# lightalchemist/nonlocal-image-edit

Measured on AMD Instinct MI355X. Metric: megapixels/sec end-to-end enhance (4K img, m=200, K=50); device-resident input and output (host->host per SURVEY 8d: host_to_host.value), higher is better.
Workload: dtype f64; 1 GPU; cfg4: 4096x4096 synthetic luminance, 20x10 samples (p=200), K=50, T=10, L=4 layers; device-resident: the luminance plane is in HBM when the timed region starts and the 4 layer planes are left in HBM (no PCIe inside `value`); parallelism=single GPU, formulation=phi_free_tables, storage=fp64 tables, histograms, reductions and MFMA; fp32 output planes

## Files before the change

nonlocal-image-edit_amd/csrc/generic64.hip:

```cpp
#include "kernels.h"

#include <algorithm>

namespace nlek {

typedef double f64x4 __attribute__((ext_vector_type(4)));

namespace {
__device__ __forceinline__ double recip0_g(double s, double eps) {
    return (fabs(s) >= eps) ? 1.0 / s : 0.0;
}
}

constexpr int kAff64Pix = 64;

template <bool CHROMA>
__global__ __launch_bounds__(256) void k_affinity64(const float* __restrict__ lum, GridSpec gs,
                                                    const Sample4* __restrict__ samples, int p, int ld, double sw,
                                                    double pw, long long pix0, long long M, double* __restrict__ kab,
                                                    int skip_samples, const unsigned* __restrict__ smask,
                                                    const float* __restrict__ pa, const float* __restrict__ pb,
                                                    const float2* __restrict__ sab, double cw) {
    extern __shared__ __attribute__((aligned(16))) unsigned char smem_raw64[];
    int2* srow_col = reinterpret_cast<int2*>(smem_raw64);
// ... 275 lines not shown
        hipLaunchKernelGGL((k_rowpass64<NCLV>), dim3((unsigned)nb), dim3(256), shm, s, mode, d_X, M, ld, w, lw, d_t_in, \
                           d_lam, d_xvec, eps, d_partial);                                                              \
    }
    if (lw <= 64) NLE_RP64(1)
    else if (lw <= 128) NLE_RP64(2)
    else if (lw <= 256) NLE_RP64(4)
    else if (lw <= 512) NLE_RP64(8)
    else if (lw <= 1024) NLE_RP64(16)
    else NLE_RP64(32)
#undef NLE_RP64
    return hipGetLastError();
}

__global__ __launch_bounds__(256) void k_gram64d(const double* __restrict__ X, long long M, int ld, int r,
                                                 const double* __restrict__ cs, long long rows_per_chunk,
                                                 double* __restrict__ partial) {
    const int lane = threadIdx.x & 63, wave = threadIdx.x >> 6, l15 = lane & 15, kq = lane >> 4;
    const int nt = (r + 15) / 16;
    int t = blockIdx.x * 4 + wave;
    const int npairs = nt * (nt + 1) / 2;
    if (t >= npairs) return;
    int ti = 0;
    while (t >= nt - ti) {
        t -= nt - ti;
        ++ti;
    }
    const int tj = ti + t;
    const long long i0 = (long long)blockIdx.y * rows_per_chunk, i1 = min(M, i0 + rows_per_chunk);
    const int ca = ti * 16 + l15, cb = tj * 16 + l15;
    f64x4 acc = f64x4{0.0, 0.0, 0.0, 0.0};
    for (long long i = i0; i < i1; i += 4) {
        const long long row = i + kq;
        const bool ok = row < i1;
        const double c = ok ? (cs ? cs[row] : 1.0) : 0.0;
        const double a = (ok && ca < r) ? c * X[(size_t)row * ld + ca] : 0.0;
        const double b = (ok && cb < r) ? c * X[(size_t)row * ld + cb] : 0.0;
        acc = __builtin_amdgcn_mfma_f64_16x16x4f64(a, b, acc, 0, 0, 0);
    }
    double* out = partial + (size_t)blockIdx.y * r * r;
#pragma unroll
    for (int e = 0; e < 4; ++e) {
        const int ra = ti * 16 + kq + 4 * e;
        if (ra < r && cb < r) out[(size_t)cb * r + ra] = acc[e];
    }
}

__global__ void k_gram64d_reduce(const double* __restrict__ partial, int nchunks, int r, double* __restrict__ G) {
    const long long idx = (long long)blockIdx.x * blockDim.x + threadIdx.x;
    if (idx >= (long long)r * r) return;
    const int a = (int)(idx % r), b = (int)(idx / r);
    const int ta = a / 16, tb = b / 16;
    const size_t src = (ta <= tb) ? (size_t)b * r + a : (size_t)a * r + b;
    double s = 0.0;
    for (int c = 0; c < nchunks; ++c) s += partial[(size_t)c * r * r + src];
    G[idx] = s;
}

long long gram64d_chunk_rows(long long M) {
    long long rows = (M + 255) / 256;
    rows = std::max<long long>(((rows + 3) / 4) * 4, 256);
    return rows;
}
size_t gram64d_partial_elems(long long M, int r) {
    const long long rows = gram64d_chunk_rows(M);
    const long long nchunks = std::max<long long>(1, (M + rows - 1) / rows);
    return (size_t)nchunks * r * r;
}

hipError_t gram64d(hipStream_t s, const double* d_X, long long M, int ld, int r, const double* d_cs, double* d_partial,
                   double* d_G) {
    const long long rows = gram64d_chunk_rows(M);
    const int nchunks = (int)std::max<long long>(1, (M + rows - 1) / rows);
    const int nt = (r + 15) / 16, npairs = nt * (nt + 1) / 2;
    hipError_t e = hipMemsetAsync(d_partial, 0, (size_t)nchunks * r * r * sizeof(double), s);
    if (e != hipSuccess) return e;
    if (M > 0)
        hipLaunchKernelGGL(k_gram64d, dim3((unsigned)((npairs + 3) / 4), (unsigned)nchunks), dim3(256), 0, s, d_X, M, ld, r, d_cs,
                           rows, d_partial);
    hipLaunchKernelGGL(k_gram64d_reduce, dim3((unsigned)(((long long)r * r + 255) / 256)), dim3(256), 0, s, d_partial, nchunks, r,
                       d_G);
    return hipGetLastError();
}

__global__ __launch_bounds__(256) void k_apply_expand64(const double* __restrict__ V, long long M, int ld, int K,
                                                        const double* __restrict__ g, int L, float* __restrict__ Y,
                                                        long long ystride) {
    extern __shared__ __attribute__((aligned(16))) unsigned char smem_raw[];
    double* sg = reinterpret_cast<double*>(smem_raw);
    for (int j = threadIdx.x; j < L * K; j += 256) sg[j] = g[(size_t)(j / K) * ld + (j % K)];
    __syncthreads();
    for (long long i = (long long)blockIdx.x * 256 + threadIdx.x; i < M; i += (long long)gridDim.x * 256) {
        const double* v = V + (size_t)i * ld;
        for (int l = 0; l < L; ++l) {
            double s0 = 0.0, s1 = 0.0;
            int k = 0;
            for (; k + 1 < K; k += 2) {
                s0 += v[k] * sg[l * K + k];
                s1 += v[k + 1] * sg[l * K + k + 1];
            }
            if (k < K) s0 += v[k] * sg[l * K + k];
            Y[(size_t)l * ystride + i] = (float)(s0 + s1);
        }
    }
}

hipError_t apply_expand64(hipStream_t s, const double* d_V, long long M, int ld, int K, const double* d_g, int L, float* d_Y,
                          long long ystride) {
    if (M <= 0 || L <= 0) return hipSuccess;
    const size_t per_layer = (size_t)K * sizeof(double);
    if (per_layer > kApplyLdsBytes) return hipErrorInvalidValue;
    const int lmax = per_layer ? (int)std::min<size_t>(kApplyLdsBytes / per_layer, (size_t)L) : L;
    const int ngroups = (L + lmax - 1) / lmax, lg = (L + ngroups - 1) / ngroups;
    const long long nb = std::min<long long>((M + 255) / 256, 4096);
    for (int l0 = 0; l0 < L; l0 += lg) {
        const int ln = std::min(lg, L - l0);
        const size_t shm = (size_t)ln * per_layer;
        if (shm > 48 * 1024) {
            hipError_t ea = hipFuncSetAttribute(reinterpret_cast<const void*>(k_apply_expand64),
                                                hipFuncAttributeMaxDynamicSharedMemorySize, (int)shm);
            if (ea != hipSuccess) return ea;
        }
        hipLaunchKernelGGL(k_apply_expand64, dim3((unsigned)nb), dim3(256), shm, s, d_V, M, ld, K, d_g + (size_t)l0 * ld, ln,
                           d_Y + (size_t)l0 * ystride, ystride);
    }
    return hipGetLastError();
}

__global__ void k_scatter_rows64(const double* __restrict__ src, const long long* __restrict__ idx, int n, int ld,
                                 double* __restrict__ X, long long M) {
    const long long f = (long long)blockIdx.x * blockDim.x + threadIdx.x;
    if (f >= (long long)n * ld) return;
    const int k = (int)(f / ld), j = (int)(f % ld);
    const long long row = idx[k];
    if (row >= 0 && row < M) X[(size_t)row * ld + j] = src[f];
}

hipError_t scatter_rows64(hipStream_t s, const double* d_src, const long long* d_idx, int n, int ld, double* d_X, long long M) {
    if (n <= 0) return hipSuccess;
    hipLaunchKernelGGL(k_scatter_rows64, dim3((unsigned)(((long long)n * ld + 255) / 256)), dim3(256), 0, s, d_src, d_idx, n, ld,
                       d_X, M);
    return hipGetLastError();
}

__global__ void k_scale_rows64(double* __restrict__ X, int m, int n, const double* __restrict__ dl) {
    const long long f = (long long)blockIdx.x * blockDim.x + threadIdx.x;
    if (f < (long long)m * n) X[f] *= dl[f % m];
}
hipError_t scale_rows64(hipStream_t s, double* d_X, int m, int n, const double* d_dl) {
    if (m <= 0 || n <= 0) return hipSuccess;
    hipLaunchKernelGGL(k_scale_rows64, dim3((unsigned)(((long long)m * n + 255) / 256)), dim3(256), 0, s, d_X, m, n, d_dl);
    return hipGetLastError();
}

__global__ void k_to_f32(const double* __restrict__ X, long long n, float* __restrict__ out) {
    for (long long i = (long long)blockIdx.x * blockDim.x + threadIdx.x; i < n; i += (long long)gridDim.x * blockDim.x)
        out[i] = (float)X[i];
}
hipError_t to_f32(hipStream_t s, const double* d_X, long long n, float* d_out) {
    if (n <= 0) return hipSuccess;
    hipLaunchKernelGGL(k_to_f32, dim3((unsigned)std::min<long long>((n + 255) / 256, 8192)), dim3(256), 0, s, d_X, n, d_out);
    return hipGetLastError();
}

}
```

nonlocal-image-edit_amd/csrc/kernels.h:

```cpp
#pragma once
#include <hip/hip_runtime.h>

#include <vector>

namespace nlek {

struct GridSpec {
    int H, W;
    int rowStep, rowOff, nSelRows;
    int colStep, colOff, nSelCols;
    __host__ __device__ int p() const { return nSelRows * nSelCols; }
};

typedef float4 Sample4;

#if defined(__HIPCC__)
__device__ __forceinline__ float affinity_value(float pr, float pc, float px, Sample4 s, float nsw, float npw) {
    const float dr = pr - s.x, dc = pc - s.y, dv = px - s.z;
    return __builtin_amdgcn_exp2f(nsw * (dr * dr + dc * dc) + npw * (dv * dv));
}
__device__ __forceinline__ bool is_sample_pixel(const GridSpec& gs, int row, int col) {
    const int dr = row - gs.rowOff, dc = col - gs.colOff;
    if (dr < 0 || dc < 0) return false;
    const int qr = dr / gs.rowStep, qc = dc / gs.colStep;
    return (qr * gs.rowStep == dr) && (qc * gs.colStep == dc) && qr < gs.nSelRows && qc < gs.nSelCols;
}
__device__ __forceinline__ bool is_sample(const GridSpec& gs, const unsigned* smask, long long gi, int row, int col) {
    return smask ? ((smask[gi >> 5] >> (unsigned)(gi & 31)) & 1u) != 0 : is_sample_pixel(gs, row, col);
}
#endif

struct LaunchObserver {
    virtual void begin(int sub) = 0;
    virtual void end() = 0;
    virtual ~LaunchObserver() = default;
};
enum { SUB_HIST_G = 0, SUB_HIST_PIX = 1, SUB_HIST_HH = 2, SUB_HIST_Z = 3 };
enum { SUB_GHIST_ROWS = 0, SUB_GHIST_EE = 1, SUB_GHIST_GEMM = 2, SUB_GHIST_FINAL = 3 };

constexpr int kRowpassMaxBlocks = 1024;
constexpr size_t kApplyLdsBytes = 64 * 1024;
constexpr int kGramTilesPerWave = 7;
constexpr int kGramRowsPerStage = 32;

enum RowpassMode { ROWPASS_COLSUM = 0, ROWPASS_RECIP = 1, ROWPASS_XVEC = 2 };

hipError_t gather_samples(hipStream_t s, const float* d_lum, GridSpec gs, float* d_out);
hipError_t gather_samples_slab(hipStream_t s, const float* d_lum, GridSpec gs, int row0, int row1, double* d_out);

hipError_t affinity(hipStream_t s, const float* d_lum, GridSpec gs, const Sample4* d_samples,
                    int p, int ld, float nsw, float npw, long long pix0, long long M,
                    float* d_kab);

hipError_t ts_gemm(hipStream_t s, bool fused, const float* d_A, int lda, const float* d_lum,
                   GridSpec gs, const Sample4* d_samples, float nsw, float npw, long long pix0,
                   const float* d_B, int ldb, int kd, float* d_C, int ldc, long long M,
                   const double* d_u, double eps, const float* d_c = nullptr);

size_t ts_gemm_bf16x3_bsplit_elems(int kd, int ldb);
hipError_t ts_gemm_bf16x3_split(hipStream_t s, const float* d_B, int kd, int ldb, unsigned short* d_Bs);
hipError_t ts_gemm_bf16x3(hipStream_t s, const float* d_lum, GridSpec gs, const Sample4* d_samples, float nsw, float npw,
                          long long pix0, const unsigned short* d_Bs, int ldb, int kd, float* d_C, int ldc, long long M,
                          const float* d_c = nullptr);

hipError_t rowpass(hipStream_t s, int mode, const float* d_X, long long M, int ld,
                   const double* d_t_in, const double* d_lam, const float* d_xvec, double eps,
                   double* d_partial, int* nblocks);
hipError_t reduce_partials(hipStream_t s, const double* d_partial, int nblocks, int ld,
                           double* d_t_out, int nslices = 1);
hipError_t scale_vec(hipStream_t s, const double* d_lam, const double* d_t, int n, double* d_u);
hipError_t row_scalings(hipStream_t s, const float* d_X, long long M, int ld, const double* d_u,
                        double eps, double* d_out);

int gram_num_tiles(int ld);
int gram_chunk_rows(long long M);
size_t gram_partial_elems(long long M, int ld);
hipError_t gram(hipStream_t s, const float* d_X, long long M, int ld, const double* d_u,
                double eps, double* d_partial, double* d_tiles);
hipError_t gram_reduce(hipStream_t s, const double* d_partial, int nchunks, int ntiles, double* d_tiles);

int sink_pass_ld(int p);
int sink_pass_rows(long long M);
int sink_pass_max_p();
hipError_t sink_pass(hipStream_t s, int mode, const float* d_lum, GridSpec gs, const Sample4* d_samples,
                     int p, const double* d_w, float nsw, float npw, long long pix0, long long M, double eps,
                     double* d_ybuf, double* d_partial);
hipError_t sink_update(hipStream_t s, int mode, int p, int r, bool chol, const double* d_X1, const double* d_X2,
                       const double* d_lam, const double* d_z, int zrows, int zld, const double* d_sA_cur, double eps,
                       double* d_v, double* d_u, double* d_sA_next, double* d_w_next);
constexpr int kG64TilesPerWave = 23;
int gram64_ld(int p);
int gram64_num_tiles(int p);
size_t gram64_partial_elems(long long M, int p);
hipError_t gram64(hipStream_t s, const float* d_lum, GridSpec gs, const Sample4* d_samples, int p, float nsw,
                  float npw, long long pix0, long long M, const double* d_c, double* d_partial, double* d_tiles);
int project64_ld(int K);
hipError_t project64(hipStream_t s, const float* d_lum, GridSpec gs, const Sample4* d_samples, int p, float nsw,
                     float npw, long long pix0, long long M, const double* d_D, int K, const double* d_c, float* d_V,
                     int ldv);

hipError_t check_levels(hipStream_t s, const float* d_lum, long long n, int* d_flag);
hipError_t hist_tables(hipStream_t s, GridSpec gs, const Sample4* d_samples, int p, double hx, double hy, int row0,
                       int nrows_local, double* d_er, double* d_ecT, double* d_Ep);

hipError_t affinity64(hipStream_t s, const float* d_lum, GridSpec gs, const Sample4* d_samples, int p, int ld, double sw,
                      double pw, long long pix0, long long M, double* d_kab, bool skip_samples = false,
                      const unsigned* d_smask = nullptr);
constexpr size_t kDynLdsDefault = 64 * 1024;
size_t affinity64_chroma_lds_bytes(int ld);
hipError_t affinity64_chroma(hipStream_t s, const float* d_lum, const float* d_a, const float* d_b, GridSpec gs,
                             const Sample4* d_samples, const float2* d_sab, int p, int ld, double sw, double pw, double cw,
                             long long pix0, long long M, double* d_kab, bool skip_samples = false,
                             const unsigned* d_smask = nullptr);
int patch_kpad(int R);
size_t patch_spatch_bytes(int p, int R);
hipError_t patch_gather(hipStream_t s, const float* d_lum, int H, int W, int R, const long long* d_pix, int n, int* d_out);
hipError_t patch_affinity64(hipStream_t s, const float* d_lum, GridSpec gs, int R, const Sample4* d_samples,
                            const signed char* d_spatch, const int* d_snorm, int p, int ld, double sw, double pwd,
                            long long pix0, long long M, double* d_kab, bool skip_samples = false,
                            const unsigned* d_smask = nullptr);
int patch_ckpad(int R);
size_t patch_cpatch_bytes(int p, int R);
constexpr size_t kPatchChromaLdsMax = 128 * 1024;
size_t patch_affinity64_chroma_lds_bytes(int ld);
hipError_t patch_affinity64_chroma(hipStream_t s, const float* d_lum, const float* d_a, const float* d_b, GridSpec gs, int R,
                                   const Sample4* d_samples, const signed char* d_spatch, const int* d_snorm,
                                   const signed char* d_cpatch, const int* d_cnorm, int p, int ld, double sw, double pwd,
                                   double cwd, long long pix0, long long M, double* d_kab, bool skip_samples = false,
                                   const unsigned* d_smask = nullptr);
int farthest_max_blocks();
hipError_t farthest_samples(hipStream_t s, const float* d_lum, int H, int W, int p, double sw, double pw, double* d_m,
                            double* d_pv, int* d_pi, int* d_list);
hipError_t gather_pix(hipStream_t s, const float* d_lum, const long long* d_pix, int n, float* d_out);
hipError_t sample_mask(hipStream_t s, const long long* d_pix, int n, long long N, unsigned* d_mask);
hipError_t add64(hipStream_t s, double* d_y, const double* d_x, size_t n);
hipError_t row_scalings64(hipStream_t s, const double* d_X, long long M, int ld, int r, const double* d_u, double eps,
                          double* d_out);
hipError_t ts_gemm64(hipStream_t s, const double* d_A, long long M, int lda, int kd, const double* d_B, int nc,
                     const double* d_rs, double* d_C, int ldc);
hipError_t gemm64s(hipStream_t s, int m, int n, int kk, const double* A, long long rsA, long long csA, const double* B,
                   long long rsB, long long csB, double* C, long long rsC, long long csC, const double* dl = nullptr,
                   const double* dk = nullptr, const double* dr = nullptr, const double* add = nullptr, long long rsD = 0,
                   long long csD = 0);
hipError_t rowpass64(hipStream_t s, int mode, const double* d_X, long long M, int ld, int w, const double* d_t_in,
                     const double* d_lam, const float* d_xvec, double eps, double* d_partial, int* nblocks);
size_t gram64d_partial_elems(long long M, int r);
hipError_t gram64d(hipStream_t s, const double* d_X, long long M, int ld, int r, const double* d_cs, double* d_partial,
                   double* d_G);
hipError_t apply_expand64(hipStream_t s, const double* d_V, long long M, int ld, int K, const double* d_g, int L, float* d_Y,
                          long long ystride);
hipError_t scatter_rows64(hipStream_t s, const double* d_src, const long long* d_idx, int n, int ld, double* d_X, long long M);
hipError_t to_f32(hipStream_t s, const double* d_X, long long n, float* d_out);
hipError_t scale_rows64(hipStream_t s, double* d_X, int m, int n, const double* d_dl);

int tridiag_max_n();
hipError_t tridiag(hipStream_t s, int n, const double* d_Q, const double* d_diag_add, double* d_V, double* d_d, double* d_e,
                   double* d_hs);

int sytrd_max_n();
int sytrd_groups(int n);
size_t sytrd_pub_elems(int n);
hipError_t sytrd_dist(hipStream_t s, int n, int G, const double* d_A, const double* d_diag_add, double* d_pub, double* d_d,
                      double* d_e, int* d_status);
hipError_t tridiag_bisect(hipStream_t s, int n, const double* d_d, const double* d_e, double* d_D);
hipError_t sytrd_back(hipStream_t s, int n, const double* d_pub, int K, double* d_Z, int ldz);
size_t potrf_tmp_elems(int n);
hipError_t potrf_inverse(hipStream_t s, int n, const double* d_A, double* d_L, double* d_Linv, double* d_tmp, double* d_scal,
                         int* d_status);
hipError_t transpose64(hipStream_t s, int n, const double* d_src, double* d_dst, int lds = 0, int ldd = 0);
hipError_t symm_lower64(hipStream_t s, int n, const double* d_src, double* d_dst);
hipError_t fill64(hipStream_t s, double* d_p, size_t n, double v);
hipError_t scale_rc64(hipStream_t s, int n, const double* d_src, int lds, const double* d_dl, const double* d_dr, double* d_dst);

constexpr int kSortedThreads = 512;
struct SortedRows {
    const unsigned short* scol;
    const uint2* desc;
    const unsigned short* first;
    const double* E;
    bool rec;
    double kappa;
    const double* E2 = nullptr;
    double hx = 0.0;
    int lev_t0 = 0, lev_nt = 16;
    bool mom = false;
};
bool sorted_gsum_ok(GridSpec gs, double hx);
hipError_t sorted_gram_sums(hipStream_t s, GridSpec gs, int nrows_local, const unsigned short* d_scol, const uint2* d_desc,
                            const unsigned short* d_first, const double* d_E2, const double* d_cvec, double* d_Aout, double hx);
bool sorted_recurrence(GridSpec gs, double hx, double* kappa);
int sorted_max_width();
size_t sorted_scol_elems(int W, int nrows_local);
int sorted_gram_max_cols();
int sorted_expand_max_cols();
int sorted_expand_max_width();
int sorted_expand_layers(GridSpec gs);
hipError_t sorted_expand(hipStream_t s, GridSpec gs, int nrows_local, const unsigned short* d_scol, const uint2* d_desc,
                         const double* d_E, const double* d_g, size_t gstride, int nl, const double* d_cvec, float* d_out,
                         long long ostride, bool rec = false, double kappa = 0.0, bool round8 = false);
hipError_t dist_table(hipStream_t s, int W, double hx, double* d_E);
hipError_t sort_rows(hipStream_t s, const float* d_lum, GridSpec gs, int row0, int nrows_local, unsigned short* d_scol,
                     uint2* d_desc, unsigned short* d_first);
hipError_t sorted_pass(hipStream_t s, int mode, GridSpec gs, int row0, int nrows_local, const unsigned short* d_scol,
                       const uint2* d_desc, const unsigned short* d_first, const double* d_E, const double* d_g, double eps,
                       double* d_ybuf, double* d_h, const double* d_cvec, const float* d_xvec, bool rec, double kappa,
                       int lev_t0 = 0, int lev_nt = 16,
                       bool mom = false);
bool sorted_moments_ok(GridSpec gs, double hx);
hipError_t sorted_gram_rows(hipStream_t s, GridSpec gs, int nrows_local, const unsigned short* d_scol, const uint2* d_desc,
                            const unsigned short* d_first, const double* d_E, const double* d_cvec, double* d_Aout, bool rec,
                            double kappa);

size_t hist_tiled_workspace_elems(GridSpec gs, int nrows_local);
hipError_t sink_hist_tiled(hipStream_t s, int mode, const float* d_lum, GridSpec gs, int p, int ldp, int row0,
                           int nrows_local, const double* d_er, const double* d_ecT, const double* d_Ep,
                           const double* d_w, double eps, double* d_ybuf, double* d_ws, double* d_z,
                           LaunchObserver* obs = nullptr, const double* d_cvec = nullptr,
                           const float* d_xvec = nullptr,
                           const SortedRows* sorted = nullptr);
int apply_layers_per_launch(GridSpec gs);
bool use_sorted_expand(GridSpec gs, const SortedRows* sorted);
hipError_t apply_hist_layers(hipStream_t s, const float* d_lum, GridSpec gs, int p, int row0, int nrows_local,
                             const double* d_er, const double* d_ecT, const double* d_Ep, const double* d_wl, int ldw,
                             int nl, const double* d_c, double* d_ws, float* d_out, long long ostride,
                             LaunchObserver* obs, const SortedRows* sorted = nullptr, bool round8 = false);
hipError_t apply_small(hipStream_t s, int p, int K, int ldk, int L, int ldw, const double* d_m, const double* d_D,
                       const double* d_Vrows, const double* d_xA , const double* d_resp,
                       double* d_t, double* d_Wp, double* d_YA);
hipError_t scatter_samples(hipStream_t s, int p, int L, const long long* d_loc, const double* d_YA, float* d_Y,
                           long long ystride, bool round8 = false);

int ghist_max_cols();
size_t ghist_workspace_elems(GridSpec gs, int nrows_local);
hipError_t gram_hist(hipStream_t s, const float* d_lum, GridSpec gs, int p, int row0, int nrows_local,
                     const double* d_er, const double* d_ecT, const double* d_Ep, const double* d_c, double* d_ws,
                     double* d_Gk, LaunchObserver* obs = nullptr, const SortedRows* sorted = nullptr);

hipError_t bgr2lab8(hipStream_t s, const unsigned char* d_bgr, long long n, const double* d_lut, unsigned char* d_lab,
                    float* d_L);
hipError_t lab2bgr8(hipStream_t s, const unsigned char* d_lab, const float* d_L, const float* d_a, const float* d_b,
                    long long n, const double* d_lut, unsigned char* d_bgr);
hipError_t channel8(hipStream_t s, const unsigned char* d_img, long long n, int ch, float* d_out);
hipError_t plane_to_u8(hipStream_t s, const float* d_y, long long n, unsigned char* d_out);
hipError_t channel8_plane(hipStream_t s, const unsigned char* d_u8, long long n, float* d_out);
int bilateral8_max_radius();
hipError_t bilateral8(hipStream_t s, const float* d_src, int H, int W, int radius, const float* d_space_w,
                      const float* d_colour_w, float* d_dst);

hipError_t col_range(hipStream_t s, const float* d_X, long long M, int ld, int ncols, float* d_out, int nblocks);

hipError_t apply_expand(hipStream_t s, const float* d_V, long long M, int ld, const double* d_g,
                        int L, float* d_Y, long long ystride);

hipError_t scatter_rows(hipStream_t s, const float* d_src, const long long* d_idx, int n, int ld,
                        float* d_X, long long M);

struct ExactPlane {
    const float* lum;
    int H, W;
    const double* d_es;
    int es_len;
    const double* d_el;
    double* d_part;
};
void exact_tables(int H, int W, double hx, double hy, std::vector<double>* es, std::vector<double>* el);
size_t exact_part_elems(long long N);
hipError_t affinity_product64(hipStream_t s, const ExactPlane& pl, const double* d_X, int ldx, int ncols, double* d_Y, int ldy);
hipError_t exact_start(hipStream_t s, double* d_X, long long N, int ld, int col0, int ncols, unsigned seed);
hipError_t exact_scale2(hipStream_t s, const double* d_X, int ldx, long long N, int b, const double* d_c, const double* d_r,
                        double* d_Z);
hipError_t exact_combine(hipStream_t s, const double* d_Y, long long N, int b, const double* d_c, const double* d_r, double* d_A,
                         int lda);
hipError_t exact_recip(hipStream_t s, double* d_v, long long N, double eps);
hipError_t exact_axpby(hipStream_t s, const double* d_S, int lds, double alpha, const double* d_B, int ldb, double beta,
                       double* d_D, int ldd, long long N, int n, int pad);
int exact_col_blocks(long long N);
hipError_t exact_colnorm2(hipStream_t s, const double* d_A, int lda, const double* d_B, int ldb, const double* d_theta,
                          long long N, int n, double* d_part);
hipError_t exact_colmaxabs(hipStream_t s, const double* d_A, int lda, long long N, int n, double* d_pv);
hipError_t exact_scale_cols(hipStream_t s, double* d_A, int lda, long long N, int n, const double* d_s);

}
```

nonlocal-image-edit_amd/csrc/ortho.h:

```cpp
#pragma once
#include "devsolve.h"

namespace nlep {

constexpr double kCholMaxInvTrace = 1e9;

struct KaDevice {
    DevBuf<double> Ka;
    DevChol ch;
};

struct Nystrom {
    int r = 0, ldr = 0;
    bool chol = false;
    std::shared_ptr<KaDevice> dev;
    std::vector<double> VA;
    std::vector<double> lam;
    std::vector<double> B;
    std::vector<double> Ka;
};

struct Ortho {
    int q = 0, K = 0, r_wa = 0, r_q = 0;
    bool chol_wa = false;
    std::vector<double> Sq, Cproj, VArows, Wa;
};

struct OrthoSS {
    int q = 0, K = 0, r_wa = 0, r_q = 0;
    bool chol_wa = false;
    std::vector<double> Sq, D, Vrows;
    int p = 0, r = 0;
    std::vector<double> cA, rA, Kr, P, Wa, S, St, A2;
};

Ortho orthogonalize_host(const Nystrom& ny, int p, const std::vector<double>& u_c, const std::vector<double>& u_r,
                         std::vector<double> G, int n_eig, bool device_f32 = true, int topk_solver = 0);
void ortho_ss_prepare(OrthoSS& o, const Nystrom& ny, int p, const std::vector<double>& sA_c, const std::vector<double>& sA_r,
                      bool literal_q = false);
void ortho_ss_finish(OrthoSS& o, std::vector<double> Gk, int n_eig, int topk_solver = 0);
void ortho_ss_device(nle_ctx* c, OrthoSS& o, const Nystrom& ny, int p, const std::vector<double>& sA_c,
                     const std::vector<double>& sA_r, double* d_Gk, int n_eig, const std::function<void()>& enqueue_gram,
                     const std::function<void()>& reduce_gram, double* host_ms, double* host_overlapped_ms, Trace& tr);

}
```

nonlocal-image-edit_amd/csrc/ortho.hip:

```cpp
#include "ortho.h"

using namespace nlep;

namespace {

template <typename F>
void par_cols(int n, long long work_per_col, F&& body) {
    const long long work = work_per_col * n;
    const int nt = (int)std::min<long long>(std::min<long long>(16, work / 40000000 + 1), n);
    if (nt <= 1) {
        body(0, n);
        return;
    }
    nleh::run_parts(nt, nt, [&](int t) { body((int)((long long)n * t / nt), (int)((long long)n * (t + 1) / nt)); });
}
void mm(const double* A, const double* B, double* C, int m, int k, int n) {
    par_cols(n, (long long)m * k, [&](int j0, int j1) { nleh::gemm_nn_cols(A, B, C, m, k, n, j0, j1); });
}
void mm_nt(const double* A, const double* B, double* C, int m, int k, int n) {
    par_cols(n, (long long)m * k, [&](int j0, int j1) { nleh::gemm_nt_cols(A, B, C, m, k, n, j0, j1); });
}
void mm_tn(const double* A, const double* B, double* C, int m, int k, int n) {
    par_cols(n, (long long)m * k, [&](int j0, int j1) { nleh::gemm_tn_cols(A, B, C, m, k, n, j0, j1); });
}

void top_eigenpairs(const std::vector<double>& Qm, int q, int n_eig, int solver, std::vector<double>* Vq,
                    std::vector<double>* Sq, int* rq) {
    if (solver == 1 && q > 1) {
        const int nev = std::min(std::max(n_eig, 1), q - 1);
        Vq->assign((size_t)q * nev, 0.0);
        Sq->assign(nev, 0.0);
        int restarts = 0;
        const int nconv = nleh::lanczos_topk(Qm.data(), q, nev, NLE_EPS, 1000, Vq->data(), Sq->data(), &restarts);
        if (nconv < 0) throw Fail{NLE_ERR_NUMERIC, "Lanczos: the projected eigenproblem did not converge"};
        if (nconv < nev)
            std::fprintf(stderr, "# converged eigenvalues: %d\nEigen decomposition NOT successful. Results might be inaccurate.\n", nconv);
        int r = 0;
        while (r < nconv && (*Sq)[r] >= NLE_EPS) ++r;
        *rq = r;
        if (std::getenv("NLE_TRACE")) std::fprintf(stderr, "[nle trace] Lanczos top-%d of %d: %d restarts, %d converged\n", nev, q, restarts, nconv);
        return;
    }
    Vq->assign((size_t)q * std::min(q, std::max(n_eig, 1)), 0.0);
    Sq->assign(q, 0.0);
    if (!nleh::eigen_decomposition_topk(Qm.data(), q, NLE_EPS, n_eig, Vq->data(), Sq->data(), rq))
        throw Fail{NLE_ERR_NUMERIC, "eigensolver did not converge on Q"};
}

void trace_wa(int kept, int q, double largest, double smallest_kept, int nd = -1, const char* where = "") {
    if (!std::getenv("NLE_TRACE")) return;
    char defl[64] = "";
    if (nd >= 0) std::snprintf(defl, sizeof defl, ", %d deflated%s", nd, where);
    std::fprintf(stderr, "[nle trace] Wa: %d of %d eigenvalues >= 1e-10 (largest %.3e, smallest kept %.3e)%s\n", kept, q, largest,
                 smallest_kept, defl);
}

struct EigRoot {
    std::vector<double> U2, l2, Us;
    int r2 = 0;
};
EigRoot eigen_root(const std::vector<double>& Wa, int q) {
    EigRoot e;
    e.U2.resize((size_t)q * q);
    e.l2.resize(q);
    if (!nleh::eigen_decomposition(Wa.data(), q, NLE_EPS, e.U2.data(), e.l2.data(), &e.r2))
        throw Fail{NLE_ERR_NUMERIC, "eigensolver did not converge on Wa"};
    e.Us.resize((size_t)q * std::max(e.r2, 1));
    for (int k = 0; k < e.r2; ++k) {
        const double s = std::sqrt(recip0(e.l2[k]));
        for (int i = 0; i < q; ++i) e.Us[(size_t)k * q + i] = e.U2[(size_t)k * q + i] * s;
    }
    trace_wa(e.r2, q, e.l2[0], e.r2 > 0 ? e.l2[e.r2 - 1] : 0.0);
    return e;
}

bool certified_cholesky(const std::vector<double>& Wa, int q, std::vector<double>& L, std::vector<double>& Li) {
    double inv_diag = 0.0;
    for (int a = 0; a < q; ++a) inv_diag += Wa[(size_t)a * q + a] > 0.0 ? 1.0 / Wa[(size_t)a * q + a] : 1e300;
    if (!(inv_diag <= kCholMaxInvTrace)) return false;
    L.resize((size_t)q * q);
    Li.resize((size_t)q * q);
    double inv_trace = 0.0;
    return nleh::cholesky_with_inverse(Wa.data(), q, L.data(), Li.data(), &inv_trace, kCholMaxInvTrace) && inv_trace <= kCholMaxInvTrace;
}

void sample_scalings(OrthoSS& o, const Nystrom& ny, int p, const std::vector<double>& sA_c, const std::vector<double>& sA_r) {
    o.p = p;
    o.r = ny.r;
    o.q = ny.r;
    o.cA.resize(p);
    o.rA.resize(p);
    for (int a = 0; a < p; ++a) {
        o.cA[a] = recip0(sA_c[a]);
        o.rA[a] = recip0(sA_r[a]);
    }
}

void build_Wa(OrthoSS& o) {
    const int p = o.p, q = o.q;
    o.Wa.resize((size_t)q * q);
    for (int b = 0; b < q; ++b)
        for (int a = 0; a < q; ++a) o.Wa[(size_t)b * q + a] = o.rA[a] * o.Kr[(size_t)b * p + a] * o.cA[b];
}

}

namespace nlep {

Ortho orthogonalize_host(const Nystrom& ny, int p, const std::vector<double>& u_c,
                         const std::vector<double>& u_r, std::vector<double> G, int n_eig, bool device_f32,
                         int topk_solver) {
    const int r = ny.r, q = ny.r;
    std::vector<double> cA(q), rA(q), cA32(q);
    std::vector<double> left((size_t)q * r), right((size_t)q * r), phi32((size_t)q * r);
    for (int a = 0; a < q; ++a) {
        double sc = 0.0, sr = 0.0, sc32 = 0.0;
        for (int k = 0; k < r; ++k) {
            const double v = ny.VA[(size_t)k * p + a];
            const double v32 = device_f32 ? (double)(float)v : v;
            phi32[(size_t)k * q + a] = v32;
            sc += v * u_c[k];
            sr += v * u_r[k];
            sc32 += v32 * u_c[k];
        }
        cA[a] = recip0(sc);
        rA[a] = recip0(sr);
        cA32[a] = recip0(sc32);
    }
    for (int k = 0; k < r; ++k)
        for (int a = 0; a < q; ++a) {
            const double v = ny.VA[(size_t)k * p + a];
            left[(size_t)k * q + a] = rA[a] * v * ny.lam[k];
            right[(size_t)k * q + a] = cA[a] * v;
        }
    Ortho o;
    o.q = q;
    o.Wa.resize((size_t)q * q);
    mm_nt(left.data(), right.data(), o.Wa.data(), q, r, q);
    for (int a = 0; a < q; ++a) {
        const double c2 = cA32[a] * cA32[a];
        for (int j = 0; j < r; ++j) {
            const double vj = c2 * phi32[(size_t)j * q + a];
            for (int i = 0; i < r; ++i) G[(size_t)j * r + i] -= phi32[(size_t)i * q + a] * vj;
        }
    }
    std::vector<double> LG((size_t)q * r), WW((size_t)q * q);
    mm(left.data(), G.data(), LG.data(), q, r, r);
    mm_nt(LG.data(), left.data(), WW.data(), q, r, q);
    const auto [U2, l2, Us, r2] = eigen_root(o.Wa, q);
    std::vector<double> S((size_t)q * q);
    o.r_wa = r2;
    if (r2 <= 0) throw Fail{NLE_ERR_NUMERIC, "Wa has no eigenvalue >= 1e-10"};
    std::vector<double> Vq, Sq, T2;
    int rq = 0, K = 0;
    if (topk_solver == 0) {
        std::vector<double> WF((size_t)q * r2), Qt((size_t)r2 * r2);
        mm(WW.data(), Us.data(), WF.data(), q, q, r2);
        mm_tn(Us.data(), WF.data(), Qt.data(), q, r2, r2);
        for (int k = 0; k < r2; ++k) Qt[(size_t)k * r2 + k] += l2[k];
        std::vector<double> Vt;
        top_eigenpairs(Qt, r2, n_eig, topk_solver, &Vt, &Sq, &rq);
        K = std::min(n_eig, rq);
        if (K <= 0) throw Fail{NLE_ERR_NUMERIC, "Q has no eigenvalue >= 1e-10"};
        T2.resize((size_t)q * K);
        mm(Us.data(), Vt.data(), T2.data(), q, r2, K);
    } else {
        mm_nt(Us.data(), U2.data(), S.data(), q, r2, q);
        std::vector<double> T1((size_t)q * q), Qm((size_t)q * q);
        mm(S.data(), WW.data(), T1.data(), q, q, q);
        mm(T1.data(), S.data(), Qm.data(), q, q, q);
        for (size_t i = 0; i < Qm.size(); ++i) Qm[i] += o.Wa[i];
        top_eigenpairs(Qm, q, n_eig, topk_solver, &Vq, &Sq, &rq);
        K = std::min(n_eig, rq);
        if (K <= 0) throw Fail{NLE_ERR_NUMERIC, "Q has no eigenvalue >= 1e-10"};
        T2.resize((size_t)q * K);
        mm(S.data(), Vq.data(), T2.data(), q, q, K);
    }
    o.K = K;
    o.r_q = rq;
    o.Sq.assign(Sq.begin(), Sq.begin() + K);
    for (int k = 0; k < K; ++k) {
        const double s = std::sqrt(recip0(Sq[k]));
        for (int i = 0; i < q; ++i) T2[(size_t)k * q + i] *= s;
    }
    o.Cproj.resize((size_t)r * K);
    mm_tn(left.data(), T2.data(), o.Cproj.data(), q, r, K);
    o.VArows.resize((size_t)q * K);
    mm(o.Wa.data(), T2.data(), o.VArows.data(), q, q, K);
    return o;
}

void ortho_ss_prepare(OrthoSS& o, const Nystrom& ny, int p, const std::vector<double>& sA_c,
                      const std::vector<double>& sA_r, bool literal_q) {
    const int r = ny.r, q = ny.r;
    sample_scalings(o, ny, p, sA_c, sA_r);
    if (ny.chol) {
        o.Kr = ny.Ka;
    } else {
        std::vector<double> VL((size_t)p * r);
        o.Kr.resize((size_t)p * p);
        for (int k = 0; k < r; ++k)
            for (int a = 0; a < p; ++a) VL[(size_t)k * p + a] = ny.VA[(size_t)k * p + a] * ny.lam[k];
        mm_nt(VL.data(), ny.VA.data(), o.Kr.data(), p, r, p);
        if (r < p) {
            o.P.resize((size_t)p * p);
            mm_nt(ny.VA.data(), ny.VA.data(), o.P.data(), p, r, p);
        }
    }
    build_Wa(o);
    o.S.resize((size_t)q * q);
    if (!literal_q && std::getenv("NLE_FORCE_EIG") == nullptr) {
        std::vector<double> L, Li;
        if (certified_cholesky(o.Wa, q, L, Li)) {
            std::vector<double> Lt((size_t)q * q);
            for (int k = 0; k < q; ++k)
                for (int a = 0; a < q; ++a) {
                    o.S[(size_t)k * q + a] = Li[(size_t)a * q + k];
                    Lt[(size_t)k * q + a] = L[(size_t)a * q + k];
                }
            o.St = std::move(Li);
            o.A2.resize((size_t)q * q);
            mm(Lt.data(), L.data(), o.A2.data(), q, q, q);
            o.r_wa = q;
            o.chol_wa = true;
            return;
        }
    }
    const auto [U2, l2, Us, r2] = eigen_root(o.Wa, q);
    mm_nt(Us.data(), U2.data(), o.S.data(), q, r2, q);
    o.r_wa = r2;
    o.St = o.S;
    o.A2 = o.Wa;
}

void ortho_ss_finish(OrthoSS& o, std::vector<double> Gk, int n_eig, int topk_solver) {
    const int p = o.p, r = o.r, q = o.q;
    const std::vector<double>&cA = o.cA, &rA = o.rA, &Kr = o.Kr, &Wa = o.Wa, &S = o.S;
    for (int a = q; a < p; ++a) {
        const double c2 = cA[a] * cA[a];
        const double* ka = Kr.data() + (size_t)a * p;
        for (int j = 0; j < p; ++j) {
            const double vj = c2 * ka[j];
            for (int i = 0; i < p; ++i) Gk[(size_t)j * p + i] += ka[i] * vj;
        }
    }
    if (r < p) {
        std::vector<double> T((size_t)p * p);
        mm(o.P.data(), Gk.data(), T.data(), p, p, p);
        mm(T.data(), o.P.data(), Gk.data(), p, p, p);
    }
    std::vector<double> WW((size_t)q * q);
    for (int b = 0; b < q; ++b)
        for (int a = 0; a < q; ++a) WW[(size_t)b * q + a] = rA[a] * Gk[(size_t)b * p + a] * rA[b];
    std::vector<double> T1((size_t)q * q), Qm((size_t)q * q);
    mm(o.St.data(), WW.data(), T1.data(), q, q, q);
    mm(T1.data(), S.data(), Qm.data(), q, q, q);
    for (size_t i = 0; i < Qm.size(); ++i) Qm[i] += o.A2[i];
    std::vector<double> Vq, Sq;
    int rq = 0;
    top_eigenpairs(Qm, q, n_eig, topk_solver, &Vq, &Sq, &rq);
    const int K = std::min(n_eig, rq);
    if (K <= 0) throw Fail{NLE_ERR_NUMERIC, "Q has no eigenvalue >= 1e-10"};
    o.K = K;
    o.r_q = rq;
    o.Sq.assign(Sq.begin(), Sq.begin() + K);
    std::vector<double> T2((size_t)q * K), RT2((size_t)q * K);
    mm(S.data(), Vq.data(), T2.data(), q, q, K);
    for (int k = 0; k < K; ++k) {
        const double sv = std::sqrt(recip0(Sq[k]));
        for (int i = 0; i < q; ++i) {
            T2[(size_t)k * q + i] *= sv;
            RT2[(size_t)k * q + i] = rA[i] * T2[(size_t)k * q + i];
        }
    }
    o.D.resize((size_t)p * K);
    if (r < p) {
        mm(o.P.data(), RT2.data(), o.D.data(), p, q, K);
    } else {
        o.D = RT2;
    }
    o.Vrows.assign((size_t)p * K, 0.0);
    std::vector<double> WT((size_t)q * K);
    mm(Wa.data(), T2.data(), WT.data(), q, q, K);
    for (int k = 0; k < K; ++k) {
        for (int a = 0; a < q; ++a) o.Vrows[(size_t)k * p + a] = WT[(size_t)k * q + a];
        for (int a = q; a < p; ++a) {
            double sv = 0.0;
            for (int j = 0; j < p; ++j) sv += Kr[(size_t)a * p + j] * o.D[(size_t)k * p + j];
            o.Vrows[(size_t)k * p + a] = cA[a] * sv;
        }
    }
}

namespace {


struct SsDevice {
    DevBuf<double> rA, cA, Kr, P, VA, lam;
};

void scalings_Kr_P(hipStream_t st, OrthoSS& o, const Nystrom& ny, int p, const std::vector<double>& sA_c,
                   const std::vector<double>& sA_r, SsDevice& dv) {
    const int r = ny.r;
    const size_t pp = (size_t)p * p;
    sample_scalings(o, ny, p, sA_c, sA_r);
    dv.rA.alloc(p);
    dv.cA.alloc(p);
    HIP_OK(hipMemcpyAsync(dv.rA.p, o.rA.data(), p * sizeof(double), hipMemcpyHostToDevice, st));
    HIP_OK(hipMemcpyAsync(dv.cA.p, o.cA.data(), p * sizeof(double), hipMemcpyHostToDevice, st));
    if (ny.chol) {
        o.Kr = ny.Ka;
        return;
    }
    dv.VA.alloc((size_t)p * r);
    dv.lam.alloc(r);
    dv.Kr.alloc(pp);
    HIP_OK(hipMemcpyAsync(dv.VA.p, ny.VA.data(), (size_t)p * r * sizeof(double), hipMemcpyHostToDevice, st));
    HIP_OK(hipMemcpyAsync(dv.lam.p, ny.lam.data(), r * sizeof(double), hipMemcpyHostToDevice, st));
    HIP_OK(nlek::gemm64s(st, p, p, r, dv.VA.p, 1, p, dv.VA.p, p, 1, dv.Kr.p, 1, p, nullptr, dv.lam.p));
    if (r < p) {
        dv.P.alloc(pp);
        HIP_OK(nlek::gemm64s(st, p, p, r, dv.VA.p, 1, p, dv.VA.p, p, 1, dv.P.p, 1, p));
    }
    o.Kr.resize(pp);
    HIP_OK(hipMemcpyAsync(o.Kr.data(), dv.Kr.p, pp * sizeof(double), hipMemcpyDeviceToHost, st));
    HIP_OK(hipStreamSynchronize(st));
}

struct WaRoot {
    enum Form { kEigen, kCholesky, kDeflated } form = kEigen;
    bool on_device = false;
    int m = 0;
    int r_wa = 0, nd = 0;
    std::vector<double> F, L, G, l2_kept;
    DevBuf<double> d_F, d_L, d_G;
    bool chol_form() const { return form != kEigen; }
};

struct WaDeviceWork {
    DevSymEig es;
    DevChol ch;
    DevBuf<double> Ah, Vd, wgt, W, neg1;
};

void wa_root_device(nle_ctx* c, const OrthoSS& o, const Nystrom& ny, const SsDevice& dv, double* d_Wa, bool force_eig,
                    const std::function<void()>& enqueue_gram, WaDeviceWork& ws, WaRoot& w, Trace& tr) {
    const int p = o.p, q = o.q, max_defl = q / 8;
    const size_t qq = (size_t)q * q;
    hipStream_t st = c->stream, sa = aux_stream(c);
    ws.es.prepare(c, q, sa);
    ws.ch.prepare(c, q, sa);
    ws.Ah.alloc(qq);
    w.d_F.alloc(qq);
    ws.Vd.alloc((size_t)q * (max_defl + 1));
    ws.wgt.alloc(max_defl + 1);
    ws.W.alloc((size_t)(max_defl + 1) * q);
    w.d_G.alloc((size_t)q * (max_defl + 1));
    ws.neg1.alloc(max_defl + 1);
    HIP_OK(hipStreamSynchronize(st));
    enqueue_gram();
    if (ny.dev)
        HIP_OK(nlek::scale_rc64(sa, q, ny.dev->Ka.p, p, dv.rA.p, dv.cA.p, d_Wa));
    else
        upload_staged(c, d_Wa, o.Wa.data(), qq, sa);
    HIP_OK(nlek::symm_lower64(sa, q, d_Wa, ws.Ah.p));
    bool reduced = false;
    if (!force_eig) {
        reduced = ws.es.reduce(c, q, ws.Ah.p, nullptr);
        if (c->world > 1) reduced = ranks_where(c, !reduced) == 0;
        tr.mark("ss:   Wa: tridiagonal form + eigenvalues (device)");
    }
    if (reduced) {
        const std::vector<double>& D = ws.es.D;
        int kept = 0;
        while (kept < q && D[kept] >= NLE_EPS) ++kept;
        const int nd = q - kept;
        if (kept > 0 && nd <= max_defl && D[0] > 0.0) {
            const double sig = D[0];
            if (nd > 0) {
                ws.es.vectors(c, kept, nd, ws.Vd.p);
                tr.mark("ss:   Wa: dropped eigenvectors (host inverse iteration)");
                std::vector<double> wgt(nd);
                for (int t = 0; t < nd; ++t) wgt[t] = sig - D[kept + t];
                HIP_OK(hipMemcpyAsync(ws.wgt.p, wgt.data(), nd * sizeof(double), hipMemcpyHostToDevice, sa));
                HIP_OK(nlek::gemm64s(sa, q, q, nd, ws.Vd.p, 1, q, ws.Vd.p, q, 1, ws.Ah.p, 1, q, nullptr, ws.wgt.p, nullptr, ws.Ah.p, 1, q));
                HIP_OK(hipStreamSynchronize(sa));
            }
            ws.ch.factor(c, q, ws.Ah.p);
            const bool fact_ok = ws.ch.finish(c);
            if (!fact_ok && std::getenv("NLE_TRACE"))
                fprintf(stderr, "[nle trace] Wa: the deflated matrix did not factor (trace of the inverse %.3e, %d dropped, sigma %.3e)\n",
                        ws.ch.inv_trace, nd, sig);
            if (fact_ok) {
                HIP_OK(nlek::transpose64(sa, q, ws.ch.Linv.p, w.d_F.p));
                if (nd > 0) {
                    HIP_OK(nlek::fill64(sa, ws.neg1.p, nd, -1.0));
                    HIP_OK(nlek::gemm64s(sa, nd, q, q, ws.Vd.p, q, 1, ws.ch.Linv.p, q, 1, ws.W.p, 1, nd));
                    HIP_OK(nlek::gemm64s(sa, q, q, nd, ws.Vd.p, 1, q, ws.W.p, 1, nd, w.d_F.p, 1, q, nullptr, ws.neg1.p, nullptr, w.d_F.p, 1, q));
                    HIP_OK(nlek::gemm64s(sa, q, nd, q, ws.ch.L.p, q, 1, ws.Vd.p, 1, q, w.d_G.p, 1, q));
                }
                w.form = nd > 0 ? WaRoot::kDeflated : WaRoot::kCholesky;
                w.on_device = true;
                w.r_wa = kept;
                w.nd = nd;
                trace_wa(kept, q, D[0], D[kept - 1], nd, " (device)");
            }
        }
    }
    if (w.on_device) {
        w.d_L.alloc(qq);
        HIP_OK(hipMemcpyAsync(w.d_L.p, ws.ch.L.p, qq * sizeof(double), hipMemcpyDeviceToDevice, sa));
    }
    HIP_OK(hipEventRecord(c->aux_ev, sa));
    HIP_OK(hipStreamWaitEvent(st, c->aux_ev, 0));
}

void wa_root_host(OrthoSS& o, bool cholesky_forms, bool force_eig, WaRoot& w, Trace& tr) {
    const int q = o.q, max_defl = q / 8;
    const size_t qq = (size_t)q * q;
    if (o.Wa.empty()) build_Wa(o);
    std::vector<double>& L = w.L;
    std::vector<double> Li, Vd;
    const bool attempt_chol = q < 64 || q >= 512;
    bool factored = cholesky_forms && !force_eig && attempt_chol && certified_cholesky(o.Wa, q, L, Li);
    int kept = q, nd = 0;
    if (!factored && cholesky_forms && !force_eig && q >= 16 && q < 512) {
        std::vector<double> Dbelow(max_defl + 1);
        Vd.resize((size_t)q * (max_defl + 1));
        double lam_max = 0.0, lam_min_kept = 0.0;
        tr.mark(attempt_chol ? "ss:   Wa built, Cholesky attempt" : "ss:   Wa built");
        if (nleh::sym_eigen_below(o.Wa.data(), q, NLE_EPS, max_defl, &kept, &lam_max, &lam_min_kept, Dbelow.data(), Vd.data())) {
            tr.mark("ss:   Wa eigenvalues + dropped eigenvectors");
            nd = q - kept;
            if (kept > 0 && nd <= max_defl && lam_max > 0.0) {
                const double sig = lam_max;
                std::vector<double> Ah(qq);
                for (int cidx = 0; cidx < q; ++cidx)
                    for (int ridx = 0; ridx < q; ++ridx)
                        Ah[(size_t)cidx * q + ridx] = ridx >= cidx ? o.Wa[(size_t)cidx * q + ridx] : o.Wa[(size_t)ridx * q + cidx];
                for (int t = 0; t < nd; ++t) {
                    const double wgt = sig - Dbelow[t];
                    const double* v = Vd.data() + (size_t)t * q;
                    for (int cidx = 0; cidx < q; ++cidx) {
                        const double vc = wgt * v[cidx];
                        for (int ridx = 0; ridx < q; ++ridx) Ah[(size_t)cidx * q + ridx] += v[ridx] * vc;
                    }
                }
                L.resize(qq);
                Li.resize(qq);
                double inv_trace = 0.0;
                factored = nleh::cholesky_with_inverse(Ah.data(), q, L.data(), Li.data(), &inv_trace);
                if (factored) {
                    tr.mark("ss:   deflated matrix + its Cholesky factor and inverse");
                    trace_wa(kept, q, lam_max, lam_min_kept, nd);
                }
            }
        }
    }
    if (factored) {
        std::vector<double>& F = w.F;
        F.resize(qq);
        for (int k = 0; k < q; ++k)
            for (int a = 0; a < q; ++a) F[(size_t)k * q + a] = Li[(size_t)a * q + k];
        w.G.assign((size_t)q * std::max(nd, 1), 0.0);
        std::vector<double> wv(q);
        for (int t = 0; t < nd; ++t) {
            const double* v = Vd.data() + (size_t)t * q;
            for (int k = 0; k < q; ++k) {
                double acc = 0.0, g = 0.0;
                for (int a = 0; a < q; ++a) {
                    acc += v[a] * Li[(size_t)a * q + k];
                    g += L[(size_t)k * q + a] * v[a];
                }
                wv[k] = acc;
                w.G[(size_t)t * q + k] = g;
            }
            for (int k = 0; k < q; ++k)
                for (int a = 0; a < q; ++a) F[(size_t)k * q + a] -= v[a] * wv[k];
        }
        w.form = nd > 0 ? WaRoot::kDeflated : WaRoot::kCholesky;
        w.r_wa = nd > 0 ? kept : q;
        w.nd = nd;
        return;
    }
    EigRoot e = eigen_root(o.Wa, q);
    w.form = WaRoot::kEigen;
    w.r_wa = e.r2;
    w.l2_kept.assign(e.l2.begin(), e.l2.begin() + e.r2);
    w.F = std::move(e.Us);
}

void upload_host_root(hipStream_t st, int q, WaRoot& w) {
    const size_t qq = (size_t)q * q;
    if (w.chol_form()) {
        w.d_L.alloc(qq);
        HIP_OK(hipMemcpyAsync(w.d_L.p, w.L.data(), qq * sizeof(double), hipMemcpyHostToDevice, st));
    }
    w.d_F.alloc((size_t)q * w.m);
    HIP_OK(hipMemcpyAsync(w.d_F.p, w.F.data(), (size_t)q * w.m * sizeof(double), hipMemcpyHostToDevice, st));
    if (w.form == WaRoot::kDeflated) {
        w.d_G.alloc((size_t)q * w.nd);
        HIP_OK(hipMemcpyAsync(w.d_G.p, w.G.data(), (size_t)q * w.nd * sizeof(double), hipMemcpyHostToDevice, st));
    }
    HIP_OK(hipStreamSynchronize(st));
}

void form_Qt(hipStream_t st, const OrthoSS& o, const SsDevice& dv, const WaRoot& w, double* d_Gk,
             const std::function<void()>& reduce_gram, double* d_Qm) {
    const int p = o.p, r = o.r, q = o.q, m = w.m;
    const size_t qq = (size_t)q * q;
    DevBuf<double> d_T((size_t)p * p), d_T1((size_t)m * q);
    reduce_gram();
    if (q < p) {
        std::vector<double> c2(p - q);
        for (int a = q; a < p; ++a) c2[a - q] = o.cA[a] * o.cA[a];
        DevBuf<double> d_c2(p - q);
        HIP_OK(hipMemcpyAsync(d_c2.p, c2.data(), (p - q) * sizeof(double), hipMemcpyHostToDevice, st));
        HIP_OK(nlek::gemm64s(st, p, p, p - q, dv.Kr.p + (size_t)q * p, 1, p, dv.Kr.p + (size_t)q * p, p, 1, d_Gk, 1, p, nullptr,
                             d_c2.p, nullptr, d_Gk, 1, p));
        HIP_OK(hipStreamSynchronize(st));
    }
    if (r < p) {
        HIP_OK(nlek::gemm64s(st, p, p, p, dv.P.p, 1, p, d_Gk, 1, p, d_T.p, 1, p));
        HIP_OK(nlek::gemm64s(st, p, p, p, d_T.p, 1, p, dv.P.p, 1, p, d_Gk, 1, p));
    }
    HIP_OK(nlek::gemm64s(st, m, q, q, w.d_F.p, q, 1, d_Gk, 1, p, d_T1.p, 1, m, nullptr, dv.rA.p));
    if (!w.chol_form()) {
        HIP_OK(nlek::gemm64s(st, m, m, q, d_T1.p, 1, m, w.d_F.p, 1, q, d_Qm, 1, m, nullptr, dv.rA.p));
        return;
    }
    DevBuf<double> d_A2(qq);
    HIP_OK(nlek::gemm64s(st, q, q, q, w.d_L.p, q, 1, w.d_L.p, 1, q, d_A2.p, 1, q));
    if (w.form == WaRoot::kDeflated) {
        DevBuf<double> d_neg(w.nd);
        HIP_OK(nlek::fill64(st, d_neg.p, w.nd, -1.0));
        HIP_OK(nlek::gemm64s(st, q, q, w.nd, w.d_G.p, 1, q, w.d_G.p, q, 1, d_A2.p, 1, q, nullptr, d_neg.p, nullptr, d_A2.p, 1, q));
    }
    HIP_OK(nlek::gemm64s(st, m, m, q, d_T1.p, 1, m, w.d_F.p, 1, q, d_Qm, 1, m, nullptr, dv.rA.p, nullptr, d_A2.p, 1, q));
}

struct QtEig {
    bool on_device = false;
    std::vector<double> Vq, Sq, sv;
    DevSymEig es;
    DevBuf<double> d_Vq, d_l2q;
};

void top_eigenpairs_Qt(nle_ctx* c, OrthoSS& o, const WaRoot& w, const double* d_Qm, int n_eig, QtEig& t, double* host_ms,
                       Trace& tr) {
    hipStream_t st = c->stream;
    const int m = w.m;
    const size_t mm_ = (size_t)m * m;
    int rq = 0;
    double h0 = 0.0;
    t.on_device = c->topk_solver == 0 && use_dev_solver(m) && !std::getenv("NLE_HOST_Q");
    if (t.on_device) {
        const double* d_add = nullptr;
        if (!w.chol_form()) {
            t.d_l2q.alloc(m);
            HIP_OK(hipMemcpyAsync(t.d_l2q.p, w.l2_kept.data(), m * sizeof(double), hipMemcpyHostToDevice, st));
            d_add = t.d_l2q.p;
        }
        t.on_device = t.es.reduce(c, m, d_Qm, d_add);
        if (c->world > 1) t.on_device = ranks_where(c, !t.on_device) == 0;
    }
    if (t.on_device) {
        tr.mark("ss: Q, its tridiagonal form and eigenvalues (device)");
        h0 = now_ms();
        t.Sq = t.es.D;
        while (rq < m && t.Sq[rq] >= NLE_EPS) ++rq;
        const int Kd = std::min(n_eig, rq);
        if (Kd > 0) {
            t.d_Vq.alloc((size_t)m * Kd);
            t.es.vectors(c, 0, Kd, t.d_Vq.p);
        }
    } else {
        std::vector<double> Qm(mm_);
        HIP_OK(hipMemcpyAsync(Qm.data(), d_Qm, mm_ * sizeof(double), hipMemcpyDeviceToHost, st));
        HIP_OK(hipStreamSynchronize(st));
        tr.mark("ss: Q on the device + download");
        h0 = now_ms();
        if (!w.chol_form())
            for (int k = 0; k < m; ++k) Qm[(size_t)k * m + k] += w.l2_kept[k];
        top_eigenpairs(Qm, m, n_eig, c->topk_solver, &t.Vq, &t.Sq, &rq);
    }
    const int K = std::min(n_eig, rq);
    if (K <= 0) throw Fail{NLE_ERR_NUMERIC, "Q has no eigenvalue >= 1e-10"};
    o.K = K;
    o.r_q = rq;
    o.Sq.assign(t.Sq.begin(), t.Sq.begin() + K);
    t.sv.resize(K);
    for (int k = 0; k < K; ++k) t.sv[k] = std::sqrt(recip0(t.Sq[k]));
    *host_ms += now_ms() - h0;
    tr.mark(t.on_device ? "ss: eigenvectors of Q (inverse iteration on the host, back-transformation enqueued)" : "ss: eig(Q) (host)");
}

void D_and_Vrows(hipStream_t st, OrthoSS& o, const SsDevice& dv, const WaRoot& w, QtEig& t, const double* d_Wa, Trace& tr) {
    const int p = o.p, r = o.r, q = o.q, m = w.m, K = o.K;
    DevBuf<double> d_sv(K), d_T2((size_t)q * K), d_D((size_t)p * K), d_Vr((size_t)p * K);
    if (!t.on_device) {
        t.d_Vq.alloc((size_t)m * K);
        HIP_OK(hipMemcpyAsync(t.d_Vq.p, t.Vq.data(), (size_t)m * K * sizeof(double), hipMemcpyHostToDevice, st));
    }
    HIP_OK(hipMemcpyAsync(d_sv.p, t.sv.data(), K * sizeof(double), hipMemcpyHostToDevice, st));
    HIP_OK(nlek::gemm64s(st, q, K, m, w.d_F.p, 1, q, t.d_Vq.p, 1, m, d_T2.p, 1, q, nullptr, nullptr, d_sv.p));
    if (r < p) {
        HIP_OK(nlek::gemm64s(st, p, K, q, dv.P.p, 1, p, d_T2.p, 1, q, d_D.p, 1, p, nullptr, dv.rA.p));
    } else {
        HIP_OK(hipMemcpyAsync(d_D.p, d_T2.p, (size_t)q * K * sizeof(double), hipMemcpyDeviceToDevice, st));
        HIP_OK(nlek::scale_rows64(st, d_D.p, p, K, dv.rA.p));
    }
    HIP_OK(nlek::gemm64s(st, q, K, q, d_Wa, 1, q, d_T2.p, 1, q, d_Vr.p, 1, p));
    if (q < p)
        HIP_OK(nlek::gemm64s(st, p - q, K, p, dv.Kr.p + q, 1, p, d_D.p, 1, p, d_Vr.p + q, 1, p, dv.cA.p + q));
    o.D.resize((size_t)p * K);
    o.Vrows.resize((size_t)p * K);
    HIP_OK(hipMemcpyAsync(o.D.data(), d_D.p, o.D.size() * sizeof(double), hipMemcpyDeviceToHost, st));
    HIP_OK(hipMemcpyAsync(o.Vrows.data(), d_Vr.p, o.Vrows.size() * sizeof(double), hipMemcpyDeviceToHost, st));
    HIP_OK(hipStreamSynchronize(st));
    tr.mark("ss: D, Vrows on the device");
}

}

void ortho_ss_device(nle_ctx* c, OrthoSS& o, const Nystrom& ny, int p, const std::vector<double>& sA_c,
                     const std::vector<double>& sA_r, double* d_Gk, int n_eig, const std::function<void()>& enqueue_gram,
                     const std::function<void()>& reduce_gram, double* host_ms, double* host_overlapped_ms, Trace& tr) {
    const int q = ny.r;
    hipStream_t st = c->stream;
    SsDevice dv;
    scalings_Kr_P(st, o, ny, p, sA_c, sA_r, dv);
    const double h0 = now_ms();
    const bool dev_wa = use_dev_solver(q) && !std::getenv("NLE_HOST_WA");
    const bool force_eig = std::getenv("NLE_FORCE_EIG") != nullptr;
    if (!(dev_wa && ny.dev)) build_Wa(o);
    DevBuf<double> d_Wa((size_t)q * q);
    WaRoot w;
    WaDeviceWork ws;
    if (dev_wa)
        wa_root_device(c, o, ny, dv, d_Wa.p, force_eig, enqueue_gram, ws, w, tr);
    else
        enqueue_gram();
    if (!w.on_device) wa_root_host(o, !dev_wa, force_eig, w, tr);
    o.r_wa = w.r_wa;
    o.chol_wa = w.form == WaRoot::kCholesky;
    *host_overlapped_ms += now_ms() - h0;
    tr.mark(w.on_device ? "ss: Wa root (device, second stream, beside the Gram kernels)" : "ss: Wa root (host, under the Gram kernels)");
    w.m = w.chol_form() ? q : std::max(w.r_wa, 0);
    if (w.m <= 0) throw Fail{NLE_ERR_NUMERIC, "Wa has no eigenvalue >= 1e-10"};
    DevBuf<double> d_Qm((size_t)w.m * w.m);
    if (!dev_wa) HIP_OK(hipMemcpyAsync(d_Wa.p, o.Wa.data(), (size_t)q * q * sizeof(double), hipMemcpyHostToDevice, st));
    if (!w.on_device) upload_host_root(st, q, w);
    form_Qt(st, o, dv, w, d_Gk, reduce_gram, d_Qm.p);
    QtEig t;
    top_eigenpairs_Qt(c, o, w, d_Qm.p, n_eig, t, host_ms, tr);
    D_and_Vrows(st, o, dv, w, t, d_Wa.p, tr);
}

}
```

nonlocal-image-edit_amd/csrc/pipeline.hip:

```cpp
#include "ortho.h"

using nlek::GridSpec;
using namespace nlep;

namespace {
struct SampleSet {
    GridSpec gs;
    int p = 0;
    std::vector<long long> pix;
    std::vector<float> val;
    std::vector<float4> packed;
    bool quantised = false;
    unsigned level_tiles = 0xffffu;
    int R = 0;
    bool listed = false;
    std::vector<int> patch;
    const float* d_a = nullptr;
    const float* d_b = nullptr;
    double hc = 0.0;
    bool chroma_quantised = false;
    std::vector<int> aval, bval;
    bool chroma() const { return d_a != nullptr; }
};

// ... 189 lines not shown
    const double sw = 1.0 / (hx * hx), pwd = (1.0 / (hy * hy)) / d;
    const bool chroma = s.chroma();
    const double cwd = chroma ? chroma_cwd(s) : 0.0;
    std::vector<double> Ka((size_t)p * p);
    for (int j = 0; j < p; ++j) {
        const int rj = (int)(s.pix[j] / s.gs.W), cj = (int)(s.pix[j] % s.gs.W);
        const int* yj = s.patch.data() + (size_t)j * d;
        for (int i = j; i < p; ++i) {
            const int ri = (int)(s.pix[i] / s.gs.W), ci = (int)(s.pix[i] % s.gs.W);
            const int* yi = s.patch.data() + (size_t)i * d;
            long long S = 0;
            for (int k = 0; k < d; ++k) S += (long long)(yi[k] - yj[k]) * (yi[k] - yj[k]);
            const long long dr = ri - rj, dc = ci - cj;
            double e = -sw * (double)(dr * dr + dc * dc) - pwd * (double)S;
            if (chroma) e = e - cwd * (double)chroma_ssd(s, i, j);
            const double v = std::exp(e);
            Ka[(size_t)j * p + i] = v;
            Ka[(size_t)i * p + j] = v;
        }
    }
    return Ka;
}

struct PatchOperands {
    DevBuf<signed char> spatch;
    DevBuf<int> snorm;
    DevBuf<float2> sab;
    DevBuf<signed char> cpatch;
    DevBuf<int> cnorm;
};
void upload_chroma_operands(nle_ctx* c, const SampleSet& s, PatchOperands* po) {
    if (s.R <= 0) {
        std::vector<float2> ab(s.p);
        for (int j = 0; j < s.p; ++j) ab[j] = make_float2((float)s.aval[j], (float)s.bval[j]);
        po->sab.alloc(s.p);
        HIP_OK(hipMemcpyAsync(po->sab.p, ab.data(), ab.size() * sizeof(float2), hipMemcpyHostToDevice, c->stream));
        HIP_OK(hipStreamSynchronize(c->stream));
        return;
    }
    const int d = (2 * s.R + 1) * (2 * s.R + 1), kp = nlek::patch_ckpad(s.R);
    std::vector<signed char> bytes(nlek::patch_cpatch_bytes(s.p, s.R), 0);
    std::vector<int> norm(s.p, 0);
    for (int j = 0; j < s.p; ++j)
        for (int k = 0; k < 2 * d; ++k) {
            const int v = (k < d ? s.aval[(size_t)j * d + k] : s.bval[(size_t)j * d + k - d]) - 128;
            bytes[(size_t)j * kp + k] = (signed char)v;
            norm[j] += v * v;
        }
    po->cpatch.alloc(bytes.size());
    po->cnorm.alloc(s.p);
    HIP_OK(hipMemcpyAsync(po->cpatch.p, bytes.data(), bytes.size(), hipMemcpyHostToDevice, c->stream));
    HIP_OK(hipMemcpyAsync(po->cnorm.p, norm.data(), norm.size() * sizeof(int), hipMemcpyHostToDevice, c->stream));
    HIP_OK(hipStreamSynchronize(c->stream));
}
void upload_patch_operands(nle_ctx* c, const SampleSet& s, PatchOperands* po) {
    if (s.chroma()) upload_chroma_operands(c, s, po);
    if (s.R <= 0) return;
    const int d = (2 * s.R + 1) * (2 * s.R + 1), kp = nlek::patch_kpad(s.R);
    std::vector<signed char> bytes(nlek::patch_spatch_bytes(s.p, s.R), 0);
    std::vector<int> norm(s.p, 0);
    for (int j = 0; j < s.p; ++j)
        for (int k = 0; k < d; ++k) {
            const int v = s.patch[(size_t)j * d + k] - 128;
            bytes[(size_t)j * kp + k] = (signed char)v;
            norm[j] += v * v;
        }
    po->spatch.alloc(bytes.size());
    po->snorm.alloc(s.p);
    HIP_OK(hipMemcpyAsync(po->spatch.p, bytes.data(), bytes.size(), hipMemcpyHostToDevice, c->stream));
    HIP_OK(hipMemcpyAsync(po->snorm.p, norm.data(), norm.size() * sizeof(int), hipMemcpyHostToDevice, c->stream));
    HIP_OK(hipStreamSynchronize(c->stream));
}

hipError_t affinity_rows64(hipStream_t st, const float* d_lum, const SampleSet& ss, const float4* d_samples,
                           const PatchOperands& po, int ld, double hx, double hy, long long pix0, long long M, double* d_kab,
                           bool skip_samples = false, const unsigned* d_smask = nullptr) {
    const double sw = 1.0 / (hx * hx), pw = 1.0 / (hy * hy);
    if (ss.chroma()) {
        const double cwd = chroma_cwd(ss);
        if (ss.R <= 0)
            return nlek::affinity64_chroma(st, d_lum, ss.d_a, ss.d_b, ss.gs, d_samples, po.sab.p, ss.p, ld, sw, pw, cwd, pix0, M,
                                           d_kab, skip_samples, d_smask);
        return nlek::patch_affinity64_chroma(st, d_lum, ss.d_a, ss.d_b, ss.gs, ss.R, d_samples, po.spatch.p, po.snorm.p,
                                             po.cpatch.p, po.cnorm.p, ss.p, ld, sw, pw / ((2 * ss.R + 1) * (2 * ss.R + 1)), cwd,
                                             pix0, M, d_kab, skip_samples, d_smask);
    }
    if (ss.R <= 0)
        return nlek::affinity64(st, d_lum, ss.gs, d_samples, ss.p, ld, sw, pw, pix0, M, d_kab, skip_samples, d_smask);
    const double pwd = pw / ((2 * ss.R + 1) * (2 * ss.R + 1));
    return nlek::patch_affinity64(st, d_lum, ss.gs, ss.R, d_samples, po.spatch.p, po.snorm.p, ss.p, ld, sw, pwd, pix0, M, d_kab,
                                  skip_samples, d_smask);
}

std::vector<double> build_Ka(const SampleSet& s, double hx, double hy) {
    if (s.R > 0) return build_Ka_patch(s, hx, hy);
    const int p = s.p;
    const double sw = 1.0 / (hx * hx), pw = 1.0 / (hy * hy);
    const bool chroma = s.chroma();
    const double cw = chroma ? chroma_cwd(s) : 0.0;
    std::vector<double> Ka((size_t)p * p);
    auto column = [&](int j) {
        const int rj = (int)(s.pix[j] / s.gs.W), cj = (int)(s.pix[j] % s.gs.W);
        for (int i = j; i < p; ++i) {
            const int ri = (int)(s.pix[i] / s.gs.W), ci = (int)(s.pix[i] % s.gs.W);
            const long long dr = ri - rj, dc = ci - cj;
            const double sq = (double)(dr * dr + dc * dc);
            const double dv = (double)s.val[i] - (double)s.val[j];
            double e = -sw * sq - pw * (dv * dv);
            if (chroma) e = e - cw * (double)chroma_ssd(s, i, j);
            const double v = std::exp(e);
            Ka[(size_t)j * p + i] = v;
            Ka[(size_t)i * p + j] = v;
        }
    };
    const int nt = p >= 384 ? 8 : 1;
    std::vector<int> cut(nt + 1, p);
    for (int t = 0; t < nt; ++t) cut[t] = (int)(p * (1.0 - std::sqrt(1.0 - (double)t / nt)));
    nleh::run_parts(nt, nt, [&](int t) {
        for (int j = cut[t]; j < cut[t + 1]; ++j) column(j);
    });
    return Ka;
}



Nystrom solve_Ka(nle_ctx* c, const std::vector<double>& Ka, int p, bool allow_chol) {
    Nystrom n;
    if (allow_chol && std::getenv("NLE_FORCE_EIG") == nullptr) {
        if (c && use_dev_solver(p) && !std::getenv("NLE_HOST_KA")) {
            const size_t pp = (size_t)p * p;
            auto kd = std::make_shared<KaDevice>();
            kd->Ka.alloc(pp);
            upload_staged(c, kd->Ka.p, Ka.data(), pp, c->stream);
            kd->ch.factor(c, p, kd->Ka.p);
            if (kd->ch.finish(c) && kd->ch.inv_trace <= kCholMaxInvTrace) {
                n.chol = true;
                n.r = p;
                n.ldr = ld4(p);
                n.lam.assign(p, 1.0);
                n.Ka = Ka;
                n.dev = std::move(kd);
                return n;
            }
        } else {
            std::vector<double> L((size_t)p * p), Li((size_t)p * p);
            double inv_trace = 0.0;
            if (nleh::cholesky_with_inverse(Ka.data(), p, L.data(), Li.data(), &inv_trace, kCholMaxInvTrace) &&
                inv_trace <= kCholMaxInvTrace) {
                n.chol = true;
                n.r = p;
                n.ldr = ld4(p);
                n.VA = std::move(L);
                n.lam.assign(p, 1.0);
                n.B.resize((size_t)p * p);
                for (int k = 0; k < p; ++k)
                    for (int a = 0; a < p; ++a) n.B[(size_t)k * p + a] = Li[(size_t)a * p + k];
                n.Ka = Ka;
                return n;
            }
        }
    }
    std::vector<double> U((size_t)p * p), D(p);
    int r = 0;
    if (!nleh::eigen_decomposition(Ka.data(), p, NLE_EPS, U.data(), D.data(), &r))
        throw Fail{NLE_ERR_NUMERIC, "eigensolver did not converge on Ka"};
    int nnz = 0;
    for (int k = 0; k < r; ++k)
        if (std::fabs(D[k]) >= NLE_EPS) ++nnz;
    r = std::min(r, nnz);
    if (r <= 0) throw Fail{NLE_ERR_NUMERIC, "Ka has no eigenvalue >= 1e-10"};
    n.r = r;
    n.ldr = ld4(r);
    n.VA.assign(U.begin(), U.begin() + (size_t)p * r);
    n.lam.assign(D.begin(), D.begin() + r);
    n.B.resize((size_t)p * r);
    for (int k = 0; k < r; ++k) {
        const double inv = recip0(n.lam[k]);
        for (int a = 0; a < p; ++a) n.B[(size_t)k * p + a] = n.VA[(size_t)k * p + a] * inv;
    }
    return n;
}

std::vector<float> build_B(const Nystrom& n, int p) {
    std::vector<float> B((size_t)p * n.ldr, 0.f);
    for (int k = 0; k < n.r; ++k) {
        const double inv = recip0(n.lam[k]);
        for (int s = 0; s < p; ++s) B[(size_t)s * n.ldr + k] = (float)(n.VA[(size_t)k * p + s] * inv);
    }
    return B;
}

inline hipError_t scatter_rows_any(hipStream_t s, const float* rows, const long long* idx, int n, int ld, float* d_X,
                                   long long M) {
    return nlek::scatter_rows(s, rows, idx, n, ld, d_X, M);
}
inline hipError_t scatter_rows_any(hipStream_t s, const double* rows, const long long* idx, int n, int ld, double* d_X,
                                   long long M) {
    return nlek::scatter_rows64(s, rows, idx, n, ld, d_X, M);
}

template <typename T>
void scatter_sample_rows(nle_ctx* c, const std::vector<long long>& pix, int nrows, const std::vector<double>& src, int K,
                         int ld, long long pix0, long long M, T* d_X) {
    std::vector<T> rows;
    std::vector<long long> idx;
    for (int a = 0; a < nrows; ++a) {
        const long long loc = pix[a] - pix0;
        if (loc < 0 || loc >= M) continue;
        idx.push_back(loc);
        const size_t off = rows.size();
        rows.resize(off + ld, T(0));
        for (int k = 0; k < K; ++k) rows[off + k] = (T)src[(size_t)k * nrows + a];
    }
    DevBuf<T> d_rows(rows.size());
    DevBuf<long long> d_idx(idx.size());
    if (!idx.empty()) {
        HIP_OK(hipMemcpyAsync(d_rows.p, rows.data(), rows.size() * sizeof(T), hipMemcpyHostToDevice, c->stream));
        HIP_OK(hipMemcpyAsync(d_idx.p, idx.data(), idx.size() * sizeof(long long), hipMemcpyHostToDevice, c->stream));
        PROFILED(c, NLE_K_SMALL, scatter_rows_any(c->stream, d_rows.p, d_idx.p, (int)idx.size(), ld, d_X, M));
    }
    HIP_OK(hipStreamSynchronize(c->stream));
}

void build_phi(nle_ctx* c, const float* d_lum, const SampleSet& ss, const Nystrom& ny, double hx,
               double hy, long long pix0, long long M, float* d_phi) {
    const int p = ss.p;
    DevBuf<float4> d_samples(p);
    HIP_OK(hipMemcpyAsync(d_samples.p, ss.packed.data(), p * sizeof(float4), hipMemcpyHostToDevice, c->stream));
    std::vector<float> B = build_B(ny, p);
    DevBuf<float> d_B(B.size());
    HIP_OK(hipMemcpyAsync(d_B.p, B.data(), B.size() * sizeof(float), hipMemcpyHostToDevice, c->stream));
    const float sw = nsw_of(hx), pw = nsw_of(hy);
    static const bool env3 = std::getenv("NLE_NYSTROM_BF16X3") != nullptr;
    if (c->nystrom_bf16x3 || env3) {
        DevBuf<unsigned short> d_Bs(nlek::ts_gemm_bf16x3_bsplit_elems(p, ny.ldr));
        HIP_OK(nlek::ts_gemm_bf16x3_split(c->stream, d_B.p, p, ny.ldr, d_Bs.p));
        PROFILED(c, NLE_K_NYSTROM, nlek::ts_gemm_bf16x3(c->stream, d_lum, ss.gs, d_samples.p, sw, pw, pix0, d_Bs.p, ny.ldr, p,
                                                        d_phi, ny.ldr, M));
    } else {
        PROFILED(c, NLE_K_NYSTROM, nlek::ts_gemm(c->stream, true, nullptr, 0, d_lum, ss.gs, d_samples.p, sw, pw, pix0,
                                                 d_B.p, ny.ldr, p, d_phi, ny.ldr, M, nullptr, NLE_EPS));
    }
    scatter_sample_rows(c, ss.pix, p, ny.VA, ny.r, ny.ldr, pix0, M, d_phi);
}

inline hipError_t rowpass_any(hipStream_t s, int mode, const float* X, long long M, int ld, int , const double* t,
                              const double* lam, const float* xv, double eps, double* partial, int* nb) {
    return nlek::rowpass(s, mode, X, M, ld, t, lam, xv, eps, partial, nb);
}
inline hipError_t rowpass_any(hipStream_t s, int mode, const double* X, long long M, int ld, int r, const double* t,
                              const double* lam, const float* xv, double eps, double* partial, int* nb) {
    return nlek::rowpass64(s, mode, X, M, ld, r, t, lam, xv, eps, partial, nb);
}
inline int pass_width(const float*, int ld, int ) { return ld; }
inline int pass_width(const double*, int , int r) { return ld4(r); }

template <typename T_>
void sinkhorn_passes(nle_ctx* c, const T_* d_phi, long long M, int ld_phi, int r,
                     const std::vector<double>& lam, int T, std::vector<double>* u_c,
                     std::vector<double>* u_r, double* d_u_c_out ) {
    if (T < 1) throw Fail{NLE_ERR_INVALID, "nSinkhornIter must be >= 1"};
    if (std::is_same<T_, double>::value && r > 2048)
        throw Fail{NLE_ERR_INVALID, "the fp64 Sinkhorn pass takes a logical width of at most 2048"};
    const int ld = pass_width(d_phi, ld_phi, r);
    std::vector<double> lam_pad(ld, 0.0);
    std::copy(lam.begin(), lam.begin() + r, lam_pad.begin());
    DevBuf<double> d_lam(ld), d_t[3], d_partial((size_t)nlek::kRowpassMaxBlocks * ld);
    for (auto& b : d_t) b.alloc(ld);
    HIP_OK(hipMemcpyAsync(d_lam.p, lam_pad.data(), ld * sizeof(double), hipMemcpyHostToDevice, c->stream));
    int nb = 0;
    PROFILED(c, NLE_K_SINKHORN_PASS, rowpass_any(c->stream, nlek::ROWPASS_COLSUM, d_phi, M, ld_phi, r, nullptr, nullptr,
                                                   nullptr, NLE_EPS, d_partial.p, &nb));
    PROFILED(c, NLE_K_REDUCE, nlek::reduce_partials(c->stream, d_partial.p, nb, ld, d_t[0].p));
    all_reduce(c, d_t[0].p, ld);
    int cur = 0;
    int idx_c_in = 0, idx_r_in = 0;
    for (int it = 0; it < T; ++it) {
        idx_c_in = cur;
        int nxt = (cur + 1) % 3;
        PROFILED(c, NLE_K_SINKHORN_PASS, rowpass_any(c->stream, nlek::ROWPASS_RECIP, d_phi, M, ld_phi, r, d_t[cur].p,
                                                       d_lam.p, nullptr, NLE_EPS, d_partial.p, &nb));
        PROFILED(c, NLE_K_REDUCE, nlek::reduce_partials(c->stream, d_partial.p, nb, ld, d_t[nxt].p));
        all_reduce(c, d_t[nxt].p, ld);
        cur = nxt;
        idx_r_in = cur;
        if (it + 1 < T) {
            nxt = (cur + 1) % 3;
            if (nxt == idx_c_in) nxt = (nxt + 1) % 3;
            PROFILED(c, NLE_K_SINKHORN_PASS, rowpass_any(c->stream, nlek::ROWPASS_RECIP, d_phi, M, ld_phi, r, d_t[cur].p,
                                                           d_lam.p, nullptr, NLE_EPS, d_partial.p, &nb));
            PROFILED(c, NLE_K_REDUCE, nlek::reduce_partials(c->stream, d_partial.p, nb, ld, d_t[nxt].p));
            all_reduce(c, d_t[nxt].p, ld);
            cur = nxt;
        }
    }
    std::vector<double> tc(ld), tr(ld);
    HIP_OK(hipMemcpyAsync(tc.data(), d_t[idx_c_in].p, ld * sizeof(double), hipMemcpyDeviceToHost, c->stream));
    HIP_OK(hipMemcpyAsync(tr.data(), d_t[idx_r_in].p, ld * sizeof(double), hipMemcpyDeviceToHost, c->stream));
    if (d_u_c_out) PROFILED(c, NLE_K_SMALL, nlek::scale_vec(c->stream, d_lam.p, d_t[idx_c_in].p, ld, d_u_c_out));
    HIP_OK(hipStreamSynchronize(c->stream));
    u_c->assign(r, 0.0);
    u_r->assign(r, 0.0);
    for (int k = 0; k < r; ++k) {
        (*u_c)[k] = lam[k] * tc[k];
        (*u_r)[k] = lam[k] * tr[k];
    }
}

std::vector<double> unpack_tiles(const std::vector<double>& tiles, int ld, int n, int ts) {
// ... 10 lines not shown
                    if (ti == tj && j < i) continue;
                    const double v = tl[a * ts + b];
                    G[(size_t)j * n + i] = v;
                    G[(size_t)i * n + j] = v;
                }
        }
    return G;
}

std::vector<double> gram_all(nle_ctx* c, const float* d_phi, long long M, int ld, int r, const double* d_u) {
    const int ntiles = nlek::gram_num_tiles(ld);
    DevBuf<double> d_partial(std::max<size_t>(nlek::gram_partial_elems(std::max<long long>(M, 1), ld), 1));
    DevBuf<double> d_tiles((size_t)ntiles * 1024);
    if (M > 0) {
        PROFILED(c, NLE_K_GRAM, nlek::gram(c->stream, d_phi, M, ld, d_u, NLE_EPS, d_partial.p, d_tiles.p));
    } else {
        HIP_OK(hipMemsetAsync(d_tiles.p, 0, (size_t)ntiles * 1024 * sizeof(double), c->stream));
    }
    all_reduce(c, d_tiles.p, (size_t)ntiles * 1024);
    std::vector<double> tiles((size_t)ntiles * 1024);
    HIP_OK(hipMemcpyAsync(tiles.data(), d_tiles.p, tiles.size() * sizeof(double), hipMemcpyDeviceToHost, c->stream));
    HIP_OK(hipStreamSynchronize(c->stream));
    return unpack_tiles(tiles, ld, r, 32);
}

struct StageMs {
    double sinkhorn = 0, gram = 0, project = 0, host = 0, host_overlapped = 0;
    void take(Timer& s, Timer& g, Timer& p) {
        sinkhorn = s.ms();
        gram = g.ms();
        project = p.ms();
    }
};

template <typename O>
void adopt_ortho(nle_filter* f, const O& o) {
    f->K = o.K;
    f->ldv = ld4(o.K);
    f->eigvals = o.Sq;
    f->r_wa = o.r_wa;
    f->r_q = o.r_q;
    f->chol_wa = o.chol_wa ? 1 : 0;
}

void train_materialised(nle_ctx* c, nle_filter* f, const float* d_lum, const SampleSet& ss, const Nystrom& ny,
                        double hx, double hy, int T, int n_eig, long long pix0, long long M, StageMs* ms) {
    Timer tm_s(c->stream), tm_g(c->stream), tm_p(c->stream);
    tm_s.start();
    DevBuf<float> d_phi((size_t)std::max<long long>(M, 1) * ny.ldr);
    build_phi(c, d_lum, ss, ny, hx, hy, pix0, M, d_phi.p);
    std::vector<double> u_c, u_r;
    DevBuf<double> d_u_c(ny.ldr);
    sinkhorn_passes(c, d_phi.p, M, ny.ldr, ny.r, ny.lam, T, &u_c, &u_r, d_u_c.p);
    tm_s.stop();
    tm_g.start();
    std::vector<double> G = gram_all(c, d_phi.p, M, ny.ldr, ny.r, d_u_c.p);
    tm_g.stop();
    double h0 = now_ms();
    Ortho o = orthogonalize_host(ny, ss.p, u_c, u_r, std::move(G), n_eig, true, c->topk_solver);
    ms->host += now_ms() - h0;
    adopt_ortho(f, o);
    f->formulation = NLE_MODE_MATERIALISED;
    tm_p.start();
    std::vector<float> Cp((size_t)ny.r * f->ldv, 0.f);
    for (int k = 0; k < o.K; ++k)
        for (int j = 0; j < ny.r; ++j) Cp[(size_t)j * f->ldv + k] = (float)o.Cproj[(size_t)k * ny.r + j];
    DevBuf<float> d_Cp(Cp.size());
    HIP_OK(hipMemcpyAsync(d_Cp.p, Cp.data(), Cp.size() * sizeof(float), hipMemcpyHostToDevice, c->stream));
    DevBuf<float> d_V((size_t)std::max<long long>(M, 1) * f->ldv);
    PROFILED(c, NLE_K_PROJECT, nlek::ts_gemm(c->stream, false, d_phi.p, ny.ldr, nullptr, ss.gs, nullptr, 0.f, 0.f, 0,
                                             d_Cp.p, f->ldv, ny.r, d_V.p, f->ldv, M, d_u_c.p, NLE_EPS));
    scatter_sample_rows(c, ss.pix, o.q, o.VArows, o.K, f->ldv, pix0, M, d_V.p);
    tm_p.stop();
    HIP_OK(hipStreamSynchronize(c->stream));
    f->v_bytes = d_V.n * sizeof(float);
    f->d_V = d_V.take();
    ms->take(tm_s, tm_g, tm_p);
}

void build_phi64(nle_ctx* c, const float* d_lum, const SampleSet& ss, const Nystrom& ny, double hx, double hy, long long pix0,
                 long long M, double* d_phi) {
    const int p = ss.p, ldp = ld4(p), r = ny.r, ldr = ny.ldr;
    DevBuf<float4> d_samples(p);
    HIP_OK(hipMemcpyAsync(d_samples.p, ss.packed.data(), p * sizeof(float4), hipMemcpyHostToDevice, c->stream));
    DevBuf<double> d_B(ny.B.size());
    HIP_OK(hipMemcpyAsync(d_B.p, ny.B.data(), ny.B.size() * sizeof(double), hipMemcpyHostToDevice, c->stream));
    PatchOperands po;
    upload_patch_operands(c, ss, &po);
    HIP_OK(hipMemsetAsync(d_phi, 0, (size_t)std::max<long long>(M, 1) * ldr * sizeof(double), c->stream));
    const long long chunk = 1ll << 20;
    DevBuf<double> d_kab((size_t)std::min<long long>(std::max<long long>(M, 1), chunk) * ldp);
    for (long long i0 = 0; i0 < M; i0 += chunk) {
        const long long m = std::min(chunk, M - i0);
        PROFILED(c, NLE_K_AFFINITY, affinity_rows64(c->stream, d_lum, ss, d_samples.p, po, ldp, hx, hy, pix0 + i0, m, d_kab.p));
        PROFILED(c, NLE_K_NYSTROM, nlek::ts_gemm64(c->stream, d_kab.p, m, ldp, p, d_B.p, r, nullptr, d_phi + (size_t)i0 * ldr, ldr));
    }
    scatter_sample_rows(c, ss.pix, p, ny.VA, r, ldr, pix0, M, d_phi);
}

std::vector<double> gram_all64(nle_ctx* c, const double* d_phi, long long M, int ld, int r, const double* d_u) {
    DevBuf<double> d_cs, d_part(std::max<size_t>(nlek::gram64d_partial_elems(std::max<long long>(M, 1), r), 1)), d_G((size_t)r * r);
    if (d_u && M > 0) {
        d_cs.alloc((size_t)M);
        PROFILED(c, NLE_K_SMALL, nlek::row_scalings64(c->stream, d_phi, M, ld, r, d_u, NLE_EPS, d_cs.p));
    }
    PROFILED(c, NLE_K_GRAM, nlek::gram64d(c->stream, d_phi, M, ld, r, d_cs.p, d_part.p, d_G.p));
    all_reduce(c, d_G.p, (size_t)r * r);
    std::vector<double> G((size_t)r * r);
    HIP_OK(hipMemcpyAsync(G.data(), d_G.p, G.size() * sizeof(double), hipMemcpyDeviceToHost, c->stream));
    HIP_OK(hipStreamSynchronize(c->stream));
    return G;
}

void train_generic64(nle_ctx* c, nle_filter* f, const float* d_lum, const SampleSet& ss, const Nystrom& ny, double hx,
                     double hy, int T, int n_eig, long long pix0, long long M, StageMs* ms) {
    Timer tm_s(c->stream), tm_g(c->stream), tm_p(c->stream);
    tm_s.start();
    const size_t phi_elems = (size_t)std::max<long long>(M, 1) * ny.ldr;
    size_t free_b = 0, total_b = 0;
    const bool no_fit = hipMemGetInfo(&free_b, &total_b) == hipSuccess && phi_elems * sizeof(double) > free_b + c->arena_bytes;
    if (ranks_where(c, no_fit) > 0)
        throw Fail{NLE_ERR_INVALID, "fp64 formulation: Phi (N x r doubles) does not fit in device memory; use an integer-valued "
                                    "luminance plane with a sample grid of at most 32 x 36 (table formulation) or NLE_MODE_MATERIALISED"};
    DevBuf<double> d_phi(phi_elems);
    build_phi64(c, d_lum, ss, ny, hx, hy, pix0, M, d_phi.p);
    std::vector<double> u_c, u_r;
    DevBuf<double> d_u_c(ny.ldr);
    sinkhorn_passes(c, d_phi.p, M, ny.ldr, ny.r, ny.lam, T, &u_c, &u_r, d_u_c.p);
    tm_s.stop();
    tm_g.start();
    std::vector<double> G = gram_all64(c, d_phi.p, M, ny.ldr, ny.r, d_u_c.p);
    tm_g.stop();
    double h0 = now_ms();
    Ortho o = orthogonalize_host(ny, ss.p, u_c, u_r, std::move(G), n_eig, false, c->topk_solver);
    ms->host += now_ms() - h0;
    adopt_ortho(f, o);
    f->formulation = NLE_MODE_MATERIALISED_F64;
    tm_p.start();
    DevBuf<double> d_Cp(o.Cproj.size()), d_cs((size_t)std::max<long long>(M, 1));
    HIP_OK(hipMemcpyAsync(d_Cp.p, o.Cproj.data(), o.Cproj.size() * sizeof(double), hipMemcpyHostToDevice, c->stream));
    PROFILED(c, NLE_K_SMALL, nlek::row_scalings64(c->stream, d_phi.p, M, ny.ldr, ny.r, d_u_c.p, NLE_EPS, d_cs.p));
    DevBuf<double> d_V((size_t)std::max<long long>(M, 1) * f->ldv);
    HIP_OK(hipMemsetAsync(d_V.p, 0, d_V.n * sizeof(double), c->stream));
    PROFILED(c, NLE_K_PROJECT, nlek::ts_gemm64(c->stream, d_phi.p, M, ny.ldr, ny.r, d_Cp.p, o.K, d_cs.p, d_V.p, f->ldv));
    scatter_sample_rows(c, ss.pix, o.q, o.VArows, o.K, f->ldv, pix0, M, d_V.p);
    tm_p.stop();
    HIP_OK(hipStreamSynchronize(c->stream));
    f->v64_bytes = d_V.n * sizeof(double);
    f->d_V64 = d_V.take();
    ms->take(tm_s, tm_g, tm_p);
}

void build_update_operands(nle_ctx* c, const Nystrom& ny, int p, DevBuf<double>& d_X1, DevBuf<double>& d_X2,
                           DevBuf<double>& d_lam) {
    const int r = ny.r;
    if (ny.dev) {
        const size_t n2 = (size_t)2 * p, pp = (size_t)p * p;
        d_X1.alloc(n2 * p);
        d_X2.alloc(n2 * p);
        d_lam.alloc(p);
        HIP_OK(hipMemsetAsync(d_X1.p, 0, n2 * p * sizeof(double), c->stream));
        HIP_OK(nlek::transpose64(c->stream, p, ny.dev->ch.Linv.p, d_X1.p, p, 2 * p));
        HIP_OK(hipMemcpyAsync(d_X2.p, ny.dev->ch.Linv.p, pp * sizeof(double), hipMemcpyDeviceToDevice, c->stream));
        HIP_OK(hipMemcpyAsync(d_X2.p + pp, ny.dev->Ka.p, pp * sizeof(double), hipMemcpyDeviceToDevice, c->stream));
        HIP_OK(nlek::fill64(c->stream, d_lam.p, p, 1.0));
    } else {
        const size_t n2 = (size_t)2 * p;
        std::vector<double> X1(n2 * r, 0.0), X2(n2 * r);
        for (int k = 0; k < r; ++k)
            for (int a = 0; a < p; ++a) {
                const double b = ny.B[(size_t)k * p + a];
                const double va = ny.chol ? ny.Ka[(size_t)k * p + a] : ny.VA[(size_t)k * p + a];
                X1[(size_t)k * n2 + a] = b;
                if (!ny.chol) X1[(size_t)k * n2 + p + a] = va;
                X2[(size_t)a * r + k] = b;
                X2[(size_t)(p + a) * r + k] = va;
            }
        d_X1.alloc(X1.size());
        d_X2.alloc(X2.size());
        d_lam.alloc(r);
        HIP_OK(hipMemcpyAsync(d_X1.p, X1.data(), X1.size() * sizeof(double), hipMemcpyHostToDevice, c->stream));
        HIP_OK(hipMemcpyAsync(d_X2.p, X2.data(), X2.size() * sizeof(double), hipMemcpyHostToDevice, c->stream));
        HIP_OK(hipMemcpyAsync(d_lam.p, ny.lam.data(), r * sizeof(double), hipMemcpyHostToDevice, c->stream));
        HIP_OK(hipStreamSynchronize(c->stream));
    }
}

struct SampleSinkhorn {
    nle_ctx* c;
    int p, T, zld;
    DevBuf<double> d_w, d_sAh, d_X1, d_X2, d_lam, d_uv;
    std::vector<double> sA_c, sA_r;

    SampleSinkhorn(nle_ctx* c_, int p_, int zld_, int T_)
        : c(c_), p(p_), T(T_), zld(zld_), d_w(zld_), d_sAh((size_t)2 * T_ * p_), d_uv((size_t)3 * p_) {
        HIP_OK(hipMemsetAsync(d_w.p, 0, zld * sizeof(double), c->stream));
    }

    Nystrom run(const std::function<Nystrom()>& solve, const std::function<void(int, bool)>& pass_pixels, double* d_z,
                int zrows) {
        pass_pixels(nlek::ROWPASS_COLSUM, false);
        Nystrom ny = solve();
        build_update_operands(c, ny, p, d_X1, d_X2, d_lam);
        auto update = [&](int n, int mode) {
            all_reduce(c, d_z, (size_t)zrows * zld);
            PROFILED(c, NLE_K_SMALL,
                     nlek::sink_update(c->stream, mode, p, ny.r, ny.chol, d_X1.p, d_X2.p, d_lam.p, d_z, zrows, zld,
                                       n > 0 ? d_sAh.p + (size_t)(n - 1) * p : nullptr, NLE_EPS, d_uv.p, d_uv.p + 2 * p,
                                       d_sAh.p + (size_t)n * p, d_w.p));
        };
        update(0, nlek::ROWPASS_COLSUM);
        for (int n = 1; n < 2 * T; ++n) {
            pass_pixels(nlek::ROWPASS_RECIP, n == 2 * T - 1);
            update(n, nlek::ROWPASS_RECIP);
        }
        sA_c.resize(p);
        sA_r.resize(p);
        HIP_OK(hipMemcpyAsync(sA_c.data(), d_sAh.p + (size_t)(2 * T - 2) * p, p * sizeof(double), hipMemcpyDeviceToHost,
                              c->stream));
        HIP_OK(hipMemcpyAsync(sA_r.data(), d_sAh.p + (size_t)(2 * T - 1) * p, p * sizeof(double), hipMemcpyDeviceToHost,
                              c->stream));
        return ny;
    }
};

void train_sample_space(nle_ctx* c, nle_filter* f, const float* d_lum, const SampleSet& ss,
                        const std::function<Nystrom()>& solve, double hx, double hy, int T, int n_eig, long long pix0,
                        long long M, StageMs* ms) {
    const int p = ss.p;
    const int P64 = nlek::sink_pass_ld(p);
    const float nsw = nsw_of(hx), npw = nsw_of(hy);
    Trace tr;
    Timer tm_s(c->stream), tm_g(c->stream), tm_p(c->stream);
    tm_s.start();
    DevBuf<float4> d_samples(P64);
    HIP_OK(hipMemsetAsync(d_samples.p, 0, P64 * sizeof(float4), c->stream));
    HIP_OK(hipMemcpyAsync(d_samples.p, ss.packed.data(), p * sizeof(float4), hipMemcpyHostToDevice, c->stream));
    constexpr int kZS = 8;
    const int npart = nlek::sink_pass_rows(std::max<long long>(M, 1));
    DevBuf<double> d_z((size_t)kZS * P64), d_partial, d_cbuf((size_t)std::max<long long>(M, 1));
    const bool hist = ss.quantised && c->mode != NLE_MODE_PHI_FREE_EXP && ss.gs.nSelCols <= nlek::ghist_max_cols() &&
                      ss.gs.nSelRows <= 32 && M > 0;
    if (!hist && p > nlek::sink_pass_max_p()) throw Fail{NLE_ERR_INVALID, "Phi-free path: too many samples for the generic kernels"};
    const int nrows_local = (int)(M / ss.gs.W), row0 = (int)(pix0 / ss.gs.W);
    DevBuf<double> d_er, d_ecT, d_Ep, d_hws;
    if (hist) {
        d_er.alloc((size_t)nrows_local * ss.gs.nSelRows);
        d_ecT.alloc((size_t)ss.gs.nSelCols * ss.gs.W);
        d_Ep.alloc((size_t)256 * p);
        d_hws.alloc(nlek::hist_tiled_workspace_elems(ss.gs, nrows_local));
        PROFILED(c, NLE_K_SMALL, nlek::hist_tables(c->stream, ss.gs, d_samples.p, p, hx, hy, row0, nrows_local, d_er.p,
                                                   d_ecT.p, d_Ep.p));
    } else {
        d_partial.alloc((size_t)npart * P64);
    }
    SampleSinkhorn sk(c, p, P64, T);
    const bool sorted = hist && ss.gs.W <= nlek::sorted_max_width() && std::getenv("NLE_NO_SORTED_ROWS") == nullptr;
    DevBuf<unsigned short> d_scol, d_first;
    DevBuf<uint2> d_desc;
    DevBuf<double> d_E, d_E2;
    nlek::SortedRows sr{};
    if (sorted) {
        d_scol.alloc(nlek::sorted_scol_elems(ss.gs.W, nrows_local));
        d_first.alloc((size_t)nrows_local * 258);
        d_desc.alloc((size_t)nrows_local * nlek::kSortedThreads);
        d_E.alloc((size_t)ss.gs.W + 1);
        PROFILED(c, NLE_K_SMALL, nlek::dist_table(c->stream, ss.gs.W, hx, d_E.p));
        PROFILED(c, NLE_K_SMALL, nlek::sort_rows(c->stream, d_lum, ss.gs, row0, nrows_local, d_scol.p, d_desc.p, d_first.p));
        HIP_OK(hipMemsetAsync(d_cbuf.p, 0, d_cbuf.n * sizeof(double), c->stream));
        sr = nlek::SortedRows{d_scol.p, d_desc.p, d_first.p, d_E.p, false, 0.0};
        sr.rec = nlek::sorted_recurrence(ss.gs, hx, &sr.kappa);
        sr.mom = nlek::sorted_moments_ok(ss.gs, hx);
        if (std::getenv("NLE_ALL_LEVEL_TILES") == nullptr) {
            int t0 = 0, t1 = 16;
            while (t0 < 15 && !((ss.level_tiles >> t0) & 1u)) ++t0;
            while (t1 > t0 + 1 && !((ss.level_tiles >> (t1 - 1)) & 1u)) --t1;
            sr.lev_t0 = t0;
            sr.lev_nt = t1 - t0;
        }
        if (nlek::sorted_gsum_ok(ss.gs, hx)) {
            d_E2.alloc((size_t)ss.gs.W + 1);
            PROFILED(c, NLE_K_SMALL, nlek::dist_table(c->stream, ss.gs.W, hx / std::sqrt(2.0), d_E2.p));
            sr.E2 = d_E2.p;
            sr.hx = hx;
        }
    }
    const nlek::SortedRows* srp = sorted ? &sr : nullptr;
    tr.mark("ss: alloc+upload");
    auto pass_pixels = [&](int mode, bool last) {
        double* ybuf = last ? d_cbuf.p : nullptr;
        if (hist) {
            static const int kmap[4] = {NLE_K_SINK_TABLES, NLE_K_SINKHORN_PASS, NLE_K_REDUCE, NLE_K_REDUCE};
            ProfObserver obs(c, kmap);
            HIP_OK(nlek::sink_hist_tiled(c->stream, mode, d_lum, ss.gs, p, P64, row0, nrows_local, d_er.p, d_ecT.p,
                                         d_Ep.p, sk.d_w.p, NLE_EPS, ybuf, d_hws.p, d_z.p, &obs, nullptr, nullptr, srp));
        } else if (M > 0) {
            PROFILED(c, NLE_K_SINKHORN_PASS, nlek::sink_pass(c->stream, mode, d_lum, ss.gs, d_samples.p, p, sk.d_w.p, nsw,
                                                             npw, pix0, M, NLE_EPS, ybuf, d_partial.p));
            PROFILED(c, NLE_K_REDUCE, nlek::reduce_partials(c->stream, d_partial.p, npart, P64, d_z.p, kZS));
        } else {
            HIP_OK(hipMemsetAsync(d_z.p, 0, (size_t)kZS * P64 * sizeof(double), c->stream));
        }
    };
    const Nystrom ny = sk.run(solve, pass_pixels, d_z.p, hist ? 1 : kZS);
    f->r = ny.r;
    f->chol_ka = ny.chol ? 1 : 0;
    f->formulation = hist ? NLE_MODE_PHI_FREE : NLE_MODE_PHI_FREE_EXP;
    tm_s.stop();
    tr.mark("ss: passes enqueued");
    HIP_OK(hipStreamSynchronize(c->stream));
    tr.mark("ss: sinkhorn sync");

    tm_g.start();
    const int ntiles = nlek::gram64_num_tiles(p);
    const size_t g_elems = hist ? (size_t)p * p : (size_t)ntiles * 256;
    DevBuf<double> d_gpart, d_tiles(g_elems);
    auto enqueue_gram = [&] {
        if (M <= 0) {
            HIP_OK(hipMemsetAsync(d_tiles.p, 0, g_elems * sizeof(double), c->stream));
        } else if (hist) {
            d_gpart.alloc(nlek::ghist_workspace_elems(ss.gs, nrows_local));
            static const int gmap[4] = {NLE_K_GRAM_ROWS, NLE_K_SMALL, NLE_K_GRAM_GEMM, NLE_K_SMALL};
            ProfObserver obs(c, gmap);
            HIP_OK(nlek::gram_hist(c->stream, d_lum, ss.gs, p, row0, nrows_local, d_er.p, d_ecT.p, d_Ep.p, d_cbuf.p,
                                   d_gpart.p, d_tiles.p, &obs, srp));
        } else {
            d_gpart.alloc(std::max<size_t>(nlek::gram64_partial_elems(M, p), 1));
            PROFILED(c, NLE_K_GRAM, nlek::gram64(c->stream, d_lum, ss.gs, d_samples.p, p, nsw, npw, pix0, M, d_cbuf.p,
                                                 d_gpart.p, d_tiles.p));
        }
    };
    OrthoSS o;
    if (hist && c->topk_solver == 0) {
        ortho_ss_device(c, o, ny, p, sk.sA_c, sk.sA_r, d_tiles.p, n_eig, enqueue_gram,
                        [&] { all_reduce(c, d_tiles.p, g_elems); }, &ms->host, &ms->host_overlapped, tr);
        tm_g.stop();
    } else {
        enqueue_gram();
        double h0 = now_ms();
        ortho_ss_prepare(o, ny, p, sk.sA_c, sk.sA_r, c->topk_solver != 0);
        const double h_overlapped = now_ms() - h0;
        tr.mark("ss: ortho prepare (host)");
        all_reduce(c, d_tiles.p, g_elems);
        std::vector<double> tiles(g_elems);
        HIP_OK(hipMemcpyAsync(tiles.data(), d_tiles.p, tiles.size() * sizeof(double), hipMemcpyDeviceToHost, c->stream));
        tm_g.stop();
        HIP_OK(hipStreamSynchronize(c->stream));
        tr.mark("ss: gram sync");
        h0 = now_ms();
        ortho_ss_finish(o, hist ? std::move(tiles) : unpack_tiles(tiles, nlek::gram64_ld(p), p, 16), n_eig, c->topk_solver);
        ms->host += now_ms() - h0;
        tr.mark("ss: ortho finish (host)");
        ms->host_overlapped += h_overlapped;
    }
    adopt_ortho(f, o);

    tm_p.start();
    if (o.K > 128) throw Fail{NLE_ERR_INVALID, "Phi-free path supports at most 128 eigenvectors"};
    const int ldd = nlek::project64_ld(o.K);
    std::vector<double> Dp((size_t)p * ldd, 0.0);
    for (int k = 0; k < o.K; ++k)
        for (int a = 0; a < p; ++a) Dp[(size_t)a * ldd + k] = o.D[(size_t)k * p + a];
    DevBuf<double> d_D(Dp.size());
    HIP_OK(hipMemcpyAsync(d_D.p, Dp.data(), Dp.size() * sizeof(double), hipMemcpyHostToDevice, c->stream));
    if (hist) {
        auto own = [&](auto& buf) {
            using T = std::remove_pointer_t<decltype(buf.p)>;
            const size_t bytes = buf.n * sizeof(T);
            T* ptr = buf.take();
            f->owned.emplace_back(ptr, bytes);
            return ptr;
        };
        std::vector<double> Vr((size_t)p * ldd, 0.0);
        for (int k = 0; k < o.K; ++k)
            for (int a = 0; a < p; ++a) Vr[(size_t)a * ldd + k] = o.Vrows[(size_t)k * p + a];
        DevBuf<double> d_Vr(Vr.size());
        DevBuf<long long> d_spix(p), d_sloc(p);
        DevBuf<float> d_slab((size_t)M);
        std::vector<long long> sloc(p);
        for (int a = 0; a < p; ++a) {
            const long long loc = ss.pix[a] - pix0;
            sloc[a] = (loc >= 0 && loc < M) ? loc : -1;
        }
        HIP_OK(hipMemcpyAsync(d_Vr.p, Vr.data(), Vr.size() * sizeof(double), hipMemcpyHostToDevice, c->stream));
        HIP_OK(hipMemcpyAsync(d_spix.p, ss.pix.data(), p * sizeof(long long), hipMemcpyHostToDevice, c->stream));
        HIP_OK(hipMemcpyAsync(d_sloc.p, sloc.data(), p * sizeof(long long), hipMemcpyHostToDevice, c->stream));
        HIP_OK(hipMemcpyAsync(d_slab.p, d_lum + pix0, (size_t)M * sizeof(float), hipMemcpyDeviceToDevice, c->stream));
        HIP_OK(hipStreamSynchronize(c->stream));
        f->lazy = true;
        f->gs = ss.gs;
        f->nsw = nsw;
        f->npw = npw;
        f->ldd = ldd;
        f->P64 = P64;
        f->d_lum = own(d_slab);
        f->d_c = own(d_cbuf);
        f->d_er = own(d_er);
        f->d_ecT = own(d_ecT);
        f->d_Ep = own(d_Ep);
        f->d_D = own(d_D);
        f->d_Vrows = own(d_Vr);
        f->d_samples = own(d_samples);
        f->d_sample_pix = own(d_spix);
        f->d_sample_loc = own(d_sloc);
        if (sorted) {
            f->has_sorted = true;
            f->sorted = nlek::SortedRows{own(d_scol), own(d_desc), own(d_first), own(d_E), sr.rec, sr.kappa};
            f->sorted.lev_t0 = sr.lev_t0;
            f->sorted.lev_nt = sr.lev_nt;
            f->sorted.mom = sr.mom;
        }
        f->h_Vrows = o.Vrows;
        f->h_sample_pix = ss.pix;
        tm_p.stop();
        ms->take(tm_s, tm_g, tm_p);
        return;
    }
    DevBuf<float> d_V((size_t)std::max<long long>(M, 1) * f->ldv);
    PROFILED(c, NLE_K_PROJECT, nlek::project64(c->stream, d_lum, ss.gs, d_samples.p, p, nsw, npw, pix0, M, d_D.p, o.K,
                                               d_cbuf.p, d_V.p, f->ldv));
    tr.mark("ss: project enqueued");
    scatter_sample_rows(c, ss.pix, p, o.Vrows, o.K, f->ldv, pix0, M, d_V.p);
    tm_p.stop();
    HIP_OK(hipStreamSynchronize(c->stream));
    tr.mark("ss: project sync");
    f->v_bytes = d_V.n * sizeof(float);
    f->d_V = d_V.take();
    ms->take(tm_s, tm_g, tm_p);
}

void train_stream64(nle_ctx* c, nle_filter* f, const float* d_lum, const SampleSet& ss, const std::function<Nystrom()>& solve,
                    double hx, double hy, int T, int n_eig, long long pix0, long long M, StageMs* ms) {
    const int p = ss.p, ld = ld4(p);
    hipStream_t st = c->stream;
    Trace tr;
    Timer tm_s(st), tm_g(st), tm_p(st);
    tm_s.start();
    size_t budget_mb = 2048;
    if (const char* e = std::getenv("NLE_STREAM64_CHUNK_MB")) budget_mb = (size_t)std::max(1, std::atoi(e));
    const long long rows_fit = (long long)((budget_mb << 20) / ((size_t)ld * sizeof(double)));
    const long long CH = std::max<long long>(256, std::min<long long>(std::max<long long>(M, 1), rows_fit));
    DevBuf<float4> d_samples(p);
    HIP_OK(hipMemcpyAsync(d_samples.p, ss.packed.data(), p * sizeof(float4), hipMemcpyHostToDevice, st));
    PatchOperands po;
    upload_patch_operands(c, ss, &po);
    DevBuf<unsigned> d_smask;
    if (ss.listed) {
        const long long N = (long long)ss.gs.H * ss.gs.W;
        DevBuf<long long> d_spix(p);
        d_smask.alloc((size_t)((N + 31) / 32));
        HIP_OK(hipMemcpyAsync(d_spix.p, ss.pix.data(), p * sizeof(long long), hipMemcpyHostToDevice, st));
        PROFILED(c, NLE_K_SMALL, nlek::sample_mask(st, d_spix.p, p, N, d_smask.p));
        HIP_OK(hipStreamSynchronize(st));
    }
    DevBuf<double> d_K((size_t)CH * ld), d_partial((size_t)nlek::kRowpassMaxBlocks * ld), d_zc(ld), d_z(ld), d_ones(ld),
        d_cbuf((size_t)std::max<long long>(M, 1));
    SampleSinkhorn sk(c, p, ld, T);
    HIP_OK(nlek::fill64(st, d_ones.p, ld, 1.0));
    tr.mark("s64: alloc+upload");
    auto chunk_rows = [&](long long i0) { return std::min<long long>(CH, M - i0); };
    auto gen = [&](long long i0, long long mc) {
        PROFILED(c, NLE_K_AFFINITY, affinity_rows64(st, d_lum, ss, d_samples.p, po, ld, hx, hy, pix0 + i0, mc, d_K.p, true,
                                                    d_smask.p));
    };
    auto pass_pixels = [&](int mode, bool last) {
        HIP_OK(hipMemsetAsync(d_z.p, 0, ld * sizeof(double), st));
        for (long long i0 = 0; i0 < M; i0 += CH) {
            const long long mc = chunk_rows(i0);
            gen(i0, mc);
            int nb = 0;
            PROFILED(c, NLE_K_SINKHORN_PASS, nlek::rowpass64(st, mode, d_K.p, mc, ld, ld, sk.d_w.p, d_ones.p, nullptr, NLE_EPS, d_partial.p, &nb));
            PROFILED(c, NLE_K_REDUCE, nlek::reduce_partials(st, d_partial.p, nb, ld, d_zc.p));
            HIP_OK(nlek::add64(st, d_z.p, d_zc.p, ld));
            if (last) PROFILED(c, NLE_K_SMALL, nlek::row_scalings64(st, d_K.p, mc, ld, p, sk.d_w.p, NLE_EPS, d_cbuf.p + i0));
        }
    };
    const Nystrom ny = sk.run(solve, pass_pixels, d_z.p, 1);
    f->r = ny.r;
    f->chol_ka = ny.chol ? 1 : 0;
    f->formulation = NLE_MODE_STREAMED_F64;
    tm_s.stop();
    HIP_OK(hipStreamSynchronize(st));
    tr.mark("s64: sinkhorn");
    tm_g.start();
    const size_t pp = (size_t)p * p;
    DevBuf<double> d_G(pp), d_Gc(pp), d_gpart(std::max<size_t>(nlek::gram64d_partial_elems(CH, p), 1));
    auto enqueue_gram = [&] {
        HIP_OK(hipMemsetAsync(d_G.p, 0, pp * sizeof(double), st));
        for (long long i0 = 0; i0 < M; i0 += CH) {
            const long long mc = chunk_rows(i0);
            gen(i0, mc);
            PROFILED(c, NLE_K_GRAM, nlek::gram64d(st, d_K.p, mc, ld, p, d_cbuf.p + i0, d_gpart.p, d_Gc.p));
            HIP_OK(nlek::add64(st, d_G.p, d_Gc.p, pp));
        }
    };
    OrthoSS o;
    ortho_ss_device(c, o, ny, p, sk.sA_c, sk.sA_r, d_G.p, n_eig, enqueue_gram, [&] { all_reduce(c, d_G.p, pp); }, &ms->host,
                    &ms->host_overlapped, tr);
    tm_g.stop();
    adopt_ortho(f, o);
    tm_p.start();
    DevBuf<double> d_D((size_t)p * o.K), d_V((size_t)std::max<long long>(M, 1) * f->ldv);
    HIP_OK(hipMemcpyAsync(d_D.p, o.D.data(), o.D.size() * sizeof(double), hipMemcpyHostToDevice, st));
    HIP_OK(hipMemsetAsync(d_V.p, 0, d_V.n * sizeof(double), st));
    for (long long i0 = 0; i0 < M; i0 += CH) {
        const long long mc = chunk_rows(i0);
        gen(i0, mc);
        PROFILED(c, NLE_K_PROJECT, nlek::ts_gemm64(st, d_K.p, mc, ld, p, d_D.p, o.K, d_cbuf.p + i0, d_V.p + (size_t)i0 * f->ldv, f->ldv));
    }
    scatter_sample_rows(c, ss.pix, p, o.Vrows, o.K, f->ldv, pix0, M, d_V.p);
    tm_p.stop();
    HIP_OK(hipStreamSynchronize(st));
    tr.mark("s64: project");
    f->v64_bytes = d_V.n * sizeof(double);
    f->d_V64 = d_V.take();
    ms->take(tm_s, tm_g, tm_p);
}

void ensure_V(nle_filter* f) {
    if (f->d_V) return;
    nle_ctx* c = f->ctx;
    if (f->d_V64) {
        DevBuf<float> d_V((size_t)std::max<long long>(f->n_local, 1) * f->ldv);
        HIP_OK(nlek::to_f32(c->stream, f->d_V64, f->n_local * f->ldv, d_V.p));
        HIP_OK(hipStreamSynchronize(c->stream));
        f->v_bytes = d_V.n * sizeof(float);
        f->d_V = d_V.take();
        return;
    }
    if (!f->lazy) return;
    const long long M = f->n_local, pix0 = (long long)f->row0 * f->W;
    DevBuf<float> d_V((size_t)std::max<long long>(M, 1) * f->ldv);
    PROFILED(c, NLE_K_PROJECT, nlek::project64(c->stream, f->d_lum - pix0, f->gs, f->d_samples, f->p, f->nsw, f->npw, pix0,
                                               M, f->d_D, f->K, f->d_c, d_V.p, f->ldv));
    scatter_sample_rows(c, f->h_sample_pix, f->p, f->h_Vrows, f->K, f->ldv, pix0, M, d_V.p);
    HIP_OK(hipStreamSynchronize(c->stream));
    f->v_bytes = d_V.n * sizeof(float);
    f->d_V = d_V.take();
}

using LayersDone = std::function<void(int, int)>;
void apply_sample_space(nle_filter* f, const float* d_x, const double* h_g , int L, float* d_y,
                        const LayersDone& done = nullptr, int group = 0, bool round8 = false) {
    nle_ctx* c = f->ctx;
    const long long M = f->n_local, pix0 = (long long)f->row0 * f->W;
    const int p = f->p, K = f->K, P64 = f->P64, nrows_local = (int)(M / f->W);
    const float* lum = f->d_lum - pix0;
    DevBuf<double> d_ws(std::max<size_t>(nlek::hist_tiled_workspace_elems(f->gs, std::max(nrows_local, 1)), 1)), d_m(P64),
        d_resp((size_t)L * K), d_t(K), d_Wp((size_t)L * P64), d_YA((size_t)L * p);
    HIP_OK(hipMemcpyAsync(d_resp.p, h_g, (size_t)L * K * sizeof(double), hipMemcpyHostToDevice, c->stream));
    if (M > 0) {
        static const int rmap[4] = {NLE_K_SINK_TABLES, NLE_K_APPLY_REDUCE, NLE_K_REDUCE, NLE_K_REDUCE};
        ProfObserver obs(c, rmap);
        HIP_OK(nlek::sink_hist_tiled(c->stream, nlek::ROWPASS_XVEC, lum, f->gs, p, P64, f->row0, nrows_local, f->d_er,
                                     f->d_ecT, f->d_Ep, nullptr, NLE_EPS, nullptr, d_ws.p, d_m.p, &obs, f->d_c, d_x,
                                     f->has_sorted ? &f->sorted : nullptr));
    } else {
        HIP_OK(hipMemsetAsync(d_m.p, 0, P64 * sizeof(double), c->stream));
    }
    all_reduce(c, d_m.p, P64);
    DevBuf<double> d_xA(p);
    {
        const bool slabs = c->slab_input && c->world > 1;
        PROFILED(c, NLE_K_SMALL, nlek::gather_samples_slab(c->stream, d_x, f->gs, slabs ? f->row0 : 0, slabs ? f->row1 : f->H, d_xA.p));
        if (slabs) all_reduce(c, d_xA.p, p);
    }
    PROFILED(c, NLE_K_SMALL, nlek::apply_small(c->stream, p, K, f->ldd, L, P64, d_m.p, f->d_D, f->d_Vrows, d_xA.p,
// ... 289 lines not shown
            std::vector<double> TS((size_t)m * nk, 0.0);
            nleh::gemm_nn_cols(Tmm.data(), S.data(), TS.data(), m, m, nk, 0, nk);
            std::vector<double> Tk((size_t)nk * nk, 0.0);
            nleh::gemm_tn_cols(S.data(), TS.data(), Tk.data(), m, nk, nk, 0, nk);
            std::fill(Tm.begin(), Tm.end(), 0.0);
            for (int j = 0; j < nk; ++j)
                for (int i = 0; i < nk; ++i) Tm[(size_t)j * ldq + i] = Tk[(size_t)j * nk + i];
            sv.ms_host += now_ms() - h0;
            m = nk;
            qn = nk + b;
            HIP_OK(hipStreamSynchronize(st));
        }
    }
    tr.mark("exact eigensolver");
    if (tr.on)
        std::fprintf(stderr, "[nle trace] exact: N %lld, %lld block products of up to %d columns (x2), %d restarts\n", N,
                     sv.products, b, restarts);
    int Kp = 0;
    while (Kp < std::min(nev, nk) && theta[Kp] >= NLE_EPS) ++Kp;
    if (Kp == 0) throw Fail{NLE_ERR_NUMERIC, "exact filter: no eigenvalue >= 1e-10"};
    const int ldv = ld4(Kp);
    DevBuf<double> d_V((size_t)N * ldv);
    HIP_OK(nlek::exact_axpby(st, V.p, ldt, 1.0, nullptr, 0, 0.0, d_V.p, ldv, N, Kp, ldv));
    const int nb = nlek::exact_col_blocks(N);
    DevBuf<double> d_pv((size_t)nb * Kp), d_s(Kp);
    HIP_OK(nlek::exact_colmaxabs(st, d_V.p, ldv, N, Kp, d_pv.p));
    std::vector<double> pv((size_t)nb * Kp), sgn(Kp, 1.0);
    HIP_OK(hipMemcpyAsync(pv.data(), d_pv.p, pv.size() * sizeof(double), hipMemcpyDeviceToHost, st));
    HIP_OK(hipStreamSynchronize(st));
    for (int k = 0; k < Kp; ++k) {
        double best = 0.0;
        for (int blk = 0; blk < nb; ++blk)
            if (std::fabs(pv[(size_t)blk * Kp + k]) > std::fabs(best)) best = pv[(size_t)blk * Kp + k];
        sgn[k] = best < 0.0 ? -1.0 : 1.0;
    }
    HIP_OK(hipMemcpyAsync(d_s.p, sgn.data(), Kp * sizeof(double), hipMemcpyHostToDevice, st));
    HIP_OK(nlek::exact_scale_cols(st, d_V.p, ldv, N, Kp, d_s.p));
    HIP_OK(hipStreamSynchronize(st));
    f->K = Kp;
    f->ldv = ldv;
    f->eigvals.assign(theta.begin(), theta.begin() + Kp);
    f->formulation = NLE_MODE_EXACT_F64;
    f->p = f->r = 0;
    f->r_wa = 0;
    f->r_q = Kp;
    f->v64_bytes = d_V.n * sizeof(double);
    f->d_V64 = d_V.take();
    f->ms[0] = 0.0;
    f->ms[2] = sv.ms_prod;
    f->ms[4] = sv.ms_host;
    f->ms[3] = std::max(0.0, now_ms() - t_solve - sv.ms_prod - sv.ms_host);
}

nle_filter* train_exact_impl(nle_ctx* c, const float* d_lum, int H, int W, double hx, double hy, int T, int n_eig) {
    check_exact(c, H, W, n_eig);
    HIP_OK(hipSetDevice(c->device));
    auto f = new nle_filter();
    try {
        f->ctx = c;
        f->H = H;
        f->W = W;
        f->row0 = 0;
        f->row1 = H;
        f->n_local = (long long)H * W;
        const double t_begin = now_ms();
        pinned_reset(c);
        Trace tr;
        train_exact64(c, f, d_lum, H, W, hx, hy, T, n_eig, tr);
        prof_flush(c);
        f->ms[5] = now_ms() - t_begin;
        c->filters.insert(f);
    } catch (...) {
        if (f->d_V64) arena_release(c, f->d_V64, f->v64_bytes);
        delete f;
        throw;
    }
    return f;
}

nle_filter* train_impl(nle_ctx* c, const float* d_lum_in, int H, int W, int nRow, int nCol, double hx,
                       double hy, int T, int n_eig) {
    const GridSpec gs = checked_grid(H, W, nRow, nCol);
    const float* d_lum = d_lum_in;
    if (c->slab_input && c->world > 1) {
        int r0, r1;
        slab(H, c->rank, c->world, &r0, &r1);
        d_lum = d_lum_in - (size_t)r0 * W;
    }
    if (T < 1) throw Fail{NLE_ERR_INVALID, "nSinkhornIter must be >= 1"};
    if (n_eig < 1) throw Fail{NLE_ERR_INVALID, "nEigenVectors must be >= 1"};
    if (!(hx > 0) || !(hy > 0)) throw Fail{NLE_ERR_INVALID, "hx and hy must be > 0"};
    if (c->mode == NLE_MODE_EXACT_F64) return train_exact_impl(c, d_lum_in, H, W, hx, hy, T, n_eig);
    if (gs.p() > 2048) throw Fail{NLE_ERR_INVALID, "more than 2048 samples is not supported"};
    if (c->world > H) throw Fail{NLE_ERR_INVALID, "more ranks than image rows"};
    const bool generic_ok = gs.p() <= nlek::sink_pass_max_p() && n_eig <= 128;
    const bool tables_ok =
        n_eig <= 128 && gs.nSelCols <= nlek::ghist_max_cols() && gs.nSelRows <= 32 && c->mode != NLE_MODE_PHI_FREE_EXP;
    if (c->mode == NLE_MODE_PHI_FREE_EXP && !generic_ok)
        throw Fail{NLE_ERR_INVALID, "Phi-free path without tables supports at most 256 samples and 128 eigenvectors"};
    if (c->mode == NLE_MODE_PHI_FREE && !generic_ok && !tables_ok)
        throw Fail{NLE_ERR_INVALID, "Phi-free path supports at most 128 eigenvectors and a 32 x 36 sample grid"};
    const int R = c->patch_radius;
    if (R > 0 && c->mode != NLE_MODE_AUTO && c->mode != NLE_MODE_MATERIALISED_F64 && c->mode != NLE_MODE_STREAMED_F64)
        throw Fail{NLE_ERR_INVALID, "patch affinities (patch radius > 0) run in NLE_MODE_AUTO, NLE_MODE_MATERIALISED_F64 or "
                                    "NLE_MODE_STREAMED_F64 only"};
    check_patch_radius(c, R, H, W);
    const bool chroma = c->chroma_a != nullptr;
    if (chroma && c->mode != NLE_MODE_AUTO && c->mode != NLE_MODE_MATERIALISED_F64 && c->mode != NLE_MODE_STREAMED_F64)
        throw Fail{NLE_ERR_INVALID, "chroma affinities (nle_ctx_set_chroma) run in NLE_MODE_AUTO, NLE_MODE_MATERIALISED_F64 or "
                                    "NLE_MODE_STREAMED_F64 only"};
    check_chroma(c, R, gs.p());
    const bool farthest = c->sampler == NLE_SAMPLER_FARTHEST;
    if (farthest && c->mode != NLE_MODE_AUTO && c->mode != NLE_MODE_MATERIALISED_F64 && c->mode != NLE_MODE_STREAMED_F64)
        throw Fail{NLE_ERR_INVALID, "the farthest sampler runs in NLE_MODE_AUTO, NLE_MODE_MATERIALISED_F64 or "
                                    "NLE_MODE_STREAMED_F64 only"};
    check_sampler(c, hx, hy);
    const bool want_fuse = R == 0 && !farthest && !chroma && (c->mode == NLE_MODE_PHI_FREE || c->mode == NLE_MODE_PHI_FREE_EXP ||
                                      (c->mode == NLE_MODE_AUTO && tables_ok));
    HIP_OK(hipSetDevice(c->device));

    auto f = new nle_filter();
    try {
        f->ctx = c;
        f->H = H;
        f->W = W;
        slab(H, c->rank, c->world, &f->row0, &f->row1);
        const long long pix0 = (long long)f->row0 * W;
        const long long M = (long long)(f->row1 - f->row0) * W;
        f->n_local = M;
        const double t_begin = now_ms();
        pinned_reset(c);
        Trace tr;
        StageMs sm;
        Timer tm_a(c->stream);
        tm_a.start();
        std::vector<long long> list;
        if (farthest) list = farthest_list(c, d_lum, gs, hx, hy);
        SampleSet ss = fetch_samples(c, d_lum, gs, (want_fuse && tables_ok) || R > 0 || chroma, c->slab_input && c->world > 1,
                                     R, farthest ? &list : nullptr, chroma);
        if (R > 0 && ranks_where(c, !ss.quantised) > 0)
            throw Fail{NLE_ERR_INVALID, "patch affinities (patch radius > 0) need an integer-valued luminance plane in [0, 255] "
                                        "(the L channel of 8-bit Lab)"};
        if (chroma && ranks_where(c, !ss.quantised || !ss.chroma_quantised) > 0)
            throw Fail{NLE_ERR_INVALID, "chroma affinities need integer-valued L, a and b planes in [0, 255] (the channels of "
                                        "8-bit Lab)"};
        f->chroma_hc = chroma ? ss.hc : 0.0;
        const bool fuse = c->mode == NLE_MODE_AUTO ? (want_fuse && tables_ok && ss.quantised)
                                                   : (want_fuse && (generic_ok || (tables_ok && ss.quantised)));
        if (c->mode == NLE_MODE_PHI_FREE && !fuse)
            throw Fail{NLE_ERR_INVALID, "Phi-free path: more than 256 samples needs an integer-valued luminance plane"};
        tr.mark("fetch_samples");
        f->p = ss.p;
        f->h_sample_pix = ss.pix;
        double h0 = now_ms();
        std::vector<double> Ka = build_Ka(ss, hx, hy);
        tr.mark("build_Ka");
        sm.host += now_ms() - h0;
        auto solve = [&](bool allow_chol) {
            const double t0 = now_ms();
            Nystrom ny = solve_Ka(c, Ka, ss.p, allow_chol);
            tr.mark(ny.chol ? "chol(Ka)" : "eig(Ka)");
            sm.host += now_ms() - t0;
            return ny;
        };
        tm_a.stop();
        bool stream64 = c->mode == NLE_MODE_STREAMED_F64;
        if (!fuse && c->mode == NLE_MODE_AUTO) {
            size_t free_b = 0, total_b = 0;
            const size_t need = (size_t)std::max<long long>(M, 1) * ld4(ss.p) * sizeof(double);
            if (hipMemGetInfo(&free_b, &total_b) == hipSuccess && need > (free_b + c->arena_bytes) / 2) stream64 = true;
            if (std::getenv("NLE_AUTO_STREAM64")) stream64 = true;
            if (c->world > 1) stream64 = ranks_where(c, stream64) > 0;
        }
        if (fuse) {
            train_sample_space(c, f, d_lum, ss, [&] { return solve(true); }, hx, hy, T, n_eig, pix0, M, &sm);
        } else if (stream64) {
            train_stream64(c, f, d_lum, ss, [&] { return solve(true); }, hx, hy, T, n_eig, pix0, M, &sm);
        } else {
            const Nystrom ny = solve(false);
            f->r = ny.r;
            if (c->mode == NLE_MODE_MATERIALISED)
                train_materialised(c, f, d_lum, ss, ny, hx, hy, T, n_eig, pix0, M, &sm);
            else
                train_generic64(c, f, d_lum, ss, ny, hx, hy, T, n_eig, pix0, M, &sm);
        }
        tr.mark("train path");
        prof_flush(c);
        f->ms[0] = tm_a.ms();
        f->ms[1] = sm.sinkhorn;
        f->ms[2] = sm.gram;
        f->ms[3] = sm.project;
        f->ms[4] = sm.host;
        f->ms[5] = now_ms() - t_begin;
        c->filters.insert(f);
    } catch (...) {
        delete f;
        throw;
    }
    return f;
}

void apply_impl(nle_filter* f, const float* d_x_in, int H, int W, const double* h_g , int L,
                float* d_y, const LayersDone& done = nullptr, int group = 0, bool round8 = false) {
    nle_ctx* c = f->ctx;
    const float* d_x = (c->slab_input && c->world > 1) ? d_x_in - (size_t)f->row0 * f->W : d_x_in;
    if ((long long)H * W != (long long)f->H * f->W)
        throw Fail{NLE_ERR_INVALID, "Number of values in channel must match that of training image."};
    if (L < 1 || L > 64) throw Fail{NLE_ERR_INVALID, "number of layers must be in [1, 64]"};
    HIP_OK(hipSetDevice(c->device));
    if (f->lazy) {
        apply_sample_space(f, d_x, h_g, L, d_y, done, group, round8);
        return;
    }
    if (!f->d_V64) ensure_V(f);
    const int ld = f->ldv;
    const long long M = f->n_local;
    const long long pix0 = (long long)f->row0 * f->W;
    DevBuf<double> d_partial((size_t)nlek::kRowpassMaxBlocks * ld), d_t(ld), d_resp((size_t)L * ld),
        d_g((size_t)L * ld);
    std::vector<double> resp((size_t)L * ld, 0.0);
    for (int l = 0; l < L; ++l)
        for (int k = 0; k < f->K; ++k) resp[(size_t)l * ld + k] = h_g[(size_t)l * f->K + k];
    HIP_OK(hipMemcpyAsync(d_resp.p, resp.data(), resp.size() * sizeof(double), hipMemcpyHostToDevice, c->stream));
    int nb = 0;
    if (f->d_V64)
        PROFILED(c, NLE_K_APPLY_REDUCE, nlek::rowpass64(c->stream, nlek::ROWPASS_XVEC, f->d_V64, M, ld, ld, nullptr, nullptr,
                                                        d_x + pix0, NLE_EPS, d_partial.p, &nb));
    else
    PROFILED(c, NLE_K_APPLY_REDUCE, nlek::rowpass(c->stream, nlek::ROWPASS_XVEC, f->d_V, M, ld, nullptr, nullptr,
                                                  d_x + pix0, NLE_EPS, d_partial.p, &nb));
    PROFILED(c, NLE_K_REDUCE, nlek::reduce_partials(c->stream, d_partial.p, nb, ld, d_t.p));
    all_reduce(c, d_t.p, ld);
    for (int l = 0; l < L; ++l)
        PROFILED(c, NLE_K_SMALL, nlek::scale_vec(c->stream, d_resp.p + (size_t)l * ld, d_t.p, ld, d_g.p + (size_t)l * ld));
    if (f->d_V64)
        PROFILED(c, NLE_K_APPLY_EXPAND, nlek::apply_expand64(c->stream, f->d_V64, M, ld, f->K, d_g.p, L, d_y, M));
    else
    PROFILED(c, NLE_K_APPLY_EXPAND, nlek::apply_expand(c->stream, f->d_V, M, ld, d_g.p, L, d_y, M));
    if (done) done(0, L);
    HIP_OK(hipStreamSynchronize(c->stream));
    prof_flush(c);
}

void layer_resp(const double* ev, int K, int L, double* out) {
    for (int j = 0; j < L; ++j)
        for (int k = 0; k < K; ++k) {
            const double a = std::pow(ev[k], (double)j);
            out[(size_t)j * K + k] = (j < L - 1) ? a - std::pow(ev[k], (double)(j + 1)) : a;
        }
}

}

extern "C" {

int nle_layer_responses(const double* h_eigvals, int K, int L, double* h_resp) {
    if (!h_eigvals || !h_resp || K < 0 || L < 1) return NLE_ERR_INVALID;
    layer_resp(h_eigvals, K, L, h_resp);
    return NLE_OK;
}

int nle_compute_kernel(nle_ctx* ctx, const float* d_lum, int H, int W, int n_row_samples, int n_col_samples,
                       double hx, double hy, double* h_Ka, float* d_kab) {
    if (!ctx || !d_lum) return NLE_ERR_INVALID;
    return guard(ctx, [&] {
        const GridSpec gs = checked_grid(H, W, n_row_samples, n_col_samples);
        if (ctx->patch_radius > 0)
            throw Fail{NLE_ERR_INVALID, "nle_compute_kernel (fp32) does not take patch affinities: use nle_compute_kernel64"};
        if (ctx->chroma_a)
            throw Fail{NLE_ERR_INVALID, "nle_compute_kernel (fp32) does not take chroma affinities: use nle_compute_kernel64"};
        if (ctx->sampler != NLE_SAMPLER_GRID)
            throw Fail{NLE_ERR_INVALID, "nle_compute_kernel (fp32) takes the grid sampler only: use nle_compute_kernel64"};
        HIP_OK(hipSetDevice(ctx->device));
        SampleSet ss = fetch_samples(ctx, d_lum, gs);
        if (h_Ka) {
            std::vector<double> Ka = build_Ka(ss, hx, hy);
            std::copy(Ka.begin(), Ka.end(), h_Ka);
        }
        if (d_kab) {
            int row0, row1;
            slab(H, ctx->rank, ctx->world, &row0, &row1);
            DevBuf<float4> d_samples(ss.p);
            HIP_OK(hipMemcpyAsync(d_samples.p, ss.packed.data(), ss.p * sizeof(float4), hipMemcpyHostToDevice, ctx->stream));
            PROFILED(ctx, NLE_K_AFFINITY,
                     nlek::affinity(ctx->stream, d_lum, gs, d_samples.p, ss.p, ld4(ss.p), nsw_of(hx), nsw_of(hy),
                                    (long long)row0 * W, (long long)(row1 - row0) * W, d_kab));
            HIP_OK(hipStreamSynchronize(ctx->stream));
            prof_flush(ctx);
        }
    });
}

int nle_nystrom(nle_ctx* ctx, const float* d_lum, int H, int W, int n_row_samples, int n_col_samples, double hx,
                double hy, double* h_eigvals, int* r, float* d_phi) {
    if (!ctx || !d_lum || !d_phi || !r) return NLE_ERR_INVALID;
    return guard(ctx, [&] {
        const GridSpec gs = checked_grid(H, W, n_row_samples, n_col_samples);
        if (ctx->patch_radius > 0)
            throw Fail{NLE_ERR_INVALID, "nle_nystrom (fp32) does not take patch affinities: use the fp64 formulations"};
        if (ctx->chroma_a)
            throw Fail{NLE_ERR_INVALID, "nle_nystrom (fp32) does not take chroma affinities: use the fp64 formulations"};
        if (ctx->sampler != NLE_SAMPLER_GRID)
            throw Fail{NLE_ERR_INVALID, "nle_nystrom (fp32) takes the grid sampler only: use the fp64 formulations"};
        HIP_OK(hipSetDevice(ctx->device));
        SampleSet ss = fetch_samples(ctx, d_lum, gs);
        std::vector<double> Ka = build_Ka(ss, hx, hy);
        Nystrom ny = solve_Ka(nullptr, Ka, ss.p, false);
        int row0, row1;
        slab(H, ctx->rank, ctx->world, &row0, &row1);
        build_phi(ctx, d_lum, ss, ny, hx, hy, (long long)row0 * W, (long long)(row1 - row0) * W, d_phi);
        *r = ny.r;
        if (h_eigvals) std::copy(ny.lam.begin(), ny.lam.end(), h_eigvals);
// ... 564 lines not shown
```

nonlocal-image-edit_amd/csrc/pipeline_internal.h:

```cpp
#pragma once
#include <hip/hip_runtime.h>
#include <dlfcn.h>
#include <rccl/rccl.h>

#include <algorithm>
#include <atomic>
#include <mutex>
#include <functional>
#include <chrono>
#include <cmath>
#include <cstdio>
#include <cstdlib>
#include <cstring>
#include <map>
#include <memory>
#include <set>
#include <string>
#include <thread>
#include <type_traits>
#include <vector>

#include "../../include/nle.h"
#include "eigen_sym.h"
#include "kernels.h"

using nlek::GridSpec;

struct nle_ctx {
    int device = 0;
    hipStream_t stream = nullptr;
    bool own_stream = false;
    int rank = 0, world = 1;
    nle_allreduce_fn allreduce = nullptr;
    void* ar_user = nullptr;
    ncclComm_t comm = nullptr;
    bool own_comm = false;
    std::atomic<int> comm_aborted{0};
    std::mutex comm_mu;
    double* d_comm = nullptr;
    size_t comm_len = 0;
    std::string err;
    std::multimap<size_t, void*> arena_free;
    size_t arena_bytes = 0;
    double* d_lut = nullptr;
    std::set<nle_filter*> filters;
    hipEvent_t aux_ev = nullptr;
    void* h_stage = nullptr;
    size_t h_stage_bytes = 0, h_stage_used = 0, h_stage_want = 0;
    hipStream_t aux_stream = nullptr;
    hipStream_t copy_stream = nullptr;
    hipEvent_t copy_ev[2] = {nullptr, nullptr};
    int mode = 0;
    bool slab_input = false;
    bool nystrom_bf16x3 = false;
    int patch_radius = 0;
    const float* chroma_a = nullptr;
    const float* chroma_b = nullptr;
    double chroma_hc = 0.0;
    int sampler = 0;
    int topk_solver = 0;
    bool profiling = false;
    bool profile_all = false;
    struct ProfRec {
        int kid;
        hipEvent_t a, b;
    };
    std::vector<ProfRec> prof_pending;
    std::vector<hipEvent_t> prof_pool;
    long long prof_launches[NLE_KERNEL_COUNT] = {0};
    double prof_ms[NLE_KERNEL_COUNT] = {0};
};

struct nle_filter {
    nle_ctx* ctx = nullptr;
    int H = 0, W = 0, row0 = 0, row1 = 0;
    long long n_local = 0;
    int K = 0, ldv = 0, r = 0, p = 0;
    float* d_V = nullptr;
    size_t v_bytes = 0;
    double* d_V64 = nullptr;
    size_t v64_bytes = 0;
    std::vector<double> eigvals;
    double chroma_hc = 0.0;
    double ms[6] = {0, 0, 0, 0, 0, 0};
    int formulation = 0, r_wa = 0, r_q = 0, chol_ka = 0, chol_wa = 0;
    bool lazy = false;
    nlek::GridSpec gs{};
    float nsw = 0.f, npw = 0.f;
    int ldd = 0, P64 = 0;
    float* d_plane = nullptr;
    size_t plane_bytes = 0;
    float* d_lum = nullptr;
    double *d_c = nullptr, *d_er = nullptr, *d_ecT = nullptr, *d_Ep = nullptr, *d_D = nullptr, *d_Vrows = nullptr;
    float4* d_samples = nullptr;
    long long *d_sample_pix = nullptr, *d_sample_loc = nullptr;
    bool has_sorted = false;
    nlek::SortedRows sorted{};
    std::vector<std::pair<void*, size_t>> owned;
    std::vector<double> h_Vrows;
    std::vector<long long> h_sample_pix;
};


namespace nlep {

struct Fail {
    int code;
    std::string msg;
};

#define HIP_OK(expr)                                                                              \
    do {                                                                                          \
        hipError_t e_ = (expr);                                                                   \
        if (e_ != hipSuccess)                                                                     \
            throw Fail{NLE_ERR_HIP, std::string(#expr) + ": " + hipGetErrorString(e_)};           \
    } while (0)

inline thread_local nle_ctx* g_cur = nullptr;
struct CurCtx {
    nle_ctx* prev;
    explicit CurCtx(nle_ctx* c) : prev(g_cur) { g_cur = c; }
    ~CurCtx() { g_cur = prev; }
};

inline void* arena_alloc(nle_ctx* c, size_t bytes) {
    if (c) {
        auto it = c->arena_free.lower_bound(bytes);
        if (it != c->arena_free.end() && it->first <= bytes + bytes / 4 + 4096) {
            void* p = it->second;
            c->arena_free.erase(it);
            return p;
        }
    }
    void* p = nullptr;
    hipError_t e = hipMalloc(&p, bytes);
    if (e != hipSuccess && c && !c->arena_free.empty()) {
        (void)hipStreamSynchronize(c->stream);
        for (auto& kv : c->arena_free) (void)hipFree(kv.second);
        c->arena_free.clear();
        c->arena_bytes = 0;
        e = hipMalloc(&p, bytes);
    }
    if (e != hipSuccess) throw Fail{NLE_ERR_HIP, std::string("hipMalloc: ") + hipGetErrorString(e)};
    if (c) c->arena_bytes += bytes;
    return p;
}

inline void arena_release(nle_ctx* c, void* p, size_t bytes) {
    if (!p) return;
    if (c) {
        c->arena_free.emplace(bytes, p);
    } else {
        (void)hipFree(p);
    }
}

template <typename T>
struct DevBuf {
    T* p = nullptr;
    size_t n = 0;
    nle_ctx* owner = nullptr;
    DevBuf() = default;
    explicit DevBuf(size_t count) { alloc(count); }
    DevBuf(const DevBuf&) = delete;
    DevBuf& operator=(const DevBuf&) = delete;
    void alloc(size_t count) {
        release();
        if (count) {
            owner = g_cur;
            p = static_cast<T*>(arena_alloc(owner, count * sizeof(T)));
        }
        n = count;
    }
    void release() {
        if (p) arena_release(owner, p, n * sizeof(T));
        p = nullptr;
        n = 0;
    }
    T* take() {
        T* q = p;
        p = nullptr;
        n = 0;
        return q;
    }
    ~DevBuf() { release(); }
};

struct Timer {
    hipEvent_t a = nullptr, b = nullptr;
    hipStream_t s;
    explicit Timer(hipStream_t st) : s(st) {
        HIP_OK(hipEventCreate(&a));
        HIP_OK(hipEventCreate(&b));
    }
    ~Timer() {
        if (a) (void)hipEventDestroy(a);
        if (b) (void)hipEventDestroy(b);
    }
    void start() { HIP_OK(hipEventRecord(a, s)); }
    void stop() { HIP_OK(hipEventRecord(b, s)); }
    double ms() {
        HIP_OK(hipEventSynchronize(b));
        float t = 0.f;
        HIP_OK(hipEventElapsedTime(&t, a, b));
        return t;
    }
};

inline int ld4(int n) { return (n + 3) & ~3; }

constexpr double kLog2e = 1.4426950408889634074;
inline float nsw_of(double h) { return (float)(-kLog2e / (h * h)); }

inline hipEvent_t prof_event(nle_ctx* c) {
    if (!c->prof_pool.empty()) {
        hipEvent_t e = c->prof_pool.back();
        c->prof_pool.pop_back();
        return e;
    }
    hipEvent_t e = nullptr;
    HIP_OK(hipEventCreate(&e));
    return e;
}

struct Prof {
    nle_ctx* c;
    int kid;
    hipEvent_t a = nullptr, b = nullptr;
    Prof(nle_ctx* c_, int kid_) : c(c_), kid(kid_) {
        if (!c->profiling) return;
        if (!c->profile_all && (kid == NLE_K_SMALL || kid == NLE_K_REDUCE || kid == NLE_K_SINK_TABLES)) return;
        a = prof_event(c);
        b = prof_event(c);
        HIP_OK(hipEventRecord(a, c->stream));
    }
    void end() {
        if (!a) return;
        HIP_OK(hipEventRecord(b, c->stream));
        c->prof_pending.push_back({kid, a, b});
        a = nullptr;
    }
};

#define PROFILED(ctx_, kid_, expr)  \
    do {                            \
        Prof pf_((ctx_), (kid_));   \
        HIP_OK(expr);               \
        pf_.end();                  \
    } while (0)

struct ProfObserver : nlek::LaunchObserver {
    nle_ctx* c;
    const int* map;
    Prof* cur = nullptr;
    ProfObserver(nle_ctx* c_, const int* map_) : c(c_), map(map_) {}
    void begin(int sub) override { cur = new Prof(c, map[sub]); }
    void end() override {
        if (cur) {
            cur->end();
            delete cur;
            cur = nullptr;
        }
    }
    ~ProfObserver() override { end(); }
};

inline void prof_flush(nle_ctx* c) {
    for (auto& r : c->prof_pending) {
        float t = 0.f;
        if (hipEventElapsedTime(&t, r.a, r.b) == hipSuccess) {
            c->prof_ms[r.kid] += t;
            c->prof_launches[r.kid] += 1;
        }
        c->prof_pool.push_back(r.a);
        c->prof_pool.push_back(r.b);
    }
    c->prof_pending.clear();
}

inline bool make_grid(int H, int W, int nRow, int nCol, GridSpec* gs) {
    if (H <= 0 || W <= 0 || nRow <= 0 || nCol <= 0 || nRow > H || nCol > W) return false;
    gs->H = H;
    gs->W = W;
    gs->rowStep = H / nRow;
    gs->colStep = W / nCol;
    gs->rowOff = (gs->rowStep - 1 + (H - gs->rowStep * nRow)) / 2;
    gs->colOff = (gs->colStep - 1 + (W - gs->colStep * nCol)) / 2;
    auto count = [](int n, int off, int step) {
        const int hi = std::min(n - 1, n - off);
        if (hi < off) return 0;
        return (hi - off) / step + 1;
    };
    gs->nSelRows = count(H, gs->rowOff, gs->rowStep);
    gs->nSelCols = count(W, gs->colOff, gs->colStep);
    return gs->nSelRows > 0 && gs->nSelCols > 0;
}

inline void slab(int H, int rank, int world, int* row0, int* row1) {
    *row0 = (int)(((long long)rank * H) / world);
    *row1 = (int)(((long long)(rank + 1) * H) / world);
}

inline double recip0(double v, double eps = NLE_EPS) { return std::fabs(v) >= eps ? 1.0 / v : 0.0; }

inline void check_image_size(int H, int W) {
    if (H <= 0 || W <= 0) throw Fail{NLE_ERR_INVALID, "image must be non-empty"};
    if ((long long)H * W >= (1ll << 31)) throw Fail{NLE_ERR_INVALID, "image too large (H*W must be < 2^31)"};
}

struct RcclApi {
    void* lib = nullptr;
    ncclResult_t (*GetUniqueId)(ncclUniqueId*) = nullptr;
    ncclResult_t (*CommInitRank)(ncclComm_t*, int, ncclUniqueId, int) = nullptr;
    ncclResult_t (*CommDestroy)(ncclComm_t) = nullptr;
    ncclResult_t (*CommAbort)(ncclComm_t) = nullptr;
    ncclResult_t (*AllReduce)(const void*, void*, size_t, ncclDataType_t, ncclRedOp_t, ncclComm_t, hipStream_t) = nullptr;
    const char* (*GetErrorString)(ncclResult_t) = nullptr;
};
inline RcclApi& rccl() {
    static RcclApi api = [] {
        RcclApi a;
        for (const char* name : {"librccl.so.1", "librccl.so", "/opt/rocm/lib/librccl.so.1"}) {
            a.lib = dlopen(name, RTLD_NOW | RTLD_GLOBAL);
            if (a.lib) break;
        }
        if (!a.lib) throw Fail{NLE_ERR_COMM, std::string("cannot load librccl.so: ") + dlerror()};
        auto sym = [&](const char* n) {
            void* p = dlsym(a.lib, n);
            if (!p) throw Fail{NLE_ERR_COMM, std::string("librccl.so lacks ") + n};
            return p;
        };
        a.GetUniqueId = reinterpret_cast<decltype(a.GetUniqueId)>(sym("ncclGetUniqueId"));
        a.CommInitRank = reinterpret_cast<decltype(a.CommInitRank)>(sym("ncclCommInitRank"));
        a.CommDestroy = reinterpret_cast<decltype(a.CommDestroy)>(sym("ncclCommDestroy"));
        a.CommAbort = reinterpret_cast<decltype(a.CommAbort)>(sym("ncclCommAbort"));
        a.AllReduce = reinterpret_cast<decltype(a.AllReduce)>(sym("ncclAllReduce"));
        a.GetErrorString = reinterpret_cast<decltype(a.GetErrorString)>(sym("ncclGetErrorString"));
        return a;
    }();
    return api;
}
#define RCCL_OK(expr)                                                                                           \
    do {                                                                                                        \
        ncclResult_t r_ = (expr);                                                                               \
        if (r_ != ncclSuccess) throw Fail{NLE_ERR_COMM, std::string(#expr) + ": " + rccl().GetErrorString(r_)}; \
    } while (0)

inline void all_reduce(nle_ctx* c, double* d, size_t n) {
    if (c->comm_aborted.load(std::memory_order_acquire))
        throw Fail{NLE_ERR_COMM, "the communicator of this ctx was aborted (another rank failed)"};
    if (c->comm) {
        std::lock_guard<std::mutex> lk(c->comm_mu);
        if (c->comm_aborted.load(std::memory_order_acquire))
            throw Fail{NLE_ERR_COMM, "the communicator of this ctx was aborted (another rank failed)"};
        RCCL_OK(rccl().AllReduce(d, d, n, ncclDouble, ncclSum, c->comm, c->stream));
        return;
    }
    if (c->world <= 1) return;
    if (!c->allreduce || !c->d_comm || c->comm_len < n)
        throw Fail{NLE_ERR_COMM, "world > 1 but no all-reduce callback / comm buffer too small"};
    HIP_OK(hipMemcpyAsync(c->d_comm, d, n * sizeof(double), hipMemcpyDeviceToDevice, c->stream));
    if (c->allreduce(c->ar_user, c->d_comm, n) != 0) throw Fail{NLE_ERR_COMM, "all-reduce callback failed"};
    HIP_OK(hipMemcpyAsync(d, c->d_comm, n * sizeof(double), hipMemcpyDeviceToDevice, c->stream));
}

inline int ranks_where(nle_ctx* c, bool flag) {
    if (c->world <= 1 && !c->comm) return flag ? 1 : 0;
    DevBuf<double> d(1);
    double v = flag ? 1.0 : 0.0;
    HIP_OK(hipMemcpyAsync(d.p, &v, sizeof v, hipMemcpyHostToDevice, c->stream));
    all_reduce(c, d.p, 1);
    HIP_OK(hipMemcpyAsync(&v, d.p, sizeof v, hipMemcpyDeviceToHost, c->stream));
    HIP_OK(hipStreamSynchronize(c->stream));
    return (int)(v + 0.5);
}

inline void pinned_reset(nle_ctx* c) {
    if (c->h_stage_want > c->h_stage_bytes) {
        if (c->h_stage) (void)hipHostFree(c->h_stage);
        c->h_stage = nullptr;
        c->h_stage_bytes = 0;
        const size_t want = c->h_stage_want + c->h_stage_want / 4;
        if (hipHostMalloc(&c->h_stage, want, hipHostMallocDefault) == hipSuccess) c->h_stage_bytes = want;
        else c->h_stage = nullptr;
    }
    c->h_stage_used = 0;
    c->h_stage_want = 0;
}
inline void* pinned_take(nle_ctx* c, size_t bytes) {
    bytes = (bytes + 255) & ~(size_t)255;
    c->h_stage_want += bytes;
    if (!c->h_stage || c->h_stage_used + bytes > c->h_stage_bytes) return nullptr;
    void* p = static_cast<char*>(c->h_stage) + c->h_stage_used;
    c->h_stage_used += bytes;
    return p;
}
inline void upload_staged(nle_ctx* c, double* d_dst, const double* h_src, size_t n, hipStream_t st) {
    if (void* hp = pinned_take(c, n * sizeof(double))) {
        std::memcpy(hp, h_src, n * sizeof(double));
        h_src = static_cast<const double*>(hp);
    }
    HIP_OK(hipMemcpyAsync(d_dst, h_src, n * sizeof(double), hipMemcpyHostToDevice, st));
}

inline double now_ms() {
    using namespace std::chrono;
    return duration<double, std::milli>(steady_clock::now().time_since_epoch()).count();
}
struct Trace {
    bool on;
    double t0, last;
    Trace() : on(std::getenv("NLE_TRACE") != nullptr) { t0 = last = now_ms(); }
    void mark(const char* what) {
        if (!on) return;
        const double t = now_ms();
        std::fprintf(stderr, "[nle trace] %-28s +%8.3f ms  (t=%8.3f)\n", what, t - last, t - t0);
        last = t;
    }
};

inline thread_local std::string g_create_err;

template <typename Fn>
int guard(nle_ctx* c, Fn&& fn) {
    CurCtx scope(c);
    try {
        fn();
        return NLE_OK;
    } catch (const Fail& e) {
        if (c) c->err = e.msg; else g_create_err = e.msg;
        return e.code;
    } catch (const std::exception& e) {
        if (c) c->err = e.what(); else g_create_err = e.what();
        return NLE_ERR_INVALID;
    }
}

}
```

Before: 3303 MP/s.

## Keep phi-free coefficient rows on device and trim host staging and syncs

Packs the D and Vrows coefficient matrices on the device with a new pack kernel instead of downloading them, transposing on the host and uploading again. Host-to-device copies now go through the pinned staging buffer, and the L^T L and -G G^T products are enqueued early so they overlap host work. The host transpose and matrix-vector loops are blocked for better cache use, and the sample-pixel and luminance-slab uploads move earlier to drop a stream sync. Together these aim to shorten host-side and PCIe latency in the small-matrix phase, but they add more code paths and lean on the pinned-buffer capacity being large enough.

Result: faster. 3445 MP/s (median of 6 runs) (+4.3%).

```diff
diff --git a/nonlocal-image-edit_amd/csrc/generic64.hip b/nonlocal-image-edit_amd/csrc/generic64.hip
--- a/nonlocal-image-edit_amd/csrc/generic64.hip
+++ b/nonlocal-image-edit_amd/csrc/generic64.hip
@@ -451,6 +451,30 @@
     return hipGetLastError();
 }
 
+__global__ void k_pack_rows64(const double* __restrict__ src0, int ld0, const double* __restrict__ dl0, double* __restrict__ dst0,
+                              const double* __restrict__ src1, int ld1, double* __restrict__ dst1, int p, int K, int ldd) {
+    const int f = blockIdx.x * blockDim.x + threadIdx.x;
+    if (f >= p * ldd) return;
+    const int a = f / ldd, k = f - a * ldd;
+    if (blockIdx.y == 0) {
+        double v = 0.0;
+        if (k < K) {
+            v = src0[(size_t)k * ld0 + a];
+            if (dl0) v *= dl0[a];
+        }
+        dst0[f] = v;
+    } else {
+        dst1[f] = k < K ? src1[(size_t)k * ld1 + a] : 0.0;
+    }
+}
+hipError_t pack_rows64(hipStream_t s, const double* d_src0, int ld0, const double* d_dl0, double* d_dst0, const double* d_src1,
+                       int ld1, double* d_dst1, int p, int K, int ldd) {
+    if (p <= 0 || ldd <= 0) return hipSuccess;
+    hipLaunchKernelGGL(k_pack_rows64, dim3((unsigned)((p * ldd + 255) / 256), 2), dim3(256), 0, s, d_src0, ld0, d_dl0, d_dst0,
+                       d_src1, ld1, d_dst1, p, K, ldd);
+    return hipGetLastError();
+}
+
 __global__ void k_to_f32(const double* __restrict__ X, long long n, float* __restrict__ out) {
     for (long long i = (long long)blockIdx.x * blockDim.x + threadIdx.x; i < n; i += (long long)gridDim.x * blockDim.x)
         out[i] = (float)X[i];
diff --git a/nonlocal-image-edit_amd/csrc/kernels.h b/nonlocal-image-edit_amd/csrc/kernels.h
--- a/nonlocal-image-edit_amd/csrc/kernels.h
+++ b/nonlocal-image-edit_amd/csrc/kernels.h
@@ -152,6 +152,8 @@
 hipError_t scatter_rows64(hipStream_t s, const double* d_src, const long long* d_idx, int n, int ld, double* d_X, long long M);
 hipError_t to_f32(hipStream_t s, const double* d_X, long long n, float* d_out);
 hipError_t scale_rows64(hipStream_t s, double* d_X, int m, int n, const double* d_dl);
+hipError_t pack_rows64(hipStream_t s, const double* d_src0, int ld0, const double* d_dl0, double* d_dst0, const double* d_src1,
+                       int ld1, double* d_dst1, int p, int K, int ldd);
 
 int tridiag_max_n();
 hipError_t tridiag(hipStream_t s, int n, const double* d_Q, const double* d_diag_add, double* d_V, double* d_d, double* d_e,
diff --git a/nonlocal-image-edit_amd/csrc/ortho.h b/nonlocal-image-edit_amd/csrc/ortho.h
--- a/nonlocal-image-edit_amd/csrc/ortho.h
+++ b/nonlocal-image-edit_amd/csrc/ortho.h
@@ -17,6 +17,7 @@
     std::vector<double> VA;
     std::vector<double> lam;
     std::vector<double> B;
+    std::vector<double> Linv;
     std::vector<double> Ka;
 };
 
@@ -32,6 +33,7 @@
     std::vector<double> Sq, D, Vrows;
     int p = 0, r = 0;
     std::vector<double> cA, rA, Kr, P, Wa, S, St, A2;
+    const double* Kr_ref = nullptr;
 };
 
 Ortho orthogonalize_host(const Nystrom& ny, int p, const std::vector<double>& u_c, const std::vector<double>& u_r,
@@ -39,8 +41,14 @@
 void ortho_ss_prepare(OrthoSS& o, const Nystrom& ny, int p, const std::vector<double>& sA_c, const std::vector<double>& sA_r,
                       bool literal_q = false);
 void ortho_ss_finish(OrthoSS& o, std::vector<double> Gk, int n_eig, int topk_solver = 0);
+struct PackedRows {
+    int ldd = 0;
+    DevBuf<double> D, Vrows;
+    std::function<void()> before_sync;
+};
 void ortho_ss_device(nle_ctx* c, OrthoSS& o, const Nystrom& ny, int p, const std::vector<double>& sA_c,
                      const std::vector<double>& sA_r, double* d_Gk, int n_eig, const std::function<void()>& enqueue_gram,
-                     const std::function<void()>& reduce_gram, double* host_ms, double* host_overlapped_ms, Trace& tr);
+                     const std::function<void()>& reduce_gram, double* host_ms, double* host_overlapped_ms, Trace& tr,
+                     PackedRows* packed = nullptr);
 
 }
diff --git a/nonlocal-image-edit_amd/csrc/ortho.hip b/nonlocal-image-edit_amd/csrc/ortho.hip
--- a/nonlocal-image-edit_amd/csrc/ortho.hip
+++ b/nonlocal-image-edit_amd/csrc/ortho.hip
@@ -24,14 +24,14 @@
     par_cols(n, (long long)m * k, [&](int j0, int j1) { nleh::gemm_tn_cols(A, B, C, m, k, n, j0, j1); });
 }
 
-void top_eigenpairs(const std::vector<double>& Qm, int q, int n_eig, int solver, std::vector<double>* Vq,
+void top_eigenpairs(const double* Qm, int q, int n_eig, int solver, std::vector<double>* Vq,
                     std::vector<double>* Sq, int* rq) {
     if (solver == 1 && q > 1) {
         const int nev = std::min(std::max(n_eig, 1), q - 1);
         Vq->assign((size_t)q * nev, 0.0);
         Sq->assign(nev, 0.0);
         int restarts = 0;
-        const int nconv = nleh::lanczos_topk(Qm.data(), q, nev, NLE_EPS, 1000, Vq->data(), Sq->data(), &restarts);
+        const int nconv = nleh::lanczos_topk(Qm, q, nev, NLE_EPS, 1000, Vq->data(), Sq->data(), &restarts);
         if (nconv < 0) throw Fail{NLE_ERR_NUMERIC, "Lanczos: the projected eigenproblem did not converge"};
         if (nconv < nev)
             std::fprintf(stderr, "# converged eigenvalues: %d\nEigen decomposition NOT successful. Results might be inaccurate.\n", nconv);
@@ -43,7 +43,7 @@
     }
     Vq->assign((size_t)q * std::min(q, std::max(n_eig, 1)), 0.0);
     Sq->assign(q, 0.0);
-    if (!nleh::eigen_decomposition_topk(Qm.data(), q, NLE_EPS, n_eig, Vq->data(), Sq->data(), rq))
+    if (!nleh::eigen_decomposition_topk(Qm, q, NLE_EPS, n_eig, Vq->data(), Sq->data(), rq))
         throw Fail{NLE_ERR_NUMERIC, "eigensolver did not converge on Q"};
 }
 
@@ -98,9 +98,10 @@
 
 void build_Wa(OrthoSS& o) {
     const int p = o.p, q = o.q;
+    const double* Kr = o.Kr_ref ? o.Kr_ref : o.Kr.data();
     o.Wa.resize((size_t)q * q);
     for (int b = 0; b < q; ++b)
-        for (int a = 0; a < q; ++a) o.Wa[(size_t)b * q + a] = o.rA[a] * o.Kr[(size_t)b * p + a] * o.cA[b];
+        for (int a = 0; a < q; ++a) o.Wa[(size_t)b * q + a] = o.rA[a] * Kr[(size_t)b * p + a] * o.cA[b];
 }
 
 }
@@ -159,7 +160,7 @@
         mm_tn(Us.data(), WF.data(), Qt.data(), q, r2, r2);
         for (int k = 0; k < r2; ++k) Qt[(size_t)k * r2 + k] += l2[k];
         std::vector<double> Vt;
-        top_eigenpairs(Qt, r2, n_eig, topk_solver, &Vt, &Sq, &rq);
+        top_eigenpairs(Qt.data(), r2, n_eig, topk_solver, &Vt, &Sq, &rq);
         K = std::min(n_eig, rq);
         if (K <= 0) throw Fail{NLE_ERR_NUMERIC, "Q has no eigenvalue >= 1e-10"};
         T2.resize((size_t)q * K);
@@ -170,7 +171,7 @@
         mm(S.data(), WW.data(), T1.data(), q, q, q);
         mm(T1.data(), S.data(), Qm.data(), q, q, q);
         for (size_t i = 0; i < Qm.size(); ++i) Qm[i] += o.Wa[i];
-        top_eigenpairs(Qm, q, n_eig, topk_solver, &Vq, &Sq, &rq);
+        top_eigenpairs(Qm.data(), q, n_eig, topk_solver, &Vq, &Sq, &rq);
         K = std::min(n_eig, rq);
         if (K <= 0) throw Fail{NLE_ERR_NUMERIC, "Q has no eigenvalue >= 1e-10"};
         T2.resize((size_t)q * K);
@@ -258,7 +259,7 @@
     for (size_t i = 0; i < Qm.size(); ++i) Qm[i] += o.A2[i];
     std::vector<double> Vq, Sq;
     int rq = 0;
-    top_eigenpairs(Qm, q, n_eig, topk_solver, &Vq, &Sq, &rq);
+    top_eigenpairs(Qm.data(), q, n_eig, topk_solver, &Vq, &Sq, &rq);
     const int K = std::min(n_eig, rq);
     if (K <= 0) throw Fail{NLE_ERR_NUMERIC, "Q has no eigenvalue >= 1e-10"};
     o.K = K;
@@ -299,17 +300,18 @@
     DevBuf<double> rA, cA, Kr, P, VA, lam;
 };
 
-void scalings_Kr_P(hipStream_t st, OrthoSS& o, const Nystrom& ny, int p, const std::vector<double>& sA_c,
+void scalings_Kr_P(nle_ctx* c, OrthoSS& o, const Nystrom& ny, int p, const std::vector<double>& sA_c,
                    const std::vector<double>& sA_r, SsDevice& dv) {
+    hipStream_t st = c->stream;
     const int r = ny.r;
     const size_t pp = (size_t)p * p;
     sample_scalings(o, ny, p, sA_c, sA_r);
     dv.rA.alloc(p);
     dv.cA.alloc(p);
-    HIP_OK(hipMemcpyAsync(dv.rA.p, o.rA.data(), p * sizeof(double), hipMemcpyHostToDevice, st));
-    HIP_OK(hipMemcpyAsync(dv.cA.p, o.cA.data(), p * sizeof(double), hipMemcpyHostToDevice, st));
+    upload_staged(c, dv.rA.p, o.rA.data(), p, st);
+    upload_staged(c, dv.cA.p, o.cA.data(), p, st);
     if (ny.chol) {
-        o.Kr = ny.Ka;
+        o.Kr_ref = ny.Ka.data();
         return;
     }
     dv.VA.alloc((size_t)p * r);
@@ -334,8 +336,21 @@
     int r_wa = 0, nd = 0;
     std::vector<double> F, L, G, l2_kept;
     DevBuf<double> d_F, d_L, d_G;
+    DevBuf<double> d_A2, d_neg;
+    bool uploaded = false;
+    bool pageable = false;
     bool chol_form() const { return form != kEigen; }
 };
+
+void enqueue_LtL(hipStream_t st, int q, WaRoot& w) {
+    w.d_A2.alloc((size_t)q * q);
+    HIP_OK(nlek::gemm64s(st, q, q, q, w.d_L.p, q, 1, w.d_L.p, 1, q, w.d_A2.p, 1, q));
+}
+void enqueue_minus_GGt(hipStream_t st, int q, WaRoot& w) {
+    w.d_neg.alloc(w.nd);
+    HIP_OK(nlek::fill64(st, w.d_neg.p, w.nd, -1.0));
+    HIP_OK(nlek::gemm64s(st, q, q, w.nd, w.d_G.p, 1, q, w.d_G.p, q, 1, w.d_A2.p, 1, q, nullptr, w.d_neg.p, nullptr, w.d_A2.p, 1, q));
+}
 
 struct WaDeviceWork {
     DevSymEig es;
@@ -415,7 +430,8 @@
     HIP_OK(hipStreamWaitEvent(st, c->aux_ev, 0));
 }
 
-void wa_root_host(OrthoSS& o, bool cholesky_forms, bool force_eig, WaRoot& w, Trace& tr) {
+void wa_root_host(nle_ctx* c, OrthoSS& o, bool cholesky_forms, bool force_eig, WaRoot& w, Trace& tr) {
+    hipStream_t st = c->stream;
     const int q = o.q, max_defl = q / 8;
     const size_t qq = (size_t)q * q;
     if (o.Wa.empty()) build_Wa(o);
@@ -458,22 +474,32 @@
         }
     }
     if (factored) {
+        w.d_L.alloc(qq);
+        w.pageable |= !upload_staged(c, w.d_L.p, L.data(), qq, st);
+        enqueue_LtL(st, q, w);
         std::vector<double>& F = w.F;
         F.resize(qq);
-        for (int k = 0; k < q; ++k)
-            for (int a = 0; a < q; ++a) F[(size_t)k * q + a] = Li[(size_t)a * q + k];
+        constexpr int kTb = 16;
+        for (int k0 = 0; k0 < q; k0 += kTb)
+            for (int a0 = 0; a0 < q; a0 += kTb)
+                for (int k = k0; k < std::min(q, k0 + kTb); ++k)
+                    for (int a = a0; a < std::min(q, a0 + kTb); ++a) F[(size_t)k * q + a] = Li[(size_t)a * q + k];
         w.G.assign((size_t)q * std::max(nd, 1), 0.0);
         std::vector<double> wv(q);
         for (int t = 0; t < nd; ++t) {
             const double* v = Vd.data() + (size_t)t * q;
-            for (int k = 0; k < q; ++k) {
-                double acc = 0.0, g = 0.0;
-                for (int a = 0; a < q; ++a) {
-                    acc += v[a] * Li[(size_t)a * q + k];
-                    g += L[(size_t)k * q + a] * v[a];
-                }
-                wv[k] = acc;
-                w.G[(size_t)t * q + k] = g;
+            std::fill(wv.begin(), wv.end(), 0.0);
+            for (int a = 0; a < q; ++a) {
+                const double va = v[a];
+                const double* lia = Li.data() + (size_t)a * q;
+                for (int k = 0; k < q; ++k) wv[k] += va * lia[k];
+            }
+            for (int k0 = 0; k0 < q; k0 += 8) {
+                const int kn = std::min(8, q - k0);
+                double g[8] = {0.0, 0.0, 0.0, 0.0, 0.0, 0.0, 0.0, 0.0};
+                for (int a = 0; a < q; ++a)
+                    for (int j = 0; j < kn; ++j) g[j] += L[(size_t)(k0 + j) * q + a] * v[a];
+                for (int j = 0; j < kn; ++j) w.G[(size_t)t * q + k0 + j] = g[j];
             }
             for (int k = 0; k < q; ++k)
                 for (int a = 0; a < q; ++a) F[(size_t)k * q + a] -= v[a] * wv[k];
@@ -481,6 +507,14 @@
         w.form = nd > 0 ? WaRoot::kDeflated : WaRoot::kCholesky;
         w.r_wa = nd > 0 ? kept : q;
         w.nd = nd;
+        w.d_F.alloc(qq);
+        w.pageable |= !upload_staged(c, w.d_F.p, F.data(), qq, st);
+        if (nd > 0) {
+            w.d_G.alloc((size_t)q * nd);
+            w.pageable |= !upload_staged(c, w.d_G.p, w.G.data(), (size_t)q * nd, st);
+            enqueue_minus_GGt(st, q, w);
+        }
+        w.uploaded = true;
         return;
     }
     EigRoot e = eigen_root(o.Wa, q);
@@ -490,26 +524,24 @@
     w.F = std::move(e.Us);
 }
 
-void upload_host_root(hipStream_t st, int q, WaRoot& w) {
-    const size_t qq = (size_t)q * q;
-    if (w.chol_form()) {
-        w.d_L.alloc(qq);
-        HIP_OK(hipMemcpyAsync(w.d_L.p, w.L.data(), qq * sizeof(double), hipMemcpyHostToDevice, st));
-    }
-    w.d_F.alloc((size_t)q * w.m);
-    HIP_OK(hipMemcpyAsync(w.d_F.p, w.F.data(), (size_t)q * w.m * sizeof(double), hipMemcpyHostToDevice, st));
-    if (w.form == WaRoot::kDeflated) {
-        w.d_G.alloc((size_t)q * w.nd);
-        HIP_OK(hipMemcpyAsync(w.d_G.p, w.G.data(), (size_t)q * w.nd * sizeof(double), hipMemcpyHostToDevice, st));
-    }
-    HIP_OK(hipStreamSynchronize(st));
-}
-
-void form_Qt(hipStream_t st, const OrthoSS& o, const SsDevice& dv, const WaRoot& w, double* d_Gk,
+void upload_host_root(nle_ctx* c, int q, WaRoot& w) {
+    hipStream_t st = c->stream;
+    if (!w.uploaded) {
+        w.d_F.alloc((size_t)q * w.m);
+        w.pageable |= !upload_staged(c, w.d_F.p, w.F.data(), (size_t)q * w.m, st);
+        w.uploaded = true;
+    }
+    if (w.pageable) HIP_OK(hipStreamSynchronize(st));
+}
+
+void form_Qt(hipStream_t st, const OrthoSS& o, const SsDevice& dv, WaRoot& w, double* d_Gk,
              const std::function<void()>& reduce_gram, double* d_Qm) {
     const int p = o.p, r = o.r, q = o.q, m = w.m;
-    const size_t qq = (size_t)q * q;
     DevBuf<double> d_T((size_t)p * p), d_T1((size_t)m * q);
+    if (w.chol_form() && !w.d_A2.p) {
+        enqueue_LtL(st, q, w);
+        if (w.form == WaRoot::kDeflated) enqueue_minus_GGt(st, q, w);
+    }
     reduce_gram();
     if (q < p) {
         std::vector<double> c2(p - q);
@@ -529,14 +561,7 @@
         HIP_OK(nlek::gemm64s(st, m, m, q, d_T1.p, 1, m, w.d_F.p, 1, q, d_Qm, 1, m, nullptr, dv.rA.p));
         return;
     }
-    DevBuf<double> d_A2(qq);
-    HIP_OK(nlek::gemm64s(st, q, q, q, w.d_L.p, q, 1, w.d_L.p, 1, q, d_A2.p, 1, q));
-    if (w.form == WaRoot::kDeflated) {
-        DevBuf<double> d_neg(w.nd);
-        HIP_OK(nlek::fill64(st, d_neg.p, w.nd, -1.0));
-        HIP_OK(nlek::gemm64s(st, q, q, w.nd, w.d_G.p, 1, q, w.d_G.p, q, 1, d_A2.p, 1, q, nullptr, d_neg.p, nullptr, d_A2.p, 1, q));
-    }
-    HIP_OK(nlek::gemm64s(st, m, m, q, d_T1.p, 1, m, w.d_F.p, 1, q, d_Qm, 1, m, nullptr, dv.rA.p, nullptr, d_A2.p, 1, q));
+    HIP_OK(nlek::gemm64s(st, m, m, q, d_T1.p, 1, m, w.d_F.p, 1, q, d_Qm, 1, m, nullptr, dv.rA.p, nullptr, w.d_A2.p, 1, q));
 }
 
 struct QtEig {
@@ -575,8 +600,13 @@
             t.es.vectors(c, 0, Kd, t.d_Vq.p);
         }
     } else {
-        std::vector<double> Qm(mm_);
-        HIP_OK(hipMemcpyAsync(Qm.data(), d_Qm, mm_ * sizeof(double), hipMemcpyDeviceToHost, st));
+        std::vector<double> Qv;
+        double* Qm = static_cast<double*>(pinned_take(c, mm_ * sizeof(double)));
+        if (!Qm) {
+            Qv.resize(mm_);
+            Qm = Qv.data();
+        }
+        HIP_OK(hipMemcpyAsync(Qm, d_Qm, mm_ * sizeof(double), hipMemcpyDeviceToHost, st));
         HIP_OK(hipStreamSynchronize(st));
         tr.mark("ss: Q on the device + download");
         h0 = now_ms();
@@ -595,29 +625,49 @@
     tr.mark(t.on_device ? "ss: eigenvectors of Q (inverse iteration on the host, back-transformation enqueued)" : "ss: eig(Q) (host)");
 }
 
-void D_and_Vrows(hipStream_t st, OrthoSS& o, const SsDevice& dv, const WaRoot& w, QtEig& t, const double* d_Wa, Trace& tr) {
+void D_and_Vrows(nle_ctx* c, OrthoSS& o, const SsDevice& dv, const WaRoot& w, QtEig& t, const double* d_Wa, Trace& tr,
+                 PackedRows* packed) {
+    hipStream_t st = c->stream;
     const int p = o.p, r = o.r, q = o.q, m = w.m, K = o.K;
-    DevBuf<double> d_sv(K), d_T2((size_t)q * K), d_D((size_t)p * K), d_Vr((size_t)p * K);
+    const size_t pK = (size_t)p * K;
+    DevBuf<double> d_sv(K), d_T2((size_t)q * K), d_D, d_Vr(pK);
     if (!t.on_device) {
         t.d_Vq.alloc((size_t)m * K);
-        HIP_OK(hipMemcpyAsync(t.d_Vq.p, t.Vq.data(), (size_t)m * K * sizeof(double), hipMemcpyHostToDevice, st));
-    }
-    HIP_OK(hipMemcpyAsync(d_sv.p, t.sv.data(), K * sizeof(double), hipMemcpyHostToDevice, st));
+        upload_staged(c, t.d_Vq.p, t.Vq.data(), (size_t)m * K, st);
+    }
+    upload_staged(c, d_sv.p, t.sv.data(), K, st);
     HIP_OK(nlek::gemm64s(st, q, K, m, w.d_F.p, 1, q, t.d_Vq.p, 1, m, d_T2.p, 1, q, nullptr, nullptr, d_sv.p));
+    const bool scale_in_pack = packed && r == p;
     if (r < p) {
+        d_D.alloc(pK);
         HIP_OK(nlek::gemm64s(st, p, K, q, dv.P.p, 1, p, d_T2.p, 1, q, d_D.p, 1, p, nullptr, dv.rA.p));
-    } else {
+    } else if (!packed) {
+        d_D.alloc(pK);
         HIP_OK(hipMemcpyAsync(d_D.p, d_T2.p, (size_t)q * K * sizeof(double), hipMemcpyDeviceToDevice, st));
         HIP_OK(nlek::scale_rows64(st, d_D.p, p, K, dv.rA.p));
     }
     HIP_OK(nlek::gemm64s(st, q, K, q, d_Wa, 1, q, d_T2.p, 1, q, d_Vr.p, 1, p));
     if (q < p)
         HIP_OK(nlek::gemm64s(st, p - q, K, p, dv.Kr.p + q, 1, p, d_D.p, 1, p, d_Vr.p + q, 1, p, dv.cA.p + q));
-    o.D.resize((size_t)p * K);
-    o.Vrows.resize((size_t)p * K);
-    HIP_OK(hipMemcpyAsync(o.D.data(), d_D.p, o.D.size() * sizeof(double), hipMemcpyDeviceToHost, st));
-    HIP_OK(hipMemcpyAsync(o.Vrows.data(), d_Vr.p, o.Vrows.size() * sizeof(double), hipMemcpyDeviceToHost, st));
+    if (packed) {
+        packed->ldd = nlek::project64_ld(K);
+        packed->D.alloc((size_t)p * packed->ldd);
+        packed->Vrows.alloc((size_t)p * packed->ldd);
+        HIP_OK(nlek::pack_rows64(st, scale_in_pack ? d_T2.p : d_D.p, p, scale_in_pack ? dv.rA.p : nullptr, packed->D.p, d_Vr.p, p,
+                                 packed->Vrows.p, p, K, packed->ldd));
+    }
+    const size_t nback = packed ? pK : 2 * pK;
+    double* hb = static_cast<double*>(pinned_take(c, nback * sizeof(double)));
+    o.Vrows.resize(pK);
+    if (!packed) o.D.resize(pK);
+    HIP_OK(hipMemcpyAsync(hb ? hb : o.Vrows.data(), d_Vr.p, pK * sizeof(double), hipMemcpyDeviceToHost, st));
+    if (!packed) HIP_OK(hipMemcpyAsync(hb ? hb + pK : o.D.data(), d_D.p, pK * sizeof(double), hipMemcpyDeviceToHost, st));
+    if (packed && packed->before_sync) packed->before_sync();
     HIP_OK(hipStreamSynchronize(st));
+    if (hb) {
+        std::memcpy(o.Vrows.data(), hb, pK * sizeof(double));
+        if (!packed) std::memcpy(o.D.data(), hb + pK, pK * sizeof(double));
+    }
     tr.mark("ss: D, Vrows on the device");
 }
 
@@ -625,11 +675,12 @@
 
 void ortho_ss_device(nle_ctx* c, OrthoSS& o, const Nystrom& ny, int p, const std::vector<double>& sA_c,
                      const std::vector<double>& sA_r, double* d_Gk, int n_eig, const std::function<void()>& enqueue_gram,
-                     const std::function<void()>& reduce_gram, double* host_ms, double* host_overlapped_ms, Trace& tr) {
+                     const std::function<void()>& reduce_gram, double* host_ms, double* host_overlapped_ms, Trace& tr,
+                     PackedRows* packed) {
     const int q = ny.r;
     hipStream_t st = c->stream;
     SsDevice dv;
-    scalings_Kr_P(st, o, ny, p, sA_c, sA_r, dv);
+    scalings_Kr_P(c, o, ny, p, sA_c, sA_r, dv);
     const double h0 = now_ms();
     const bool dev_wa = use_dev_solver(q) && !std::getenv("NLE_HOST_WA");
     const bool force_eig = std::getenv("NLE_FORCE_EIG") != nullptr;
@@ -637,11 +688,13 @@
     DevBuf<double> d_Wa((size_t)q * q);
     WaRoot w;
     WaDeviceWork ws;
-    if (dev_wa)
+    if (dev_wa) {
         wa_root_device(c, o, ny, dv, d_Wa.p, force_eig, enqueue_gram, ws, w, tr);
-    else
+    } else {
         enqueue_gram();
-    if (!w.on_device) wa_root_host(o, !dev_wa, force_eig, w, tr);
+        if (!upload_staged(c, d_Wa.p, o.Wa.data(), (size_t)q * q, st)) w.pageable = true;
+    }
+    if (!w.on_device) wa_root_host(c, o, !dev_wa, force_eig, w, tr);
     o.r_wa = w.r_wa;
     o.chol_wa = w.form == WaRoot::kCholesky;
     *host_overlapped_ms += now_ms() - h0;
@@ -649,12 +702,11 @@
     w.m = w.chol_form() ? q : std::max(w.r_wa, 0);
     if (w.m <= 0) throw Fail{NLE_ERR_NUMERIC, "Wa has no eigenvalue >= 1e-10"};
     DevBuf<double> d_Qm((size_t)w.m * w.m);
-    if (!dev_wa) HIP_OK(hipMemcpyAsync(d_Wa.p, o.Wa.data(), (size_t)q * q * sizeof(double), hipMemcpyHostToDevice, st));
-    if (!w.on_device) upload_host_root(st, q, w);
+    if (!w.on_device) upload_host_root(c, q, w);
     form_Qt(st, o, dv, w, d_Gk, reduce_gram, d_Qm.p);
     QtEig t;
     top_eigenpairs_Qt(c, o, w, d_Qm.p, n_eig, t, host_ms, tr);
-    D_and_Vrows(st, o, dv, w, t, d_Wa.p, tr);
-}
-
-}
+    D_and_Vrows(c, o, dv, w, t, d_Wa.p, tr, packed);
+}
+
+}
diff --git a/nonlocal-image-edit_amd/csrc/pipeline.hip b/nonlocal-image-edit_amd/csrc/pipeline.hip
--- a/nonlocal-image-edit_amd/csrc/pipeline.hip
+++ b/nonlocal-image-edit_amd/csrc/pipeline.hip
@@ -365,9 +365,7 @@
                 n.ldr = ld4(p);
                 n.VA = std::move(L);
                 n.lam.assign(p, 1.0);
-                n.B.resize((size_t)p * p);
-                for (int k = 0; k < p; ++k)
-                    for (int a = 0; a < p; ++a) n.B[(size_t)k * p + a] = Li[(size_t)a * p + k];
+                n.Linv = std::move(Li);
                 n.Ka = Ka;
                 return n;
             }
@@ -684,37 +682,43 @@
 }
 
 void build_update_operands(nle_ctx* c, const Nystrom& ny, int p, DevBuf<double>& d_X1, DevBuf<double>& d_X2,
-                           DevBuf<double>& d_lam) {
+                           DevBuf<double>& d_lam, std::vector<double>& h_X1, std::vector<double>& h_X2) {
     const int r = ny.r;
-    if (ny.dev) {
+    if (ny.chol) {
         const size_t n2 = (size_t)2 * p, pp = (size_t)p * p;
         d_X1.alloc(n2 * p);
         d_X2.alloc(n2 * p);
         d_lam.alloc(p);
         HIP_OK(hipMemsetAsync(d_X1.p, 0, n2 * p * sizeof(double), c->stream));
-        HIP_OK(nlek::transpose64(c->stream, p, ny.dev->ch.Linv.p, d_X1.p, p, 2 * p));
-        HIP_OK(hipMemcpyAsync(d_X2.p, ny.dev->ch.Linv.p, pp * sizeof(double), hipMemcpyDeviceToDevice, c->stream));
-        HIP_OK(hipMemcpyAsync(d_X2.p + pp, ny.dev->Ka.p, pp * sizeof(double), hipMemcpyDeviceToDevice, c->stream));
+        if (ny.dev) {
+            HIP_OK(hipMemcpyAsync(d_X2.p, ny.dev->ch.Linv.p, pp * sizeof(double), hipMemcpyDeviceToDevice, c->stream));
+            HIP_OK(hipMemcpyAsync(d_X2.p + pp, ny.dev->Ka.p, pp * sizeof(double), hipMemcpyDeviceToDevice, c->stream));
+        } else {
+            upload_staged(c, d_X2.p, ny.Linv.data(), pp, c->stream);
+            upload_staged(c, d_X2.p + pp, ny.Ka.data(), pp, c->stream);
+        }
+        HIP_OK(nlek::transpose64(c->stream, p, d_X2.p, d_X1.p, p, 2 * p));
         HIP_OK(nlek::fill64(c->stream, d_lam.p, p, 1.0));
     } else {
         const size_t n2 = (size_t)2 * p;
-        std::vector<double> X1(n2 * r, 0.0), X2(n2 * r);
+        std::vector<double>&X1 = h_X1, &X2 = h_X2;
+        X1.resize(n2 * r);
+        X2.resize(n2 * r);
         for (int k = 0; k < r; ++k)
             for (int a = 0; a < p; ++a) {
                 const double b = ny.B[(size_t)k * p + a];
-                const double va = ny.chol ? ny.Ka[(size_t)k * p + a] : ny.VA[(size_t)k * p + a];
+                const double va = ny.VA[(size_t)k * p + a];
                 X1[(size_t)k * n2 + a] = b;
-                if (!ny.chol) X1[(size_t)k * n2 + p + a] = va;
+                X1[(size_t)k * n2 + p + a] = va;
                 X2[(size_t)a * r + k] = b;
                 X2[(size_t)(p + a) * r + k] = va;
             }
         d_X1.alloc(X1.size());
         d_X2.alloc(X2.size());
         d_lam.alloc(r);
-        HIP_OK(hipMemcpyAsync(d_X1.p, X1.data(), X1.size() * sizeof(double), hipMemcpyHostToDevice, c->stream));
-        HIP_OK(hipMemcpyAsync(d_X2.p, X2.data(), X2.size() * sizeof(double), hipMemcpyHostToDevice, c->stream));
-        HIP_OK(hipMemcpyAsync(d_lam.p, ny.lam.data(), r * sizeof(double), hipMemcpyHostToDevice, c->stream));
-        HIP_OK(hipStreamSynchronize(c->stream));
+        upload_staged(c, d_X1.p, X1.data(), X1.size(), c->stream);
+        upload_staged(c, d_X2.p, X2.data(), X2.size(), c->stream);
+        upload_staged(c, d_lam.p, ny.lam.data(), r, c->stream);
     }
 }
 
@@ -722,6 +726,7 @@
     nle_ctx* c;
     int p, T, zld;
     DevBuf<double> d_w, d_sAh, d_X1, d_X2, d_lam, d_uv;
+    std::vector<double> h_X1, h_X2;
     std::vector<double> sA_c, sA_r;
 
     SampleSinkhorn(nle_ctx* c_, int p_, int zld_, int T_)
@@ -733,7 +738,7 @@
                 int zrows) {
         pass_pixels(nlek::ROWPASS_COLSUM, false);
         Nystrom ny = solve();
-        build_update_operands(c, ny, p, d_X1, d_X2, d_lam);
+        build_update_operands(c, ny, p, d_X1, d_X2, d_lam, h_X1, h_X2);
         auto update = [&](int n, int mode) {
             all_reduce(c, d_z, (size_t)zrows * zld);
             PROFILED(c, NLE_K_SMALL,
@@ -818,6 +823,23 @@
         }
     }
     const nlek::SortedRows* srp = sorted ? &sr : nullptr;
+    DevBuf<long long> d_spix, d_sloc;
+    DevBuf<float> d_slab;
+    std::vector<long long> sloc;
+    bool pix_uploaded = false;
+    auto upload_sample_pixels = [&] {
+        d_spix.alloc(p);
+        d_sloc.alloc(p);
+        sloc.resize(p);
+        for (int a = 0; a < p; ++a) {
+            const long long loc = ss.pix[a] - pix0;
+            sloc[a] = (loc >= 0 && loc < M) ? loc : -1;
+        }
+        HIP_OK(hipMemcpyAsync(d_spix.p, ss.pix.data(), p * sizeof(long long), hipMemcpyHostToDevice, c->stream));
+        HIP_OK(hipMemcpyAsync(d_sloc.p, sloc.data(), p * sizeof(long long), hipMemcpyHostToDevice, c->stream));
+        pix_uploaded = true;
+    };
+    if (hist) d_slab.alloc((size_t)M);
     tr.mark("ss: alloc+upload");
     auto pass_pixels = [&](int mode, bool last) {
         double* ybuf = last ? d_cbuf.p : nullptr;
@@ -826,6 +848,10 @@
             ProfObserver obs(c, kmap);
             HIP_OK(nlek::sink_hist_tiled(c->stream, mode, d_lum, ss.gs, p, P64, row0, nrows_local, d_er.p, d_ecT.p,
                                          d_Ep.p, sk.d_w.p, NLE_EPS, ybuf, d_hws.p, d_z.p, &obs, nullptr, nullptr, srp));
+            if (mode == nlek::ROWPASS_COLSUM)
+                HIP_OK(hipMemcpyAsync(d_slab.p, d_lum + pix0, (size_t)M * sizeof(float), hipMemcpyDeviceToDevice, c->stream));
+            else if (!pix_uploaded)
+                upload_sample_pixels();
         } else if (M > 0) {
             PROFILED(c, NLE_K_SINKHORN_PASS, nlek::sink_pass(c->stream, mode, d_lum, ss.gs, d_samples.p, p, sk.d_w.p, nsw,
                                                              npw, pix0, M, NLE_EPS, ybuf, d_partial.p));
@@ -838,6 +864,7 @@
     f->r = ny.r;
     f->chol_ka = ny.chol ? 1 : 0;
     f->formulation = hist ? NLE_MODE_PHI_FREE : NLE_MODE_PHI_FREE_EXP;
+    if (hist && !pix_uploaded) upload_sample_pixels();
     tm_s.stop();
     tr.mark("ss: passes enqueued");
     HIP_OK(hipStreamSynchronize(c->stream));
@@ -863,10 +890,15 @@
         }
     };
     OrthoSS o;
+    PackedRows packed;
     if (hist && c->topk_solver == 0) {
+        packed.before_sync = [&] {
+            tm_g.stop();
+            tm_p.start();
+            tm_p.stop();
+        };
         ortho_ss_device(c, o, ny, p, sk.sA_c, sk.sA_r, d_tiles.p, n_eig, enqueue_gram,
-                        [&] { all_reduce(c, d_tiles.p, g_elems); }, &ms->host, &ms->host_overlapped, tr);
-        tm_g.stop();
+                        [&] { all_reduce(c, d_tiles.p, g_elems); }, &ms->host, &ms->host_overlapped, tr, &packed);
     } else {
         enqueue_gram();
         double h0 = now_ms();
@@ -887,14 +919,30 @@
     }
     adopt_ortho(f, o);
 
-    tm_p.start();
+    if (packed.ldd == 0) tm_p.start();
     if (o.K > 128) throw Fail{NLE_ERR_INVALID, "Phi-free path supports at most 128 eigenvectors"};
     const int ldd = nlek::project64_ld(o.K);
-    std::vector<double> Dp((size_t)p * ldd, 0.0);
-    for (int k = 0; k < o.K; ++k)
-        for (int a = 0; a < p; ++a) Dp[(size_t)a * ldd + k] = o.D[(size_t)k * p + a];
-    DevBuf<double> d_D(Dp.size());
-    HIP_OK(hipMemcpyAsync(d_D.p, Dp.data(), Dp.size() * sizeof(double), hipMemcpyHostToDevice, c->stream));
+    DevBuf<double> d_D, d_Vr;
+    std::vector<double> Dp, Vr;
+    if (packed.ldd > 0) {
+        if (packed.ldd != ldd) throw Fail{NLE_ERR_INVALID, "Phi-free path: packed coefficient rows of another width"};
+        d_D = std::move(packed.D);
+        d_Vr = std::move(packed.Vrows);
+    } else {
+        Dp.assign((size_t)p * ldd, 0.0);
+        for (int k = 0; k < o.K; ++k)
+            for (int a = 0; a < p; ++a) Dp[(size_t)a * ldd + k] = o.D[(size_t)k * p + a];
+        d_D.alloc(Dp.size());
+        HIP_OK(hipMemcpyAsync(d_D.p, Dp.data(), Dp.size() * sizeof(double), hipMemcpyHostToDevice, c->stream));
+        if (hist) {
+            Vr.assign((size_t)p * ldd, 0.0);
+            for (int k = 0; k < o.K; ++k)
+                for (int a = 0; a < p; ++a) Vr[(size_t)a * ldd + k] = o.Vrows[(size_t)k * p + a];
+            d_Vr.alloc(Vr.size());
+            HIP_OK(hipMemcpyAsync(d_Vr.p, Vr.data(), Vr.size() * sizeof(double), hipMemcpyHostToDevice, c->stream));
+            HIP_OK(hipStreamSynchronize(c->stream));
+        }
+    }
     if (hist) {
         auto own = [&](auto& buf) {
             using T = std::remove_pointer_t<decltype(buf.p)>;
@@ -903,22 +951,6 @@
             f->owned.emplace_back(ptr, bytes);
             return ptr;
         };
-        std::vector<double> Vr((size_t)p * ldd, 0.0);
-        for (int k = 0; k < o.K; ++k)
-            for (int a = 0; a < p; ++a) Vr[(size_t)a * ldd + k] = o.Vrows[(size_t)k * p + a];
-        DevBuf<double> d_Vr(Vr.size());
-        DevBuf<long long> d_spix(p), d_sloc(p);
-        DevBuf<float> d_slab((size_t)M);
-        std::vector<long long> sloc(p);
-        for (int a = 0; a < p; ++a) {
-            const long long loc = ss.pix[a] - pix0;
-            sloc[a] = (loc >= 0 && loc < M) ? loc : -1;
-        }
-        HIP_OK(hipMemcpyAsync(d_Vr.p, Vr.data(), Vr.size() * sizeof(double), hipMemcpyHostToDevice, c->stream));
-        HIP_OK(hipMemcpyAsync(d_spix.p, ss.pix.data(), p * sizeof(long long), hipMemcpyHostToDevice, c->stream));
-        HIP_OK(hipMemcpyAsync(d_sloc.p, sloc.data(), p * sizeof(long long), hipMemcpyHostToDevice, c->stream));
-        HIP_OK(hipMemcpyAsync(d_slab.p, d_lum + pix0, (size_t)M * sizeof(float), hipMemcpyDeviceToDevice, c->stream));
-        HIP_OK(hipStreamSynchronize(c->stream));
         f->lazy = true;
         f->gs = ss.gs;
         f->nsw = nsw;
@@ -944,7 +976,7 @@
         }
         f->h_Vrows = o.Vrows;
         f->h_sample_pix = ss.pix;
-        tm_p.stop();
+        if (packed.ldd == 0) tm_p.stop();
         ms->take(tm_s, tm_g, tm_p);
         return;
     }
@@ -1540,12 +1572,11 @@
         tr.mark("fetch_samples");
         f->p = ss.p;
         f->h_sample_pix = ss.pix;
-        double h0 = now_ms();
-        std::vector<double> Ka = build_Ka(ss, hx, hy);
-        tr.mark("build_Ka");
-        sm.host += now_ms() - h0;
+        std::vector<double> Ka;
         auto solve = [&](bool allow_chol) {
             const double t0 = now_ms();
+            Ka = build_Ka(ss, hx, hy);
+            tr.mark("build_Ka");
             Nystrom ny = solve_Ka(c, Ka, ss.p, allow_chol);
             tr.mark(ny.chol ? "chol(Ka)" : "eig(Ka)");
             sm.host += now_ms() - t0;
diff --git a/nonlocal-image-edit_amd/csrc/pipeline_internal.h b/nonlocal-image-edit_amd/csrc/pipeline_internal.h
--- a/nonlocal-image-edit_amd/csrc/pipeline_internal.h
+++ b/nonlocal-image-edit_amd/csrc/pipeline_internal.h
@@ -164,6 +164,15 @@
     explicit DevBuf(size_t count) { alloc(count); }
     DevBuf(const DevBuf&) = delete;
     DevBuf& operator=(const DevBuf&) = delete;
+    DevBuf(DevBuf&& o) noexcept : p(o.p), n(o.n), owner(o.owner) { o.p = nullptr, o.n = 0; }
+    DevBuf& operator=(DevBuf&& o) noexcept {
+        if (this != &o) {
+            release();
+            p = o.p, n = o.n, owner = o.owner;
+            o.p = nullptr, o.n = 0;
+        }
+        return *this;
+    }
     void alloc(size_t count) {
         release();
         if (count) {
@@ -395,12 +404,14 @@
     c->h_stage_used += bytes;
     return p;
 }
-inline void upload_staged(nle_ctx* c, double* d_dst, const double* h_src, size_t n, hipStream_t st) {
-    if (void* hp = pinned_take(c, n * sizeof(double))) {
+inline bool upload_staged(nle_ctx* c, double* d_dst, const double* h_src, size_t n, hipStream_t st) {
+    void* hp = pinned_take(c, n * sizeof(double));
+    if (hp) {
         std::memcpy(hp, h_src, n * sizeof(double));
         h_src = static_cast<const double*>(hp);
     }
     HIP_OK(hipMemcpyAsync(d_dst, h_src, n * sizeof(double), hipMemcpyHostToDevice, st));
+    return hp != nullptr;
 }
 
 inline double now_ms() {
```
